# norlab-ulaval/mask_bev

Measured on AMD Instinct MI355X. Metric: LiDAR scans/sec fwd+bwd, 120k-pt 512x512 BEV 100q, higher is better.
Workload: dtype bf16; 1 GPU; semantic_kitti_512: 120000 pts/scan, 512x512 BEV, 100 queries; scans_per_gpu=4, global_batch=4, parallelism=dp1, step=fwd + Hungarian loss + bwd + AdamW; inputs device-resident, launch=hip-graph, tuned_gemm_table=True, k3_adam_fused=True

## Files before the change

### include/maskbev_hip.h

```cpp
#ifndef MASKBEV_HIP_H_
#define MASKBEV_HIP_H_

#include <stddef.h>
#include <stdint.h>

#ifdef __cplusplus
extern "C" {
#endif

typedef enum {
  MBV_OK = 0,
  MBV_ERR_BAD_ARG = -1,
  MBV_ERR_WORKSPACE = -2,
  MBV_ERR_UNSUPPORTED = -3
} mbv_status;

int mbv_abi_version(void);

#define MBV_DT_F32 0
#define MBV_DT_BF16 1
#define MBV_DT_F16 2

size_t mbv_voxelize_workspace_bytes(int64_t total_points, int32_t batch, int64_t cells_per_scan);

// ... 18 lines not shown
int mbv_skinny_gemm_f32_supported(int64_t m, int32_t contraction, int32_t out_cols);
int mbv_skinny_gemm_f32(const float* x, const float* w, float* y, int64_t m, int32_t c, int32_t n, int32_t ldw,
                        int32_t weight_is_nk, void* stream);
int mbv_skinny_gemm_f32_addrows(const float* x, const float* w, float* y, int64_t m, int32_t c, int32_t n, int32_t ldw,
                                const float* add, const int64_t* index, void* stream);

int64_t mbv_pfn_forward_layout(int64_t num_rows, int64_t num_pillars, const int32_t* units, int32_t num_layers,
                               int64_t* offsets);
int mbv_pfn_forward(const float* rows, int32_t in_features, const int32_t* row_start, const int32_t* num_points,
                    const int64_t* row_pillar, int64_t num_rows, int64_t num_pillars, int32_t max_points,
                    const float* const* weights,
                    const float* const* gammas, const float* const* betas, float* const* running_means,
                    float* const* running_vars, const int32_t* units, int32_t num_layers, float eps, float momentum,
                    int32_t training, float* workspace, int64_t workspace_floats, void* stream);

int mbv_pfn_stats(float* y, const float* t, float* y_pad, const int32_t* row_start, const int32_t* num_points,
                  int64_t num_pillars, int32_t units, int32_t max_points, double* sums, void* stream);

int mbv_pfn_bn_finalize(const double* sums, double count, const float* gamma, const float* beta, float eps,
                        float momentum, int32_t training, float* running_mean, float* running_var, int32_t units,
                        float* scale, float* shift, float* mean, float* rstd, void* stream);

int mbv_pfn_apply_max(const float* y, const float* y_pad, const float* scale, const float* shift,
                      const int32_t* row_start, const int32_t* num_points, int64_t num_pillars, int32_t units,
                      int32_t max_points, float* a, float* a_pad, float* m, void* stream);

int mbv_pfn_bwd_route(const float* y, const float* y_pad, const float* scale, const float* shift,
                      const float* mean, const float* rstd, float* dz, int32_t has_da, const float* sum_da_pad,
                      const float* dm, const int32_t* row_start, const int32_t* num_points, int64_t num_pillars,
                      int32_t units, int32_t max_points, float* dz_pad, double* sums, void* stream);

int mbv_pfn_bwd_bn(const float* y, const float* y_pad, float* dz, float* dz_pad, const float* mean,
                   const float* rstd, const float* gamma, const double* sums, double count, int32_t training,
                   const int32_t* row_start, const int32_t* num_points, int64_t num_pillars, int32_t units,
                   int32_t max_points, float* dt, void* stream);

size_t mbv_scatter_layernorm_workspace_bytes(int32_t batch);

int mbv_scatter_layernorm_patch_supported(int32_t channels, int32_t ny, int32_t nx, int32_t patch);

int mbv_scatter_layernorm_fwd(const float* feats, const int32_t* pillar_batch_start,
                              const int32_t* cell_to_pillar, const float* weight, const float* bias,
                              int32_t batch, int32_t channels, int32_t ny, int32_t nx, float eps,
                              int32_t patch, int32_t patch_dtype, void* out, float* stats, void* workspace,
                              size_t workspace_bytes, void* stream, void* ev_start, void* ev_stop);
int mbv_scatter_layernorm_fwd2(const float* feats, const int32_t* pillar_batch_start, const int32_t* cell_to_pillar,
                               const float* weight, const float* bias, int32_t batch, int32_t channels, int32_t ny, int32_t nx,
                               float eps, int32_t patch, int32_t patch_dtype, void* out, float* stats, void* workspace,
                               size_t workspace_bytes, uint32_t* amax_out, void* stream, void* ev_start, void* ev_stop);

int mbv_scatter_layernorm_bwd(const void* grad_out, int32_t patch, int32_t patch_dtype, const float* feats,
                              const int32_t* pillar_batch_start, const int32_t* cell_to_pillar,
                              const float* weight, const float* stats,
                              int32_t batch, int32_t channels, int32_t ny, int32_t nx, int64_t num_pillars,
                              float* grad_feats, float* grad_weight, float* grad_bias, int32_t accumulate,
                              void* workspace, size_t workspace_bytes, void* stream,
                              void* ev_start, void* ev_stop);

int mbv_scatter_layernorm_bwd_adamw(const void* grad_out, int32_t patch, int32_t patch_dtype, const float* feats,
                                    const int32_t* pillar_batch_start, const int32_t* cell_to_pillar, float* weight,
                                    float* bias, const float* stats, int32_t batch, int32_t channels, int32_t ny, int32_t nx,
                                    int64_t num_pillars, float* grad_feats, float* exp_avg_w, float* exp_avg_sq_w,
                                    float* exp_avg_b, float* exp_avg_sq_b, void* shadow_w, void* shadow_b,
                                    int32_t shadow_dtype, float lr, float beta1, float beta2, float eps, float weight_decay,
                                    int64_t step, int32_t decoupled, void* workspace, size_t workspace_bytes, void* stream,
                                    void* ev_start, void* ev_stop);

int mbv_ms_deform_attn_fwd(const float* value, const int64_t* spatial_shapes, const int64_t* level_start,
                           const float* sampling_loc, const float* attn_weight,
                           int32_t batch, int32_t num_value, int32_t num_heads, int32_t head_dim,
                           int32_t num_levels, int32_t num_query, int32_t num_points,
                           float* out, void* stream);

int mbv_ms_deform_attn_fwd_v(const void* value, int32_t value_dtype, const int64_t* spatial_shapes, const int64_t* level_start,
                             const float* sampling_loc, const float* attn_weight, int32_t batch, int32_t num_value,
                             int32_t num_heads, int32_t head_dim, int32_t num_levels, int32_t num_query, int32_t num_points,
                             float* out, void* stream);
int mbv_ms_deform_attn_bwd_locattn(const float* grad_out, const void* value, int32_t value_dtype, const int64_t* spatial_shapes,
                                   const int64_t* level_start, const float* sampling_loc, const float* attn_weight,
                                   int32_t batch, int32_t num_value, int32_t num_heads, int32_t head_dim, int32_t num_levels,
                                   int32_t num_query, int32_t num_points, float* grad_loc, float* grad_attn, void* stream);

int mbv_ms_deform_attn_bwd_split(int32_t head_dim, int32_t num_levels, const int64_t* spatial_shapes_host);

int mbv_ms_deform_attn_bwd_value_packed_supported(int32_t head_dim, int32_t num_levels, int32_t num_points,
                                                  int32_t num_query, const int64_t* spatial_shapes_host);
size_t mbv_ms_deform_attn_bwd_value_packed_workspace_bytes(int32_t batch, int32_t num_heads, int32_t num_levels,
                                                           int32_t num_query);
int mbv_ms_deform_attn_bwd_value_packed(const float* grad_out, const float* sampling_loc, const float* attn_weight,
                                        int32_t batch, int32_t num_value, int32_t num_heads, int32_t head_dim,
                                        int32_t num_levels, int32_t num_query, int32_t num_points,
                                        const int64_t* spatial_shapes_host, void* grad_value, int32_t out_dtype,
                                        int64_t out_ld, void* workspace, size_t workspace_bytes, void* stream);

int mbv_ms_deform_attn_bwd(const float* grad_out, const float* value, const int64_t* spatial_shapes,
                           const int64_t* level_start, const float* sampling_loc, const float* attn_weight,
                           int32_t batch, int32_t num_value, int32_t num_heads, int32_t head_dim,
                           int32_t num_levels, int32_t num_query, int32_t num_points,
                           const int64_t* spatial_shapes_host, float* grad_value, float* grad_loc, float* grad_attn,
                           int32_t part, void* stream);

int mbv_msda_prepare_supported(int32_t num_levels, int32_t num_points);

int mbv_msda_query_inputs(const float* x, const float* pos, int64_t rows, int64_t pos_rows, int32_t C, int32_t dtype,
                          void* x_lo, void* q_lo, void* stream);

int mbv_msda_prepare_fwd(const void* offsets, const void* logits, int32_t is_bf16, const float* ref_points,
                         const int64_t* spatial_shapes_host, int32_t batch, int32_t num_query, int32_t num_heads,
                         int32_t num_levels, int32_t num_points, float* loc, float* attn, void* stream);

int mbv_msda_prepare_fwd_ld(const void* offsets, int64_t ld_offsets, const void* logits, int64_t ld_logits,
                            const float* bias_offsets, const float* bias_logits, int32_t is_bf16, const float* ref_points,
                            const int64_t* spatial_shapes_host, int32_t batch, int32_t num_query, int32_t num_heads,
                            int32_t num_levels, int32_t num_points, float* loc, float* attn, void* stream);

int mbv_msda_prepare_bwd(const float* grad_loc, const float* grad_attn, const float* attn,
                         const int64_t* spatial_shapes_host, int32_t batch, int32_t num_query, int32_t num_heads,
                         int32_t num_levels, int32_t num_points, int32_t out_bf16, void* grad_offsets,
                         void* grad_logits, void* stream);

int mbv_msda_prepare_bwd_ld(const float* grad_loc, const float* grad_attn, const float* attn,
                            const int64_t* spatial_shapes_host, int32_t batch, int32_t num_query, int32_t num_heads,
                            int32_t num_levels, int32_t num_points, int32_t out_bf16, void* grad_offsets,
                            int64_t ld_offsets, void* grad_logits, int64_t ld_logits, void* stream);

int64_t mbv_window_attn_lse_elems(int32_t batch, int32_t H, int32_t W, int32_t heads, int32_t ws);

int mbv_window_attn_fwd(const void* qkv, const float* qkv_bias, const float* bias_table, int32_t is_bf16,
                        int32_t batch, int32_t H, int32_t W, int32_t C, int32_t heads, int32_t ws, int32_t shift,
                        void* out, float* lse, void* stream);

int mbv_window_attn_bwd(const void* qkv, const float* qkv_bias, const float* bias_table, const void* out,
                        const void* grad_out, const float* lse, int32_t is_bf16,
                        int32_t batch, int32_t H, int32_t W, int32_t C, int32_t heads, int32_t ws, int32_t shift,
                        void* grad_qkv, float* grad_table, float* grad_qkv_bias, int32_t full_bias_grad,
                        int32_t accumulate, void* stream);

int mbv_window_attn_split_supported(int32_t C, int32_t heads, int32_t ws);
int mbv_window_attn_split_fwd(const float* qkv, const float* qkv_bias, const float* bias_table, int32_t batch, int32_t H,
                              int32_t W, int32_t C, int32_t heads, int32_t ws, int32_t shift, const uint32_t* amax_qkv,
                              float* out, float* lse, void* stream);
int mbv_window_attn_split_bwd(const float* qkv, const float* qkv_bias, const float* bias_table, const float* out,
                              const float* grad_out, const float* lse, int32_t batch, int32_t H, int32_t W, int32_t C,
                              int32_t heads, int32_t ws, int32_t shift, const uint32_t* amax_qkv,
                              const uint32_t* amax_grad_out, float* grad_qkv, float* grad_table, float* grad_qkv_bias,
                              int32_t full_bias_grad, int32_t accumulate, uint32_t* amax_grad_qkv, void* stream);

int mbv_point_sample_fwd(const float* src, const int32_t* src_index, const float* coords,
                         const int32_t* coord_index, int32_t num_rows, int32_t num_points, int32_t H, int32_t W,
                         float* out, void* stream);

int mbv_point_sample_bwd(const float* grad_out, const int32_t* src_index, const float* coords,
                         const int32_t* coord_index, int32_t num_rows, int32_t num_points, int32_t H, int32_t W,
                         int64_t num_src_maps, float* grad_src, void* stream);

int mbv_point_sample_bwd_stack(const float* grad_out, const int32_t* src_index, const float* coords,
                               const int32_t* coord_index, int32_t num_rows, int32_t num_points, int32_t H, int32_t W,
                               int32_t outer, int32_t inner, int32_t rows, void* grad_src, int32_t out_dtype, void* stream);

int64_t mbv_packed_mask_words(int32_t H, int32_t W);

int mbv_pack_binary_masks(const float* src, int64_t num_maps, int32_t H, int32_t W, uint32_t* packed, void* stream);

int mbv_point_sample_packed_fwd(const uint32_t* packed, const int32_t* src_index, const float* coords,
                                const int32_t* coord_index, int32_t num_rows, int32_t num_points,
                                int32_t H, int32_t W, float* out, void* stream);
// ... 324 lines not shown
```

### mask_bev_amd/_lib.py

```python
from __future__ import annotations

import ctypes
import os
from ctypes import c_double, c_float, c_int32, c_int64, c_size_t, c_void_p
from typing import Dict, List, Tuple

_PKG_DIR = os.path.dirname(os.path.abspath(__file__))
LIB_PATH = os.path.join(_PKG_DIR, 'libmaskbev_hip.so')

ABI_VERSION = 59


class MaskBevHipError(RuntimeError):
    pass


_P = c_void_p
_F = c_float
_I = c_int32
_L = c_int64
_D = c_double

SIGNATURES: Dict[str, Tuple[object, List[object]]] = {
    'mbv_abi_version': (ctypes.c_int, []),
    'mbv_voxelize_workspace_bytes': (c_size_t, [_L, _I, _L]),
    'mbv_voxelize': (ctypes.c_int, [_P, _I, _L, _P, _I, _F, _F, _F, _F, _F, _F, _F, _F, _F, _I, _I, _I, _I, _I, _I, _L,
                                    _P, _P, _P, _P, _P, _P, _P, c_size_t, _P]),
    'mbv_gather_voxels': (ctypes.c_int, [_P, _I, _P, _L, _I, _P, _P]),
    'mbv_pfn_decorate': (ctypes.c_int, [_P, _I, _P, _P, _P, _P, _L, _I, _F, _F, _F, _F, _F, _F, _P, _P, _P]),
    'mbv_pfn_stats': (ctypes.c_int, [_P, _P, _P, _P, _P, _L, _I, _I, _P, _P]),
    'mbv_pfn_bn_finalize': (ctypes.c_int, [_P, c_double, _P, _P, _F, _F, _I, _P, _P, _I, _P, _P, _P, _P, _P]),
    'mbv_pfn_apply_max': (ctypes.c_int, [_P, _P, _P, _P, _P, _P, _L, _I, _I, _P, _P, _P, _P]),
    'mbv_pfn_bwd_route': (ctypes.c_int, [_P, _P, _P, _P, _P, _P, _P, _I, _P, _P, _P, _P, _L, _I, _I, _P, _P, _P]),
    'mbv_pfn_bwd_bn': (ctypes.c_int, [_P, _P, _P, _P, _P, _P, _P, _P, c_double, _I, _P, _P, _L, _I, _I, _P, _P]),
    'mbv_scatter_layernorm_workspace_bytes': (c_size_t, [_I]),
    'mbv_scatter_layernorm_patch_supported': (ctypes.c_int, [_I, _I, _I, _I]),
    'mbv_scatter_layernorm_fwd': (ctypes.c_int, [_P, _P, _P, _P, _P, _I, _I, _I, _I, _F, _I, _I, _P, _P, _P, c_size_t,
                                                 _P, _P, _P]),
    'mbv_scatter_layernorm_fwd2': (ctypes.c_int, [_P, _P, _P, _P, _P, _I, _I, _I, _I, _F, _I, _I, _P, _P, _P, c_size_t,
                                                  _P, _P, _P, _P]),
    'mbv_scatter_layernorm_bwd': (ctypes.c_int, [_P, _I, _I, _P, _P, _P, _P, _P, _I, _I, _I, _I, _L, _P, _P, _P, _I, _P,
                                                 c_size_t, _P, _P, _P]),
    'mbv_scatter_layernorm_bwd_adamw': (ctypes.c_int, [_P, _I, _I, _P, _P, _P, _P, _P, _P, _I, _I, _I, _I, _L, _P, _P, _P, _P, _P,
                                                       _P, _P, _I, _F, _F, _F, _F, _F, _L, _I, _P, c_size_t, _P, _P, _P]),
    'mbv_msda_prepare_supported': (ctypes.c_int, [_I, _I]),
    'mbv_pfn_forward_layout': (ctypes.c_int64, [_L, _L, _P, _I, _P]),
    'mbv_pfn_forward': (ctypes.c_int, [_P, _I, _P, _P, _P, _L, _L, _I, _P, _P, _P, _P, _P, _P, _I, _F, _F, _I, _P, _L, _P]),
    'mbv_skinny_gemm_f32_addrows': (ctypes.c_int, [_P, _P, _P, _L, _I, _I, _I, _P, _P, _P]),
    'mbv_skinny_gemm_f32_supported': (ctypes.c_int, [_L, _I, _I]),
    'mbv_skinny_gemm_f32': (ctypes.c_int, [_P, _P, _P, _L, _I, _I, _I, _I, _P]),
    'mbv_msda_prepare_fwd': (ctypes.c_int, [_P, _P, _I, _P, _P, _I, _I, _I, _I, _I, _P, _P, _P]),
    'mbv_msda_prepare_fwd_ld': (ctypes.c_int, [_P, _L, _P, _L, _P, _P, _I, _P, _P, _I, _I, _I, _I, _I, _P, _P, _P]),
    'mbv_msda_prepare_bwd': (ctypes.c_int, [_P, _P, _P, _P, _I, _I, _I, _I, _I, _I, _P, _P, _P]),
    'mbv_msda_prepare_bwd_ld': (ctypes.c_int, [_P, _P, _P, _P, _I, _I, _I, _I, _I, _I, _P, _L, _P, _L, _P]),
    'mbv_ms_deform_attn_fwd': (ctypes.c_int, [_P, _P, _P, _P, _P, _I, _I, _I, _I, _I, _I, _I, _P, _P]),
    'mbv_ms_deform_attn_fwd_v': (ctypes.c_int, [_P, _I, _P, _P, _P, _P, _I, _I, _I, _I, _I, _I, _I, _P, _P]),
    'mbv_ms_deform_attn_bwd_locattn': (ctypes.c_int, [_P, _P, _I, _P, _P, _P, _P, _I, _I, _I, _I, _I, _I, _I, _P, _P, _P]),
    'mbv_ms_deform_attn_bwd_split': (ctypes.c_int, [_I, _I, _P]),
    'mbv_ms_deform_attn_bwd_value_packed_supported': (ctypes.c_int, [_I, _I, _I, _I, _P]),
    'mbv_ms_deform_attn_bwd_value_packed_workspace_bytes': (c_size_t, [_I, _I, _I, _I]),
    'mbv_ms_deform_attn_bwd_value_packed': (ctypes.c_int, [_P, _P, _P, _I, _I, _I, _I, _I, _I, _I, _P, _P, _I, _L, _P, c_size_t, _P]),
    'mbv_ms_deform_attn_bwd': (ctypes.c_int, [_P, _P, _P, _P, _P, _P, _I, _I, _I, _I, _I, _I, _I, _P, _P, _P, _P, _I,
                                              _P]),
    'mbv_rowchain_max_stages': (ctypes.c_int, []),
    'mbv_rowchain_slots': (ctypes.c_int, []),
    'mbv_rowchain_run': (ctypes.c_int, [_P, _I, _I, _I, _F, _I, _P]),
    'mbv_rowchain_run_split': (ctypes.c_int, [_P, _I, _I, _I, _F, _I, _I, _P]),
    'mbv_transpose_group': (ctypes.c_int, [_P, _P, _P, _P, _I, _I, _P]),
    'mbv_copy_group': (ctypes.c_int, [_P, _P, _P, _I, _P]),
    'mbv_fragment_group': (ctypes.c_int, [_P, _P, _P, _P, _P, _P, _I, _P]),
    'mbv_window_attn_lse_elems': (_L, [_I, _I, _I, _I, _I]),
    'mbv_window_attn_fwd': (ctypes.c_int, [_P, _P, _P, _I, _I, _I, _I, _I, _I, _I, _I, _P, _P, _P]),
    'mbv_window_attn_bwd': (ctypes.c_int, [_P, _P, _P, _P, _P, _P, _I, _I, _I, _I, _I, _I, _I, _I, _P, _P, _P, _I, _I, _P]),
    'mbv_point_sample_fwd': (ctypes.c_int, [_P, _P, _P, _P, _I, _I, _I, _I, _P, _P]),
    'mbv_point_sample_bwd': (ctypes.c_int, [_P, _P, _P, _P, _I, _I, _I, _I, _L, _P, _P]),
    'mbv_point_sample_bwd_stack': (ctypes.c_int, [_P, _P, _P, _P, _I, _I, _I, _I, _I, _I, _I, _P, _I, _P]),
    'mbv_hungarian': (ctypes.c_int, [_P, _I, _I, _I, _P, _P]),
    'mbv_hungarian_padded': (ctypes.c_int, [_P, _I, _I, _I, _P, _P, _P]),
    'mbv_hungarian_wide_t': (ctypes.c_int, [_P, _I, _I, _I, _P, _P]),
    'mbv_select_uncertain_points': (ctypes.c_int, [_P, _P, _L, _I, _I, _P, _P]),
    'mbv_adamw_step': (ctypes.c_int, [_P, _P, _P, _P, _P, _I, _L, _F, _F, _F, _F, _F, _L, _F, _I, _I, _P, _P, _P, _P]),
    'mbv_grad_nonfinite': (ctypes.c_int, [_P, _L, _P, _P]),
    'mbv_loss_scale_update': (ctypes.c_int, [_P, _P, _P, _F, _F, _I, _P, _P]),
    'mbv_refresh_shadow': (ctypes.c_int, [_P, _P, _I, _L, _P]),
    'mbv_colsum_accum': (ctypes.c_int, [_P, _I, _L, _I, _P, _P]),
    'mbv_act_bwd_colsum': (ctypes.c_int, [_P, _P, _I, _I, _L, _I, _P, _P, _P]),
    'mbv_wgrad_small_f32': (ctypes.c_int, [_P, _P, _I, _I, _I, _P, _P, _P]),
    'mbv_wgrad_small_f32_group': (ctypes.c_int, [_P, _P, _P, _P, _P, _P, _P, _I, _P]),
    'mbv_mask_loss_rows_fwd': (ctypes.c_int, [_P, _P, _L, _I, _P, _P]),
    'mbv_mask_loss_rows_bwd': (ctypes.c_int, [_P, _P, _P, _L, _I, _P, _P]),
    'mbv_dice_bce_reduce': (ctypes.c_int, [_P, _L, _I, _F, _F, _P, _P, _P, _P]),
    'mbv_mask_loss_rows_bwd_coef': (ctypes.c_int, [_P, _P, _P, _P, _I, _P, _I, _L, _I, _I, _P, _P]),
    'mbv_sample_select_uncertain': (ctypes.c_int, [_P, _P, _P, _P, _L, _I, _I, _I, _I, _P, _I, _P, _P]),
    'mbv_uniform_points': (ctypes.c_int, [_P, _L, _I, _P, _P]),
    'mbv_add_layernorm_supported': (ctypes.c_int, [_I]),
    'mbv_add_layernorm_bwd_blocks': (_L, [_L, _I]),
    'mbv_add_layernorm_fwd': (ctypes.c_int, [_P, _I, _P, _I, _P, _P, _L, _I, _F, _P, _P, _I, _P, _P, _P]),
    'mbv_add_layernorm_fwd2': (ctypes.c_int, [_P, _I, _P, _I, _L, _P, _P, _L, _I, _F, _P, _P, _I, _P, _I, _P, _P, _P]),
    'mbv_transposed_batch_sum_accum': (ctypes.c_int, [_P, _I, _L, _I, _P, _P]),
    'mbv_add_layernorm_bwd': (ctypes.c_int, [_P, _I, _P, _I, _P, _P, _P, _P, _L, _I, _P, _P, _I, _P, _P, _I, _P, _P,
                                             _I, _P]),
    'mbv_add_layernorm_bwd2': (ctypes.c_int, [_P, _I, _P, _I, _P, _I, _P, _P, _P, _P, _L, _I, _P, _P, _I, _P, _P, _I, _P,
                                              _P, _I, _P]),
    'mbv_add_layernorm_bwd3': (ctypes.c_int, [_P, _I, _P, _I, _P, _I, _P, _P, _P, _P, _L, _I, _P, _P, _I, _P, _P, _I, _P,
                                              _P, _I, _P, _P]),
    'mbv_add_layernorm_bwd_direct': (ctypes.c_int, [_L, _I]),
    'mbv_merge_layernorm_supported': (ctypes.c_int, [_I, _I, _I]),
    'mbv_merge_layernorm_fwd': (ctypes.c_int, [_P, _L, _I, _I, _I, _P, _P, _F, _P, _I, _P, _P, _P]),
    'mbv_merge_layernorm_bwd': (ctypes.c_int, [_P, _I, _P, _P, _P, _P, _L, _I, _I, _I, _P, _P, _P, _I, _P, _I, _P]),
    'mbv_colsum_accum_group': (ctypes.c_int, [_P, _P, _P, _P, _P, _P, _I, _P]),
    'mbv_instance_ids': (ctypes.c_int, [_P, _I, _I, _I, _I, _I, _P, _P, _P, _P]),
    'mbv_expand_instance_masks': (ctypes.c_int, [_P, _P, _I, _I, _I, _I, _P, _P, _P]),
    'mbv_matched_mask_iou': (ctypes.c_int, [_P, _P, _P, _P, _I, _I, _I, _I, _I, _P, _P, _P]),
    'mbv_match_cost_terms': (ctypes.c_int, [_P, _L, _I, _I, _I, _P, _P, _P]),
    'mbv_match_cost': (ctypes.c_int, [_P, _P, _P, _P, _L, _I, _I, _I, _I, _I, _P, _P]),
    'mbv_match_products_supported': (ctypes.c_int, [_I, _I, _I]),
    'mbv_match_products': (ctypes.c_int, [_P, _P, _L, _I, _I, _I, _I, _P, _P, _P]),
    'mbv_match_cost_split': (ctypes.c_int, [_P, _P, _P, _P, _L, _I, _I, _I, _I, _I, _I, _P, _P]),
    'mbv_cls_loss_fwd': (ctypes.c_int, [_P, _P, _P, _P, _I, _I, _I, _I, _I, _F, _F, _P, _P, _P]),
    'mbv_cls_loss_bwd': (ctypes.c_int, [_P, _P, _P, _P, _P, _P, _I, _I, _I, _I, _I, _F, _F, _P, _P]),
    'mbv_packed_mask_words': (_L, [_I, _I]),
    'mbv_pack_binary_masks': (ctypes.c_int, [_P, _L, _I, _I, _P, _P]),
    'mbv_point_sample_packed_fwd': (ctypes.c_int, [_P, _P, _P, _P, _I, _I, _I, _I, _P, _P]),
    'mbv_mask_logits_fwd': (ctypes.c_int, [_P, _P, _I, _I, _I, _I, _L, _P, _I, _P]),
    'mbv_attn_mask_from_logits': (ctypes.c_int, [_P, _I, _L, _I, _I, _I, _I, _P, _P]),
    'mbv_attn_workspace_bytes': (c_size_t, [_I, _I, _I, _I, _I]),
    'mbv_attn_fwd': (ctypes.c_int, [_P, _P, _P, _P, _I, _I, _I, _I, _I, _I, _P, _P, _P, c_size_t, _P]),
    'mbv_attn_bwd': (ctypes.c_int, [_P, _P, _P, _P, _P, _P, _P, _I, _I, _I, _I, _I, _I, _P, _P, _P, _P]),
    'mbv_attn_fwd_ld': (ctypes.c_int, [_P, _P, _P, _I, _P, _I, _I, _I, _I, _I, _I, _P, _P, _P, c_size_t, _P]),
    'mbv_gemm16_supported': (ctypes.c_int, [_I, _L, _L, _L]),
    'mbv_gemm16_nt': (ctypes.c_int, [_P, _P, _P, _P, _P, _L, _L, _L, _L, _L, _L, _I, _I, _I, _I, _L, _L, _L, _P]),
    'mbv_gemm16_nt_acc': (ctypes.c_int, [_P, _P, _P, _L, _L, _L, _L, _L, _L, _I, _I, _I, _L, _L, _L, _P]),
    'mbv_gemm16_nn_workspace_bytes': (c_size_t, [_L, _L, _I]),
    'mbv_gemm16_nn': (ctypes.c_int, [_P, _P, _P, _P, _P, _L, _L, _L, _L, _L, _L, _L, _I, _I, _I, _I, _L, _L, _L, _P,
                                     c_size_t, _P]),
    'mbv_gemm16_nn_part_rows': (ctypes.c_int64, [_L, _L, _I]),
    'mbv_gemm16_nn_parts': (ctypes.c_int, [_P, _P, _P, _P, _P, c_size_t, _L, _L, _L, _L, _L, _L, _L, _I, _I, _I, _I, _L,
                                           _L, _L, _P]),
    'mbv_gemm16_tn_workspace_bytes': (c_size_t, [_L, _L, _L]),
    'mbv_gemm16_tn': (ctypes.c_int, [_P, _P, _P, _L, _L, _L, _L, _L, _L, _I, _I, _I, _I, _I, _L, _L, _L, _P, c_size_t,
                                     _P]),
# ... 99 lines not shown
```

### mask_bev_amd/csrc/msda.hip

```cpp

#include "common.hpp"

namespace {

__device__ __forceinline__ int64_t xcd_block(unsigned bid, unsigned nwg) {
  const unsigned q = nwg >> 3, r = nwg & 7, x = bid & 7, s = bid >> 3;
  return (int64_t)((x < r ? x * (q + 1) : r * (q + 1) + (x - r) * q) + s);
}

struct Corner {
  int off[4];
  float wgt[4];
  float lh, lw;
};

__device__ __forceinline__ bool bilinear_setup(float loc_x, float loc_y, int h, int w, int stride_pix, Corner& c) {
  const float him = loc_y * (float)h - 0.5f;
  const float wim = loc_x * (float)w - 0.5f;
  if (!(him > -1.f && wim > -1.f && him < (float)h && wim < (float)w)) return false;
  const int hl = (int)floorf(him), wl = (int)floorf(wim);
  const int hh = hl + 1, wh = wl + 1;
  const float lh = him - (float)hl, lw = wim - (float)wl;
  const float uh = 1.f - lh, uw = 1.f - lw;
  c.lh = lh;
  c.lw = lw;
  c.wgt[0] = uh * uw;
  c.wgt[1] = uh * lw;
  c.wgt[2] = lh * uw;
  c.wgt[3] = lh * lw;
  c.off[0] = (hl >= 0 && wl >= 0) ? (hl * w + wl) * stride_pix : -1;
  c.off[1] = (hl >= 0 && wh <= w - 1) ? (hl * w + wh) * stride_pix : -1;
  c.off[2] = (hh <= h - 1 && wl >= 0) ? (hh * w + wl) * stride_pix : -1;
  c.off[3] = (hh <= h - 1 && wh <= w - 1) ? (hh * w + wh) * stride_pix : -1;
  return true;
}

__global__ void __launch_bounds__(256) k_msda_fwd(const float* __restrict__ value,
                                                  const int64_t* __restrict__ shapes,
                                                  const int64_t* __restrict__ level_start,
                                                  const float* __restrict__ loc, const float* __restrict__ attn,
                                                  int64_t total, int num_value, int heads, int dim, int levels,
                                                  int num_query, int points, float* __restrict__ out) {
  const int64_t idx = (int64_t)blockIdx.x * blockDim.x + threadIdx.x;
  if (idx >= total) return;
  const int d = (int)(idx % dim);
  int64_t t = idx / dim;
  const int hd = (int)(t % heads);
  t /= heads;
  const int b = (int)(t / num_query);
  const int stride_pix = heads * dim;
  const float* vb = value + (int64_t)b * num_value * stride_pix + hd * dim + d;
  const int64_t lw_base = (t * heads + hd) * levels * points;
  float acc = 0.f;
  for (int l = 0; l < levels; ++l) {
    const int h = (int)shapes[l * 2], w = (int)shapes[l * 2 + 1];
    const float* vl = vb + level_start[l] * stride_pix;
    for (int p = 0; p < points; ++p) {
      const int64_t k = lw_base + l * points + p;
      const float lx = loc[k * 2], ly = loc[k * 2 + 1], aw = attn[k];
      Corner c;
      if (bilinear_setup(lx, ly, h, w, stride_pix, c)) {
        float v = 0.f;
#pragma unroll
        for (int j = 0; j < 4; ++j)
          if (c.off[j] >= 0) v += c.wgt[j] * vl[c.off[j]];
        acc += aw * v;
      }
    }
  }
  out[idx] = acc;
}

template <int VK>
__device__ __forceinline__ float4 value4(const void* __restrict__ base, int64_t elem) {
  if constexpr (VK == MBV_DT_F32) {
    return *reinterpret_cast<const float4*>(reinterpret_cast<const float*>(base) + elem);
  } else {
    const uint2 u = *reinterpret_cast<const uint2*>(reinterpret_cast<const unsigned short*>(base) + elem);
    if constexpr (VK == MBV_DT_BF16)
      return make_float4(__uint_as_float(u.x << 16), __uint_as_float(u.x & 0xffff0000u), __uint_as_float(u.y << 16),
                         __uint_as_float(u.y & 0xffff0000u));
    return make_float4((float)__builtin_bit_cast(_Float16, (unsigned short)(u.x & 0xffffu)),
                       (float)__builtin_bit_cast(_Float16, (unsigned short)(u.x >> 16)),
                       (float)__builtin_bit_cast(_Float16, (unsigned short)(u.y & 0xffffu)),
// ... 411 lines not shown
  l1 = red[0];
#pragma unroll
  for (int i = 1; i < NT / 64; ++i) l1 += red[i];
  l1 *= 1.0001f;
  if (!(l1 == l1) || l1 > 3.0e38f) l1 = 3.0e38f;
  int e = 0;
  if (l1 > 0.f) (void)frexpf(l1, &e);
  const float scale = ldexpf(1.f, 29 - e), inv_scale = ldexpf(1.f, e - 29);
  float4 n_go = make_float4(0.f, 0.f, 0.f, 0.f), n_l01 = n_go, n_l23 = n_go, n_a4 = n_go;
  const float* go_b = A.go_t + ((((int64_t)b * heads + hd) * 8 + grp4) * num_query) * 4 + (PLANES == 2 ? 0 : (split & 1) * 2);
  const float* loc_b = A.loc_t + ((((int64_t)b * heads + hd) * levels + level) * num_query) * 8;
  const float* attn_b = A.attn_t + ((((int64_t)b * heads + hd) * levels + level) * num_query) * 4;
  auto load_q = [&](int q, float4& go, float4& l01, float4& l23, float4& a4) {
    if constexpr (PLANES == 2) {
      go = *reinterpret_cast<const float4*>(go_b + (int64_t)q * 4);
    } else {
      const float2 g = *reinterpret_cast<const float2*>(go_b + (int64_t)q * 4);
      go = make_float4(g.x, g.y, 0.f, 0.f);
    }
    l01 = *reinterpret_cast<const float4*>(loc_b + (int64_t)q * 8);
    l23 = *reinterpret_cast<const float4*>(loc_b + (int64_t)q * 8 + 4);
    a4 = *reinterpret_cast<const float4*>(attn_b + (int64_t)q * 4);
  };
  if ((int)threadIdx.x < num_query) load_q(threadIdx.x, n_go, n_l01, n_l23, n_a4);
  for (int q = threadIdx.x; q < num_query; q += NT) {
    float4 go = n_go;
    const float4 l01 = n_l01, l23 = n_l23, a4 = n_a4;
    if (q + NT < num_query) load_q(q + NT, n_go, n_l01, n_l23, n_a4);
    go.x *= scale; go.y *= scale; go.z *= scale; go.w *= scale;
    const float lx[4] = {l01.x, l01.z, l23.x, l23.z}, ly[4] = {l01.y, l01.w, l23.y, l23.w};
    const float aw[4] = {a4.x, a4.y, a4.z, a4.w};
#pragma unroll
    for (int u = 0; u < 4; ++u) {
      Corner c;
      if (!bilinear_setup(lx[u], ly[u], h, w, 1, c)) continue;
#pragma unroll
      for (int j = 0; j < 4; ++j) {
        const int off = c.off[j];
        if (off < 0) continue;
        const float wj = c.wgt[j] * aw[u];
        atomicAdd(&map[off], fx_pack(wj * go.x, wj * go.y));
        if constexpr (PLANES == 2) atomicAdd(&map[npix + off], fx_pack(wj * go.z, wj * go.w));
      }
    }
  }
  __syncthreads();
  const int64_t gv = ((int64_t)b * A.num_value + A.lstart[level]) * A.out_ld + hd * dim + split * CH;
  for (int i = threadIdx.x; i < npix; i += NT) {
#pragma unroll
    for (int pl = 0; pl < PLANES; ++pl) {
      const long long v = (long long)map[pl * npix + i];
      const int lo = (int)(unsigned)(v & 0xffffffffll);
      const int hi = (int)((v - (long long)lo) >> 32);
      fx_store2<DT>(A.out, gv + (int64_t)i * A.out_ld + 2 * pl, (float)lo * inv_scale, (float)hi * inv_scale);
    }
  }
}

struct Taps4 {
  int off[4];
  float wgt[4];
};
__device__ __forceinline__ void taps_clamped(float loc_x, float loc_y, float aw, int h, int w, int stride_pix, Taps4& t) {
  const float him = loc_y * (float)h - 0.5f;
  const float wim = loc_x * (float)w - 0.5f;
  const bool in = him > -1.f && wim > -1.f && him < (float)h && wim < (float)w;
  const int hl = (int)floorf(him), wl = (int)floorf(wim);
  const int hh = hl + 1, wh = wl + 1;
  const float lh = him - (float)hl, lw = wim - (float)wl;
  const float uh = 1.f - lh, uw = 1.f - lw;
  const bool t0 = in && hl >= 0 && wl >= 0, t1 = in && hl >= 0 && wh <= w - 1;
  const bool t2 = in && hh <= h - 1 && wl >= 0, t3 = in && hh <= h - 1 && wh <= w - 1;
  t.off[0] = t0 ? (hl * w + wl) * stride_pix : 0;
  t.off[1] = t1 ? (hl * w + wh) * stride_pix : 0;
  t.off[2] = t2 ? (hh * w + wl) * stride_pix : 0;
  t.off[3] = t3 ? (hh * w + wh) * stride_pix : 0;
  t.wgt[0] = t0 ? aw * uh * uw : 0.f;
  t.wgt[1] = t1 ? aw * uh * lw : 0.f;
  t.wgt[2] = t2 ? aw * lh * uw : 0.f;
  t.wgt[3] = t3 ? aw * lh * lw : 0.f;
}

template <int VK>
__global__ void __launch_bounds__(256) k_msda_fwd_p4(const void* __restrict__ value, const int64_t* __restrict__ shapes,
                                                     const int64_t* __restrict__ level_start,
                                                     const float* __restrict__ loc, const float* __restrict__ attn,
                                                     int64_t total4, int num_value, int heads, int dim, int levels,
                                                     int num_query, float* __restrict__ out) {
  const int64_t idx = xcd_block(blockIdx.x, gridDim.x) * blockDim.x + threadIdx.x;
  if (idx >= total4) return;
  const int d4n = dim >> 2;
  const int d4 = (int)(idx % d4n);
  int64_t t = idx / d4n;
  const int hd = (int)(t % heads);
  t /= heads;
  const int b = (int)(t / num_query);
  const int stride_pix = heads * dim;
  const int64_t vb = (int64_t)b * num_value * stride_pix + hd * dim + d4 * 4;
  const int64_t lw_base = (t * heads + hd) * levels * 4;
  float4 acc = make_float4(0.f, 0.f, 0.f, 0.f);
  for (int l = 0; l < levels; ++l) {
    const int h = (int)shapes[l * 2], w = (int)shapes[l * 2 + 1];
    const int64_t vl = vb + level_start[l] * stride_pix;
    const float4 xy0 = *reinterpret_cast<const float4*>(loc + (lw_base + l * 4) * 2);
    const float4 xy1 = *reinterpret_cast<const float4*>(loc + (lw_base + l * 4) * 2 + 4);
    const float4 aw = *reinterpret_cast<const float4*>(attn + lw_base + l * 4);
    Taps4 tp[4];
    taps_clamped(xy0.x, xy0.y, aw.x, h, w, stride_pix, tp[0]);
    taps_clamped(xy0.z, xy0.w, aw.y, h, w, stride_pix, tp[1]);
    taps_clamped(xy1.x, xy1.y, aw.z, h, w, stride_pix, tp[2]);
    taps_clamped(xy1.z, xy1.w, aw.w, h, w, stride_pix, tp[3]);
    float4 x[16];
#pragma unroll
    for (int p = 0; p < 4; ++p)
#pragma unroll
      for (int j = 0; j < 4; ++j) x[p * 4 + j] = value4<VK>(value, vl + tp[p].off[j]);
#pragma unroll
    for (int p = 0; p < 4; ++p)
#pragma unroll
      for (int j = 0; j < 4; ++j) {
        const float wj = tp[p].wgt[j];
        acc.x += wj * x[p * 4 + j].x; acc.y += wj * x[p * 4 + j].y;
        acc.z += wj * x[p * 4 + j].z; acc.w += wj * x[p * 4 + j].w;
      }
  }
  *reinterpret_cast<float4*>(out + ((t * heads + hd) * dim + d4 * 4)) = acc;
}

__global__ void __launch_bounds__(256) k_msda_bwd_relayout(const float* __restrict__ grad_out,
                                                           const float* __restrict__ loc, const float* __restrict__ attn,
                                                           int num_query, int heads, int levels, int q_tiles,
                                                           float* __restrict__ go_t, float* __restrict__ loc_t,
                                                           float* __restrict__ attn_t, float* __restrict__ l1_part) {
  __shared__ __attribute__((aligned(16))) float s_go[64 * 32];
  __shared__ __attribute__((aligned(16))) float s_loc[64 * 8 * 8];
  __shared__ __attribute__((aligned(16))) float s_at[64 * 8 * 4];
  __shared__ float s_sum[8 * 8];
  const int tile = blockIdx.x % q_tiles;
  const int bh = blockIdx.x / q_tiles;
  const int hd = bh % heads, b = bh / heads;
  const int q0 = tile * 64;
  const int tid = threadIdx.x;
  if (tid < 64) s_sum[tid] = 0.f;
  for (int p = tid; p < 64 * 8; p += 256) {
    const int q = p >> 3, c = p & 7;
    const int qq = q0 + q < num_query ? q0 + q : num_query - 1;
    *reinterpret_cast<float4*>(s_go + q * 32 + c * 4) =
        *reinterpret_cast<const float4*>(grad_out + (((int64_t)b * num_query + qq) * heads + hd) * 32 + c * 4);
  }
  const int lp = levels * 2;
  for (int p = tid; p < 64 * lp; p += 256) {
    const int q = p / lp, c = p - q * lp;
    const int qq = q0 + q < num_query ? q0 + q : num_query - 1;
    *reinterpret_cast<float4*>(s_loc + q * 64 + c * 4) =
        *reinterpret_cast<const float4*>(loc + ((((int64_t)b * num_query + qq) * heads + hd) * levels) * 8 + c * 4);
  }
  for (int p = tid; p < 64 * levels; p += 256) {
    const int q = p / levels, l = p - q * levels;
    const int qq = q0 + q < num_query ? q0 + q : num_query - 1;
    *reinterpret_cast<float4*>(s_at + q * 32 + l * 4) =
        *reinterpret_cast<const float4*>(attn + ((((int64_t)b * num_query + qq) * heads + hd) * levels + l) * 4);
  }
  __syncthreads();
  for (int p = tid; p < 8 * 64; p += 256) {
    const int g = p >> 6, q = p & 63;
    if (q0 + q < num_query)
      *reinterpret_cast<float4*>(go_t + ((((int64_t)b * heads + hd) * 8 + g) * num_query + q0 + q) * 4) =
          *reinterpret_cast<const float4*>(s_go + q * 32 + g * 4);
  }
  for (int p = tid; p < levels * 64 * 2; p += 256) {
    const int l = p / 128, r = p - l * 128, q = r >> 1, hf = r & 1;
    if (q0 + q < num_query)
      *reinterpret_cast<float4*>(loc_t + ((((int64_t)b * heads + hd) * levels + l) * num_query + q0 + q) * 8 + hf * 4) =
          *reinterpret_cast<const float4*>(s_loc + q * 64 + l * 8 + hf * 4);
  }
  for (int p = tid; p < levels * 64; p += 256) {
    const int l = p >> 6, q = p & 63;
    if (q0 + q < num_query)
      *reinterpret_cast<float4*>(attn_t + ((((int64_t)b * heads + hd) * levels + l) * num_query + q0 + q) * 4) =
          *reinterpret_cast<const float4*>(s_at + q * 32 + l * 4);
  }
  for (int p = tid; p < 64 * 8; p += 256) {
    const int q = p & 63, g = p >> 6;
    const bool live = q0 + q < num_query;
    const float4 gv = *reinterpret_cast<const float4*>(s_go + q * 32 + g * 4);
    const float m = fmaxf(fmaxf(fabsf(gv.x), fabsf(gv.y)), fmaxf(fabsf(gv.z), fabsf(gv.w)));
    for (int l = 0; l < levels; ++l) {
      const float4 a = *reinterpret_cast<const float4*>(s_at + q * 32 + l * 4);
      float t = live ? m * (fabsf(a.x) + fabsf(a.y) + fabsf(a.z) + fabsf(a.w)) : 0.f;
#pragma unroll
      for (int o = 32; o > 0; o >>= 1) t += __shfl_xor(t, o);
      if ((tid & 63) == 0) s_sum[l * 8 + g] = t;
    }
  }
  __syncthreads();
  if (tid < levels * 8) {
    const int l = tid >> 3, g = tid & 7;
    l1_part[((((int64_t)b * heads + hd) * q_tiles + tile) * levels + l) * 8 + g] = s_sum[l * 8 + g];
  }
}

template <int DT>
__global__ void __launch_bounds__(512) k_msda_bwd_value_fx(const MsdaFxArgs A) {
  extern __shared__ __attribute__((aligned(16))) unsigned long long fxmap[];
  int level = 0;
  for (int l = 1; l < A.levels; ++l)
    if ((int)blockIdx.x >= A.block_begin[l]) level = l;
  const int local = (int)blockIdx.x - A.block_begin[level];
  if (A.planes[level] == 2)
// ... 11 lines not shown
                                                          int64_t total8, int num_value, int heads, int levels,
                                                          int num_query, int points, float* __restrict__ grad_loc,
                                                          float* __restrict__ grad_attn) {
  constexpr int dim = 32;
  const int stride_pix = heads * dim;
  const int64_t idx = xcd_block(blockIdx.x, gridDim.x) * blockDim.x + threadIdx.x;
  const bool live = idx < total8;
  const int64_t sidx = live ? idx : total8 - 1;
  const int d4 = (int)(sidx & 7);
  int64_t t = sidx >> 3;
  const int hd = (int)(t % heads);
  t /= heads;
  const int b = (int)(t / num_query);
  const int64_t vb = (int64_t)b * num_value * stride_pix + hd * dim + d4 * 4;
  const int64_t lw_base = (t * heads + hd) * levels * points;
  const float4 go = *reinterpret_cast<const float4*>(grad_out + (t * heads + hd) * dim + d4 * 4);
  float keep_w = 0.f, keep_x = 0.f, keep_y = 0.f;
  for (int l = 0; l < levels; ++l) {
    const int h = (int)shapes[l * 2], w = (int)shapes[l * 2 + 1];
    const int64_t vl = vb + level_start[l] * stride_pix;
    for (int p = 0; p < points; ++p) {
      const int64_t k = lw_base + l * points + p;
      const float lx = loc[k * 2], ly = loc[k * 2 + 1], aw = attn[k];
      float g_w = 0.f, g_x = 0.f, g_y = 0.f;
      Corner c;
      if (bilinear_setup(lx, ly, h, w, stride_pix, c)) {
        float s4[4];
#pragma unroll
        for (int j = 0; j < 4; ++j) {
          s4[j] = 0.f;
          if (c.off[j] >= 0) {
            const float4 x = value4<VK>(value, vl + c.off[j]);
            s4[j] = go.x * x.x + go.y * x.y + go.z * x.z + go.w * x.w;
          }
        }
        const float uh = 1.f - c.lh, uw = 1.f - c.lw;
        g_w = c.wgt[0] * s4[0] + c.wgt[1] * s4[1] + c.wgt[2] * s4[2] + c.wgt[3] * s4[3];
        const float gh = -uw * s4[0] - c.lw * s4[1] + uw * s4[2] + c.lw * s4[3];
        const float gw = -uh * s4[0] + uh * s4[1] - c.lh * s4[2] + c.lh * s4[3];
        g_x = (float)w * gw * aw;
        g_y = (float)h * gh * aw;
      }
      g_w = group8_allsum(g_w);
      g_x = group8_allsum(g_x);
      g_y = group8_allsum(g_y);
      const int sidx8 = l * points + p;
      if ((sidx8 & 7) == d4) { keep_w = g_w; keep_x = g_x; keep_y = g_y; }
      if ((sidx8 & 7) == 7 || (l == levels - 1 && p == points - 1)) {
        const int first = sidx8 & ~7;
        if (live && first + d4 <= sidx8) {
          grad_attn[lw_base + first + d4] = keep_w;
          *reinterpret_cast<float2*>(grad_loc + (lw_base + first + d4) * 2) = make_float2(keep_x, keep_y);
        }
      }
    }
  }
}

struct TapsG {
  int off[4];
  float ok[4];
  float lh, lw;
  float in;
};
__device__ __forceinline__ void taps_grad(float loc_x, float loc_y, int h, int w, int stride_pix, TapsG& t) {
  const float him = loc_y * (float)h - 0.5f;
  const float wim = loc_x * (float)w - 0.5f;
  const bool in = him > -1.f && wim > -1.f && him < (float)h && wim < (float)w;
  const int hl = (int)floorf(him), wl = (int)floorf(wim);
  const int hh = hl + 1, wh = wl + 1;
  t.lh = him - (float)hl;
  t.lw = wim - (float)wl;
  t.in = in ? 1.f : 0.f;
  const bool t0 = in && hl >= 0 && wl >= 0, t1 = in && hl >= 0 && wh <= w - 1;
  const bool t2 = in && hh <= h - 1 && wl >= 0, t3 = in && hh <= h - 1 && wh <= w - 1;
  t.off[0] = t0 ? (hl * w + wl) * stride_pix : 0;
  t.off[1] = t1 ? (hl * w + wh) * stride_pix : 0;
  t.off[2] = t2 ? (hh * w + wl) * stride_pix : 0;
  t.off[3] = t3 ? (hh * w + wh) * stride_pix : 0;
  t.ok[0] = t0 ? 1.f : 0.f; t.ok[1] = t1 ? 1.f : 0.f; t.ok[2] = t2 ? 1.f : 0.f; t.ok[3] = t3 ? 1.f : 0.f;
}

template <int VK>
__global__ void __launch_bounds__(256) k_msda_bwd_locattn_p4(const float* __restrict__ grad_out,
                                                             const void* __restrict__ value,
                                                             const int64_t* __restrict__ shapes,
                                                             const int64_t* __restrict__ level_start,
                                                             const float* __restrict__ loc, const float* __restrict__ attn,
                                                             int64_t total8, int num_value, int heads, int levels,
                                                             int num_query, float* __restrict__ grad_loc,
                                                             float* __restrict__ grad_attn) {
  constexpr int dim = 32, points = 4;
  const int stride_pix = heads * dim;
  const int64_t idx = xcd_block(blockIdx.x, gridDim.x) * blockDim.x + threadIdx.x;
  const bool live = idx < total8;
  const int64_t sidx = live ? idx : total8 - 1;
  const int d4 = (int)(sidx & 7);
  int64_t t = sidx >> 3;
  const int hd = (int)(t % heads);
  t /= heads;
  const int b = (int)(t / num_query);
  const int64_t vb = (int64_t)b * num_value * stride_pix + hd * dim + d4 * 4;
  const int64_t lw_base = (t * heads + hd) * levels * points;
  const float4 go = *reinterpret_cast<const float4*>(grad_out + (t * heads + hd) * dim + d4 * 4);
  float keep_w = 0.f, keep_x = 0.f, keep_y = 0.f;
  for (int l = 0; l < levels; ++l) {
    const int h = (int)shapes[l * 2], w = (int)shapes[l * 2 + 1];
    const int64_t vl = vb + level_start[l] * stride_pix;
    const float4 xy0 = *reinterpret_cast<const float4*>(loc + (lw_base + l * 4) * 2);
    const float4 xy1 = *reinterpret_cast<const float4*>(loc + (lw_base + l * 4) * 2 + 4);
    const float4 aw4 = *reinterpret_cast<const float4*>(attn + lw_base + l * 4);
    const float awp[4] = {aw4.x, aw4.y, aw4.z, aw4.w};
    TapsG tp[4];
    taps_grad(xy0.x, xy0.y, h, w, stride_pix, tp[0]);
    taps_grad(xy0.z, xy0.w, h, w, stride_pix, tp[1]);
    taps_grad(xy1.x, xy1.y, h, w, stride_pix, tp[2]);
    taps_grad(xy1.z, xy1.w, h, w, stride_pix, tp[3]);
    float4 x[16];
#pragma unroll
    for (int p = 0; p < 4; ++p)
#pragma unroll
      for (int j = 0; j < 4; ++j) x[p * 4 + j] = value4<VK>(value, vl + tp[p].off[j]);
#pragma unroll
    for (int p = 0; p < 4; ++p) {
      float s4[4];
#pragma unroll
      for (int j = 0; j < 4; ++j) {
        const float4 v = x[p * 4 + j];
        s4[j] = tp[p].ok[j] * (go.x * v.x + go.y * v.y + go.z * v.z + go.w * v.w);
      }
      const float lh = tp[p].lh, lw = tp[p].lw, uh = 1.f - lh, uw = 1.f - lw;
      float g_w = uh * uw * s4[0] + uh * lw * s4[1] + lh * uw * s4[2] + lh * lw * s4[3];
      const float gh = -uw * s4[0] - lw * s4[1] + uw * s4[2] + lw * s4[3];
      const float gw = -uh * s4[0] + uh * s4[1] - lh * s4[2] + lh * s4[3];
      float g_x = (float)w * gw * awp[p] * tp[p].in;
      float g_y = (float)h * gh * awp[p] * tp[p].in;
      g_w = group8_allsum(g_w * tp[p].in);
      g_x = group8_allsum(g_x);
      g_y = group8_allsum(g_y);
      const int sidx8 = l * points + p;
      if ((sidx8 & 7) == d4) { keep_w = g_w; keep_x = g_x; keep_y = g_y; }
      if ((sidx8 & 7) == 7 || (l == levels - 1 && p == points - 1)) {
        const int first = sidx8 & ~7;
        if (live && first + d4 <= sidx8) {
          grad_attn[lw_base + first + d4] = keep_w;
          *reinterpret_cast<float2*>(grad_loc + (lw_base + first + d4) * 2) = make_float2(keep_x, keep_y);
        }
      }
    }
  }
}

struct MsdaLevels {
  int levels;
  int h[8], w[8], lstart[8];
};

bool pow2_le64(int d) { return d > 0 && d <= 64 && (d & (d - 1)) == 0; }

}

extern "C" int mbv_ms_deform_attn_fwd(const float* value, const int64_t* spatial_shapes, const int64_t* level_start,
                                      const float* sampling_loc, const float* attn_weight, int32_t batch,
                                      int32_t num_value, int32_t num_heads, int32_t head_dim, int32_t num_levels,
                                      int32_t num_query, int32_t num_points, float* out, void* stream_) {
  hipStream_t stream = reinterpret_cast<hipStream_t>(stream_);
  if (batch <= 0 || num_value <= 0 || num_heads <= 0 || num_levels <= 0 || num_query <= 0 || num_points <= 0)
    return MBV_ERR_BAD_ARG;
  if (!pow2_le64(head_dim)) return MBV_ERR_UNSUPPORTED;
  if (!value || !spatial_shapes || !level_start || !sampling_loc || !attn_weight || !out) return MBV_ERR_BAD_ARG;
  const int64_t total = (int64_t)batch * num_query * num_heads * head_dim;
  if ((head_dim & 3) == 0 && ((reinterpret_cast<size_t>(value) | reinterpret_cast<size_t>(out)) & 15) == 0) {
    const int64_t total4 = total / 4;
    if (num_points == 4 && ((reinterpret_cast<size_t>(sampling_loc) | reinterpret_cast<size_t>(attn_weight)) & 15) == 0) {
      hipLaunchKernelGGL(k_msda_fwd_p4<MBV_DT_F32>, dim3((unsigned)((total4 + 255) / 256)), dim3(256), 0, stream,
                         (const void*)value, spatial_shapes, level_start, sampling_loc, attn_weight, total4, num_value,
                         num_heads, head_dim, num_levels, num_query, out);
      MBV_CHECK_LAUNCH();
      return MBV_OK;
    }
    hipLaunchKernelGGL(k_msda_fwd_v4<MBV_DT_F32>, dim3((unsigned)((total4 + 255) / 256)), dim3(256), 0, stream,
                       (const void*)value, spatial_shapes, level_start, sampling_loc, attn_weight, total4, num_value,
                       num_heads, head_dim, num_levels, num_query, num_points, out);
    MBV_CHECK_LAUNCH();
    return MBV_OK;
  }
  hipLaunchKernelGGL(k_msda_fwd, dim3((unsigned)((total + 255) / 256)), dim3(256), 0, stream, value, spatial_shapes,
                     level_start, sampling_loc, attn_weight, total, num_value, num_heads, head_dim, num_levels,
                     num_query, num_points, out);
  MBV_CHECK_LAUNCH();
  return MBV_OK;
}

extern "C" int mbv_ms_deform_attn_fwd_v(const void* value, int32_t value_dtype, const int64_t* spatial_shapes,
                                        const int64_t* level_start, const float* sampling_loc, const float* attn_weight,
                                        int32_t batch, int32_t num_value, int32_t num_heads, int32_t head_dim,
                                        int32_t num_levels, int32_t num_query, int32_t num_points, float* out, void* stream_) {
  if (value_dtype == MBV_DT_F32)
    return mbv_ms_deform_attn_fwd(reinterpret_cast<const float*>(value), spatial_shapes, level_start, sampling_loc,
                                  attn_weight, batch, num_value, num_heads, head_dim, num_levels, num_query, num_points, out,
                                  stream_);
  hipStream_t stream = reinterpret_cast<hipStream_t>(stream_);
  if (batch <= 0 || num_value <= 0 || num_heads <= 0 || num_levels <= 0 || num_query <= 0 || num_points <= 0)
    return MBV_ERR_BAD_ARG;
  if (value_dtype != MBV_DT_BF16 && value_dtype != MBV_DT_F16) return MBV_ERR_BAD_ARG;
  if (!pow2_le64(head_dim) || (head_dim & 3)) return MBV_ERR_UNSUPPORTED;
  if (!value || !spatial_shapes || !level_start || !sampling_loc || !attn_weight || !out) return MBV_ERR_BAD_ARG;
  if ((reinterpret_cast<size_t>(value) & 7) || (reinterpret_cast<size_t>(out) & 15)) return MBV_ERR_UNSUPPORTED;
  const int64_t total4 = (int64_t)batch * num_query * num_heads * head_dim / 4;
  const dim3 grid((unsigned)((total4 + 255) / 256)), block(256);
  if (num_points == 4 && ((reinterpret_cast<size_t>(sampling_loc) | reinterpret_cast<size_t>(attn_weight)) & 15) == 0) {
    if (value_dtype == MBV_DT_BF16)
      hipLaunchKernelGGL(k_msda_fwd_p4<MBV_DT_BF16>, grid, block, 0, stream, value, spatial_shapes, level_start, sampling_loc,
                         attn_weight, total4, num_value, num_heads, head_dim, num_levels, num_query, out);
    else
      hipLaunchKernelGGL(k_msda_fwd_p4<MBV_DT_F16>, grid, block, 0, stream, value, spatial_shapes, level_start, sampling_loc,
                         attn_weight, total4, num_value, num_heads, head_dim, num_levels, num_query, out);
    MBV_CHECK_LAUNCH();
    return MBV_OK;
  }
  if (value_dtype == MBV_DT_BF16)
    hipLaunchKernelGGL(k_msda_fwd_v4<MBV_DT_BF16>, grid, block, 0, stream, value, spatial_shapes, level_start, sampling_loc,
                       attn_weight, total4, num_value, num_heads, head_dim, num_levels, num_query, num_points, out);
  else
    hipLaunchKernelGGL(k_msda_fwd_v4<MBV_DT_F16>, grid, block, 0, stream, value, spatial_shapes, level_start, sampling_loc,
                       attn_weight, total4, num_value, num_heads, head_dim, num_levels, num_query, num_points, out);
  MBV_CHECK_LAUNCH();
  return MBV_OK;
}

extern "C" int mbv_ms_deform_attn_bwd_locattn(const float* grad_out, const void* value, int32_t value_dtype,
                                              const int64_t* spatial_shapes, const int64_t* level_start,
                                              const float* sampling_loc, const float* attn_weight, int32_t batch,
                                              int32_t num_value, int32_t num_heads, int32_t head_dim, int32_t num_levels,
                                              int32_t num_query, int32_t num_points, float* grad_loc, float* grad_attn,
                                              void* stream_) {
  hipStream_t stream = reinterpret_cast<hipStream_t>(stream_);
  if (batch <= 0 || num_value <= 0 || num_heads <= 0 || num_levels <= 0 || num_query <= 0 || num_points <= 0)
    return MBV_ERR_BAD_ARG;
  if (head_dim != 32) return MBV_ERR_UNSUPPORTED;
  if (!grad_out || !value || !spatial_shapes || !level_start || !sampling_loc || !attn_weight || !grad_loc || !grad_attn)
    return MBV_ERR_BAD_ARG;
  if ((reinterpret_cast<size_t>(grad_out) & 15) || (reinterpret_cast<size_t>(value) & (value_dtype == MBV_DT_F32 ? 15 : 7)))
    return MBV_ERR_UNSUPPORTED;
  const int64_t total8 = (int64_t)batch * num_query * num_heads * 8;
  const dim3 grid((unsigned)((total8 + 255) / 256)), block(256);
  const bool p4 = num_points == 4 && ((reinterpret_cast<size_t>(sampling_loc) | reinterpret_cast<size_t>(attn_weight)) & 15) == 0;
#define MBV_LOCATTN(VK)                                                                                                  \
  if (p4)                                                                                                                \
    hipLaunchKernelGGL(k_msda_bwd_locattn_p4<VK>, grid, block, 0, stream, grad_out, value, spatial_shapes, level_start,  \
                       sampling_loc, attn_weight, total8, num_value, num_heads, num_levels, num_query, grad_loc,         \
                       grad_attn);                                                                                       \
  else                                                                                                                   \
    hipLaunchKernelGGL(k_msda_bwd_locattn<VK>, grid, block, 0, stream, grad_out, value, spatial_shapes, level_start,     \
                       sampling_loc, attn_weight, total8, num_value, num_heads, num_levels, num_query, num_points,       \
                       grad_loc, grad_attn)
  if (value_dtype == MBV_DT_F32) { MBV_LOCATTN(MBV_DT_F32); }
  else if (value_dtype == MBV_DT_BF16) { MBV_LOCATTN(MBV_DT_BF16); }
  else if (value_dtype == MBV_DT_F16) { MBV_LOCATTN(MBV_DT_F16); }
  else return MBV_ERR_BAD_ARG;
#undef MBV_LOCATTN
  MBV_CHECK_LAUNCH();
  return MBV_OK;
}

extern "C" int mbv_ms_deform_attn_bwd_split(int32_t head_dim, int32_t num_levels, const int64_t* spatial_shapes_host) {
  if (!spatial_shapes_host || head_dim != 32 || num_levels <= 0 || num_levels > 8) return 0;
  for (int l = 0; l < num_levels; ++l) {
    const int64_t h = spatial_shapes_host[2 * l], w = spatial_shapes_host[2 * l + 1];
    if (h <= 0 || w <= 0 || h * w > 4096) return 0;
  }
  return 1;
}

extern "C" int mbv_ms_deform_attn_bwd(const float* grad_out, const float* value, const int64_t* spatial_shapes,
                                      const int64_t* level_start, const float* sampling_loc,
                                      const float* attn_weight, int32_t batch, int32_t num_value, int32_t num_heads,
                                      int32_t head_dim, int32_t num_levels, int32_t num_query, int32_t num_points,
                                      const int64_t* spatial_shapes_host, float* grad_value, float* grad_loc,
                                      float* grad_attn, int32_t part, void* stream_) {
  hipStream_t stream = reinterpret_cast<hipStream_t>(stream_);
  if (batch <= 0 || num_value <= 0 || num_heads <= 0 || num_levels <= 0 || num_query <= 0 || num_points <= 0)
    return MBV_ERR_BAD_ARG;
  if (!pow2_le64(head_dim)) return MBV_ERR_UNSUPPORTED;
  if (!grad_out || !value || !spatial_shapes || !level_start || !sampling_loc || !attn_weight) return MBV_ERR_BAD_ARG;
  if ((!grad_value && ((part & 3) != 2)) || ((!grad_loc || !grad_attn) && ((part & 3) != 1))) return MBV_ERR_BAD_ARG;
  const int level_mask = part >> 2;
  part &= 3;
  if (part < 1 || level_mask < 0 || level_mask > 255 || (level_mask && part != 1)) return MBV_ERR_BAD_ARG;
  {
    bool fits = mbv_ms_deform_attn_bwd_split(head_dim, num_levels, spatial_shapes_host) != 0 &&
                ((reinterpret_cast<size_t>(grad_out) | reinterpret_cast<size_t>(value) |
                  reinterpret_cast<size_t>(grad_value) | reinterpret_cast<size_t>(sampling_loc) |
                  reinterpret_cast<size_t>(attn_weight)) & 15) == 0;
    MsdaLevels lv;
    lv.levels = num_levels;
    int lstart = 0, max_pix = 0;
    for (int l = 0; fits && l < num_levels; ++l) {
      const int h = (int)spatial_shapes_host[2 * l], w = (int)spatial_shapes_host[2 * l + 1];
      if (h <= 0 || w <= 0 || h * w > 4096) { fits = false; break; }
      lv.h[l] = h; lv.w[l] = w; lv.lstart[l] = lstart;
      lstart += h * w;
      if (h * w > max_pix) max_pix = h * w;
    }
    if (fits && lstart == num_value) {
      static bool attr_done = false;
      if (!attr_done && max_pix * 32 > 65536) {
        MBV_CHECK_HIP(hipFuncSetAttribute(reinterpret_cast<const void*>(&k_msda_bwd_value<4>),
                                          hipFuncAttributeMaxDynamicSharedMemorySize, 131072));
        MBV_CHECK_HIP(hipFuncSetAttribute(reinterpret_cast<const void*>(&k_msda_bwd_value<0>),
                                          hipFuncAttributeMaxDynamicSharedMemorySize, 131072));
        attr_done = true;
      }
      const int which = part;
      for (int l = num_levels - 1; l >= 0 && (which & 1); --l) {
        if (level_mask && !((level_mask >> l) & 1)) continue;
        const dim3 grid((unsigned)(batch * num_heads * 8)), block(1024);
        const size_t lds = (size_t)lv.h[l] * lv.w[l] * 4 * sizeof(double);
        if (num_points == 4)
          hipLaunchKernelGGL(k_msda_bwd_value<4>, grid, block, lds, stream, grad_out, sampling_loc, attn_weight, l,
                             num_levels, lv.h[l], lv.w[l], lv.lstart[l], num_value, num_query, num_heads, num_points,
                             grad_value);
        else
          hipLaunchKernelGGL(k_msda_bwd_value<0>, grid, block, lds, stream, grad_out, sampling_loc, attn_weight, l,
                             num_levels, lv.h[l], lv.w[l], lv.lstart[l], num_value, num_query, num_heads, num_points,
                             grad_value);
        MBV_CHECK_LAUNCH();
      }
      if (which & 2) {
        const int64_t total8 = (int64_t)batch * num_query * num_heads * 8;
        if (num_points == 4 && ((reinterpret_cast<size_t>(sampling_loc) | reinterpret_cast<size_t>(attn_weight)) & 15) == 0)
          hipLaunchKernelGGL(k_msda_bwd_locattn_p4<MBV_DT_F32>, dim3((unsigned)((total8 + 255) / 256)), dim3(256), 0, stream,
                             grad_out, (const void*)value, spatial_shapes, level_start, sampling_loc, attn_weight, total8,
                             num_value, num_heads, num_levels, num_query, grad_loc, grad_attn);
        else
          hipLaunchKernelGGL(k_msda_bwd_locattn<MBV_DT_F32>, dim3((unsigned)((total8 + 255) / 256)), dim3(256), 0, stream,
                             grad_out, (const void*)value, spatial_shapes, level_start, sampling_loc, attn_weight, total8,
                             num_value, num_heads, num_levels, num_query, num_points, grad_loc, grad_attn);
        MBV_CHECK_LAUNCH();
      }
      return MBV_OK;
    }
  }
  if (part != 3) return MBV_ERR_UNSUPPORTED;
  MBV_CHECK_HIP(mbv_fill_async(grad_value, 0, sizeof(float) * (size_t)batch * num_value * num_heads * head_dim, stream));
  if (spatial_shapes_host && num_query == num_value && num_levels <= 8) {
    MsdaBands cfg;
    cfg.levels = num_levels;
// ... 133 lines not shown
```

### mask_bev_amd/csrc/msda_prepare.hip

```cpp
#include "common.hpp"

namespace {

constexpr int kMaxLP = 16;

template <typename T>
__device__ __forceinline__ float ldf(const T* p);
template <>
__device__ __forceinline__ float ldf<float>(const float* p) { return *p; }
template <>
__device__ __forceinline__ float ldf<unsigned short>(const unsigned short* p) { return __uint_as_float((unsigned)*p << 16); }
template <typename T>
__device__ __forceinline__ void stf(T* p, float v);
template <>
__device__ __forceinline__ void stf<float>(float* p, float v) { *p = v; }
template <>
__device__ __forceinline__ void stf<unsigned short>(unsigned short* p, float v) { *p = f32_to_bf16_rne(v); }
template <typename T>
__device__ __forceinline__ float round_like(float v);
template <>
__device__ __forceinline__ float round_like<float>(float v) { return v; }
template <>
__device__ __forceinline__ float round_like<unsigned short>(float v) { return __uint_as_float((unsigned)f32_to_bf16_rne(v) << 16); }

template <typename T>
__device__ __forceinline__ void ld4(const T* p, float* v);
template <>
__device__ __forceinline__ void ld4<float>(const float* p, float* v) {
  const float4 q = *reinterpret_cast<const float4*>(p);
  v[0] = q.x; v[1] = q.y; v[2] = q.z; v[3] = q.w;
}
template <>
__device__ __forceinline__ void ld4<unsigned short>(const unsigned short* p, float* v) {
  const uint2 u = *reinterpret_cast<const uint2*>(p);
  v[0] = __uint_as_float(u.x << 16); v[1] = __uint_as_float(u.x & 0xffff0000u);
  v[2] = __uint_as_float(u.y << 16); v[3] = __uint_as_float(u.y & 0xffff0000u);
}
template <typename T>
__device__ __forceinline__ void st4(T* p, const float* v);
template <>
__device__ __forceinline__ void st4<float>(float* p, const float* v) {
  *reinterpret_cast<float4*>(p) = make_float4(v[0], v[1], v[2], v[3]);
}
template <>
__device__ __forceinline__ void st4<unsigned short>(unsigned short* p, const float* v) {
  uint2 u;
  u.x = pack_bf16x2(v[0], v[1]);
  u.y = pack_bf16x2(v[2], v[3]);
  *reinterpret_cast<uint2*>(p) = u;
}

template <>
__device__ __forceinline__ float ldf<_Float16>(const _Float16* p) { return (float)*p; }
template <>
__device__ __forceinline__ void stf<_Float16>(_Float16* p, float v) { *p = (_Float16)v; }
template <>
__device__ __forceinline__ float round_like<_Float16>(float v) { return (float)(_Float16)v; }
template <>
__device__ __forceinline__ void ld4<_Float16>(const _Float16* p, float* v) {
  typedef _Float16 h4 __attribute__((ext_vector_type(4)));
  const h4 q = *reinterpret_cast<const h4*>(p);
  v[0] = (float)q[0]; v[1] = (float)q[1]; v[2] = (float)q[2]; v[3] = (float)q[3];
}
template <>
__device__ __forceinline__ void st4<_Float16>(_Float16* p, const float* v) {
  typedef _Float16 h4 __attribute__((ext_vector_type(4)));
  h4 q;
  q[0] = (_Float16)v[0]; q[1] = (_Float16)v[1]; q[2] = (_Float16)v[2]; q[3] = (_Float16)v[3];
  *reinterpret_cast<h4*>(p) = q;
}

struct Norm { float w[8], h[8]; };

template <typename T>
__global__ void __launch_bounds__(256) k_msda_prepare_fwd(const T* __restrict__ off, const T* __restrict__ logit,
                                                          const float* __restrict__ ref, Norm nrm, long rows,
                                                          int num_query, int heads, int levels, int points,
                                                          float* __restrict__ loc, float* __restrict__ attn,
                                                          long ld_off, long ld_logit, const float* __restrict__ b_off,
                                                          const float* __restrict__ b_logit) {
  const long i = (long)blockIdx.x * blockDim.x + threadIdx.x;
  if (i >= rows) return;
  const int lp = levels * points;
  const long tok = i / heads;
  const int head = (int)(i - tok * heads);
  const int n = (int)(tok % num_query);
  const float rx = ref[2 * n], ry = ref[2 * n + 1];
  const T* o = off + tok * ld_off + (long)head * lp * 2;
  const T* a = logit + tok * ld_logit + (long)head * lp;
  const float* bo = b_off ? b_off + (long)head * lp * 2 : nullptr;
  const float* ba = b_logit ? b_logit + (long)head * lp : nullptr;
  float v[kMaxLP];
  float m = -INFINITY;
  const bool vec = (lp & 3) == 0;
  if (vec) {
#pragma unroll
    for (int k = 0; k < kMaxLP; k += 4) {
      if (k < lp) ld4<T>(a + k, v + k);
      else v[k] = v[k + 1] = v[k + 2] = v[k + 3] = -INFINITY;
    }
  } else {
#pragma unroll
    for (int k = 0; k < kMaxLP; ++k) v[k] = k < lp ? ldf<T>(a + k) : -INFINITY;
  }
  if (ba) {
#pragma unroll
    for (int k = 0; k < kMaxLP; ++k)
      if (k < lp) v[k] += ba[k];
  }
#pragma unroll
  for (int k = 0; k < kMaxLP; ++k) m = fmaxf(m, v[k]);
  float s = 0.f;
#pragma unroll
  for (int k = 0; k < kMaxLP; ++k) {
    v[k] = k < lp ? expf(v[k] - m) : 0.f;
    s += v[k];
  }
  const float inv = 1.f / s;
  float* lo = loc + i * lp * 2;
  float* ao = attn + i * lp;
  if (vec) {
#pragma unroll
    for (int k = 0; k < kMaxLP; k += 4) {
      if (k < lp) {
        const float w4[4] = {v[k] * inv, v[k + 1] * inv, v[k + 2] * inv, v[k + 3] * inv};
        st4<float>(ao + k, w4);
        float o8[8], r8[8];
        ld4<T>(o + 2 * k, o8);
        ld4<T>(o + 2 * k + 4, o8 + 4);
        if (bo) {
#pragma unroll
          for (int e = 0; e < 8; ++e) o8[e] += bo[2 * k + e];
        }
#pragma unroll
        for (int e = 0; e < 4; ++e) {
          const int l = (k + e) / points;
          r8[2 * e] = rx + round_like<T>(o8[2 * e] / nrm.w[l]);
          r8[2 * e + 1] = ry + round_like<T>(o8[2 * e + 1] / nrm.h[l]);
        }
        st4<float>(lo + 2 * k, r8);
        st4<float>(lo + 2 * k + 4, r8 + 4);
      }
    }
    return;
  }
#pragma unroll
  for (int k = 0; k < kMaxLP; ++k) {
    if (k < lp) {
      const int l = k / points;
      ao[k] = v[k] * inv;
      lo[2 * k] = rx + round_like<T>((ldf<T>(o + 2 * k) + (bo ? bo[2 * k] : 0.f)) / nrm.w[l]);
      lo[2 * k + 1] = ry + round_like<T>((ldf<T>(o + 2 * k + 1) + (bo ? bo[2 * k + 1] : 0.f)) / nrm.h[l]);
    }
  }
}

template <typename T>
__global__ void __launch_bounds__(256) k_msda_prepare_bwd(const float* __restrict__ g_loc,
                                                          const float* __restrict__ g_attn,
                                                          const float* __restrict__ attn, Norm nrm, long rows,
                                                          int levels, int points, T* __restrict__ g_off,
                                                          T* __restrict__ g_logit, int heads, long ld_off,
                                                          long ld_logit) {
  const long i = (long)blockIdx.x * blockDim.x + threadIdx.x;
  if (i >= rows) return;
  const int lp = levels * points;
  const float* gl = g_loc + i * lp * 2;
  const float* ga = g_attn + i * lp;
  const float* aw = attn + i * lp;
  float a[kMaxLP], g[kMaxLP];
  float dot = 0.f;
  const bool vec = (lp & 3) == 0;
  if (vec) {
#pragma unroll
    for (int k = 0; k < kMaxLP; k += 4) {
      if (k < lp) {
        ld4<float>(aw + k, a + k);
        ld4<float>(ga + k, g + k);
      } else {
        a[k] = a[k + 1] = a[k + 2] = a[k + 3] = 0.f;
        g[k] = g[k + 1] = g[k + 2] = g[k + 3] = 0.f;
      }
    }
  } else {
#pragma unroll
    for (int k = 0; k < kMaxLP; ++k) {
      a[k] = k < lp ? aw[k] : 0.f;
      g[k] = k < lp ? ga[k] : 0.f;
    }
  }
#pragma unroll
  for (int k = 0; k < kMaxLP; ++k) dot += a[k] * g[k];
  const long bn = i / heads;
  const int hh = (int)(i - bn * heads);
  T* go = g_off + bn * ld_off + (long)hh * lp * 2;
  T* gq = g_logit + bn * ld_logit + (long)hh * lp;
  if (vec) {
#pragma unroll
    for (int k = 0; k < kMaxLP; k += 4) {
      if (k < lp) {
        const float q4[4] = {a[k] * (g[k] - dot), a[k + 1] * (g[k + 1] - dot), a[k + 2] * (g[k + 2] - dot),
                             a[k + 3] * (g[k + 3] - dot)};
        st4<T>(gq + k, q4);
        float l8[8], o8[8];
        ld4<float>(gl + 2 * k, l8);
        ld4<float>(gl + 2 * k + 4, l8 + 4);
#pragma unroll
        for (int e = 0; e < 4; ++e) {
          const int l = (k + e) / points;
          o8[2 * e] = round_like<T>(l8[2 * e]) / nrm.w[l];
          o8[2 * e + 1] = round_like<T>(l8[2 * e + 1]) / nrm.h[l];
        }
        st4<T>(go + 2 * k, o8);
        st4<T>(go + 2 * k + 4, o8 + 4);
      }
    }
    return;
  }
#pragma unroll
  for (int k = 0; k < kMaxLP; ++k) {
    if (k < lp) {
      const int l = k / points;
      stf<T>(gq + k, a[k] * (g[k] - dot));
      stf<T>(go + 2 * k, round_like<T>(gl[2 * k]) / nrm.w[l]);
      stf<T>(go + 2 * k + 1, round_like<T>(gl[2 * k + 1]) / nrm.h[l]);
    }
  }
}

bool fill_norm(const int64_t* shapes_host, int levels, Norm& n) {
  if (!shapes_host || levels < 1 || levels > 8) return false;
  for (int l = 0; l < 8; ++l) { n.w[l] = 1.f; n.h[l] = 1.f; }
  for (int l = 0; l < levels; ++l) {
    const int64_t h = shapes_host[2 * l], w = shapes_host[2 * l + 1];
    if (h <= 0 || w <= 0) return false;
    n.h[l] = (float)h; n.w[l] = (float)w;
  }
  return true;
}

__global__ void __launch_bounds__(256) k_msda_query_inputs(const float* __restrict__ x, const float* __restrict__ pos,
                                                           long n4, long pos_n4, int f16, unsigned short* __restrict__ x_lo,
                                                           unsigned short* __restrict__ q_lo) {
  const long i = (long)blockIdx.x * 256 + threadIdx.x;
  if (i >= n4) return;
  const float4 a = reinterpret_cast<const float4*>(x)[i];
  const float4 p = reinterpret_cast<const float4*>(pos)[i % pos_n4];
  const float q[4] = {a.x + p.x, a.y + p.y, a.z + p.z, a.w + p.w};
  const float v[4] = {a.x, a.y, a.z, a.w};
  unsigned short xo[4], qo[4];
#pragma unroll
  for (int e = 0; e < 4; ++e) {
    if (f16) {
      xo[e] = __builtin_bit_cast(unsigned short, (_Float16)v[e]);
      qo[e] = __builtin_bit_cast(unsigned short, (_Float16)q[e]);
    } else {
      xo[e] = f32_to_bf16_rne(v[e]);
      qo[e] = f32_to_bf16_rne(q[e]);
    }
  }
  reinterpret_cast<uint2*>(x_lo)[i] = make_uint2(xo[0] | ((unsigned)xo[1] << 16), xo[2] | ((unsigned)xo[3] << 16));
  reinterpret_cast<uint2*>(q_lo)[i] = make_uint2(qo[0] | ((unsigned)qo[1] << 16), qo[2] | ((unsigned)qo[3] << 16));
}

}

extern "C" int mbv_msda_prepare_supported(int32_t num_levels, int32_t num_points) {
  return num_levels >= 1 && num_levels <= 8 && num_points >= 1 && num_levels * num_points <= kMaxLP;
}

extern "C" int mbv_msda_prepare_fwd_ld(const void* offsets, int64_t ld_offsets, const void* logits, int64_t ld_logits,
                                       const float* bias_offsets, const float* bias_logits, int32_t is_bf16,
                                       const float* ref_points, const int64_t* spatial_shapes_host, int32_t batch,
                                       int32_t num_query, int32_t num_heads, int32_t num_levels, int32_t num_points,
                                       float* loc, float* attn, void* stream) {
  if (batch <= 0 || num_query <= 0 || num_heads <= 0) return MBV_ERR_BAD_ARG;
  if (ld_offsets < (int64_t)num_heads * num_levels * num_points * 2 || ld_logits < (int64_t)num_heads * num_levels * num_points)
    return MBV_ERR_BAD_ARG;
  if (!mbv_msda_prepare_supported(num_levels, num_points)) return MBV_ERR_UNSUPPORTED;
  {
    const size_t es = is_bf16 ? 2 : 4;
    if ((num_levels * num_points) % 4 == 0 &&
        (((reinterpret_cast<size_t>(offsets) | reinterpret_cast<size_t>(logits)) & (4 * es - 1)) != 0 ||
         (ld_offsets % 4) != 0 || (ld_logits % 4) != 0))
      return MBV_ERR_BAD_ARG;
  }
  if (!offsets || !logits || !ref_points || !loc || !attn) return MBV_ERR_BAD_ARG;
  Norm n;
  if (!fill_norm(spatial_shapes_host, num_levels, n)) return MBV_ERR_BAD_ARG;
  const long rows = (long)batch * num_query * num_heads;
  const dim3 grid((unsigned)((rows + 255) / 256)), block(256);
  if (is_bf16 == MBV_DT_F16)
    hipLaunchKernelGGL(k_msda_prepare_fwd<_Float16>, grid, block, 0, (hipStream_t)stream,
                       reinterpret_cast<const _Float16*>(offsets), reinterpret_cast<const _Float16*>(logits),
                       ref_points, n, rows, num_query, num_heads, num_levels, num_points, loc, attn, (long)ld_offsets,
                       (long)ld_logits, bias_offsets, bias_logits);
  else if (is_bf16)
    hipLaunchKernelGGL(k_msda_prepare_fwd<unsigned short>, grid, block, 0, (hipStream_t)stream,
                       reinterpret_cast<const unsigned short*>(offsets), reinterpret_cast<const unsigned short*>(logits),
                       ref_points, n, rows, num_query, num_heads, num_levels, num_points, loc, attn, (long)ld_offsets,
                       (long)ld_logits, bias_offsets, bias_logits);
  else
    hipLaunchKernelGGL(k_msda_prepare_fwd<float>, grid, block, 0, (hipStream_t)stream,
                       reinterpret_cast<const float*>(offsets), reinterpret_cast<const float*>(logits), ref_points, n,
                       rows, num_query, num_heads, num_levels, num_points, loc, attn, (long)ld_offsets, (long)ld_logits,
                       bias_offsets, bias_logits);
  MBV_CHECK_LAUNCH();
  return MBV_OK;
}

extern "C" int mbv_msda_prepare_fwd(const void* offsets, const void* logits, int32_t is_bf16, const float* ref_points,
                                    const int64_t* spatial_shapes_host, int32_t batch, int32_t num_query,
                                    int32_t num_heads, int32_t num_levels, int32_t num_points, float* loc, float* attn,
                                    void* stream) {
  const int64_t lp = (int64_t)num_levels * num_points;
  if (!offsets || !logits) return MBV_ERR_BAD_ARG;
  return mbv_msda_prepare_fwd_ld(offsets, num_heads * lp * 2, logits, num_heads * lp, nullptr, nullptr, is_bf16,
                                 ref_points, spatial_shapes_host, batch, num_query, num_heads, num_levels, num_points, loc,
                                 attn, stream);
}

// ... 56 lines not shown
```

### mask_bev_amd/layers.py

```python
from __future__ import annotations

import math
from typing import Dict, Optional, Sequence, Tuple

import torch
import torch.nn as nn
import torch.nn.functional as F

from . import ops


def trunc_normal_(t: torch.Tensor, std: float = 0.02) -> torch.Tensor:
    return nn.init.trunc_normal_(t, mean=0.0, std=std, a=-2 * std, b=2 * std)


class Linear(nn.Linear):

    def forward(self, x: torch.Tensor, skip_bias_grad: bool = False) -> torch.Tensor:
        return ops.linear(x, self.weight, self.bias, skip_bias_grad=skip_bias_grad)


class LayerNorm(nn.LayerNorm):

    def forward(self, x: torch.Tensor, residual: Optional[torch.Tensor] = None, gemm_input: bool = False,
# ... 178 lines not shown
        px = torch.stack((px[:, :, 0::2].sin(), px[:, :, 1::2].cos()), dim=3).view(h, w, -1)
        py = torch.stack((py[:, :, 0::2].sin(), py[:, :, 1::2].cos()), dim=3).view(h, w, -1)
        pe = torch.cat((py, px), dim=2).permute(2, 0, 1).unsqueeze(0).contiguous()
        _SINE_CACHE[key] = pe
    return pe


class _AttnParams(nn.Module):

    def __init__(self, embed_dims: int):
        super().__init__()
        self.in_proj_weight = nn.Parameter(torch.empty(3 * embed_dims, embed_dims))
        self.in_proj_bias = nn.Parameter(torch.zeros(3 * embed_dims))
        self.out_proj = Linear(embed_dims, embed_dims)
        nn.init.xavier_uniform_(self.in_proj_weight)
        nn.init.zeros_(self.out_proj.bias)


class MultiheadAttention(nn.Module):

    def __init__(self, embed_dims: int, num_heads: int):
        super().__init__()
        self.embed_dims, self.num_heads = embed_dims, num_heads
        self.attn = _AttnParams(embed_dims)

    def forward(self, query, key, value, query_pos=None, key_pos=None, blocked: Optional[torch.Tensor] = None,
                add_identity: bool = True, defer_out_bias: bool = False, shared_kv=None):
        e, h = self.embed_dims, self.num_heads
        w, bias = self.attn.in_proj_weight, self.attn.in_proj_bias
        q_in = query + query_pos if query_pos is not None else query
        q = ops.linear(q_in, w, bias, rows=(0, e))
        if shared_kv is not None:
            holder, token, slot = shared_kv
            o = ops.attention_shared_kv(q, token, blocked, h, holder, slot)
        else:
            if key is query and key_pos is query_pos:
                k = q_in
            else:
                k = key + key_pos if key_pos is not None else key
            k = ops.linear(k, w, bias, rows=(e, 2 * e))
            v = ops.linear(value, w, bias, rows=(2 * e, 3 * e))
            o = ops.attention(q, k, v, blocked, h)
        o = self.attn.out_proj(o, skip_bias_grad=defer_out_bias and not add_identity)
        return query + o if add_identity else o


class MultiScaleDeformableAttention(nn.Module):

    def __init__(self, embed_dims: int = 256, num_heads: int = 8, num_levels: int = 3, num_points: int = 4):
        super().__init__()
        self.embed_dims, self.num_heads, self.num_levels, self.num_points = embed_dims, num_heads, num_levels, num_points
        self.sampling_offsets = Linear(embed_dims, num_heads * num_levels * num_points * 2)
        self.attention_weights = Linear(embed_dims, num_heads * num_levels * num_points)
        self.value_proj = Linear(embed_dims, embed_dims)
        self.output_proj = Linear(embed_dims, embed_dims)
        self.init_weights()

    def init_weights(self):
        nn.init.zeros_(self.sampling_offsets.weight)
        thetas = torch.arange(self.num_heads, dtype=torch.float32) * (2.0 * math.pi / self.num_heads)
        grid = torch.stack([thetas.cos(), thetas.sin()], -1)
        grid = (grid / grid.abs().max(-1, keepdim=True)[0]).view(self.num_heads, 1, 1, 2).repeat(
            1, self.num_levels, self.num_points, 1)
        for i in range(self.num_points):
            grid[:, :, i, :] *= i + 1
        with torch.no_grad():
            self.sampling_offsets.bias.copy_(grid.view(-1))
        nn.init.zeros_(self.attention_weights.weight)
        nn.init.zeros_(self.attention_weights.bias)
        nn.init.xavier_uniform_(self.value_proj.weight)
        nn.init.zeros_(self.value_proj.bias)
        nn.init.xavier_uniform_(self.output_proj.weight)
        nn.init.zeros_(self.output_proj.bias)

    def forward(self, query: torch.Tensor, query_pos: torch.Tensor, reference_points: torch.Tensor,
                spatial_shapes: Sequence[Tuple[int, int]], shapes_t: torch.Tensor, level_start: torch.Tensor,
                add_identity: bool = True, defer_out_bias: bool = False, pos_share=None, pos_share_index: int = 0,
                wcat=None):
        b, n, e = query.shape
        h, l, p = self.num_heads, self.num_levels, self.num_points
        if (spatial_shapes is not None and query.is_cuda and query.dtype == torch.float32
                and query_pos.shape[0] == 1 and sum(hh * ww for hh, ww in spatial_shapes) == n
                and ops.msda_prepare_supported(l, p)):
            out = ops.msda_query_side(query, query_pos, reference_points, self.value_proj, self.sampling_offsets,
                                      self.attention_weights, h, l, p, spatial_shapes, shapes_t, level_start,
                                      pos_share=pos_share, pos_share_index=pos_share_index, wcat=wcat)
            out = self.output_proj(out, skip_bias_grad=defer_out_bias and not add_identity)
            return out + query if add_identity else out
        q = query + query_pos
        if torch.is_autocast_enabled('cuda') and q.is_cuda:
            q = q.to(torch.get_autocast_dtype('cuda'))
        value = self.value_proj(query).view(b, n, h, e // h)
        off = self.sampling_offsets(q).view(b, n, h, l, p, 2)
        aw = self.attention_weights(q).view(b, n, h, l * p)
        if spatial_shapes is not None and off.is_cuda and ops.msda_prepare_supported(l, p):
            loc, aw = ops.msda_prepare(off, aw, reference_points, spatial_shapes)
        else:
            aw = aw.softmax(-1).view(b, n, h, l, p)
            normalizer = torch.stack([shapes_t[:, 1], shapes_t[:, 0]], -1).to(off.dtype)
            loc = reference_points.view(1, n, 1, 1, 1, 2) + off / normalizer.view(1, 1, 1, l, 1, 2)
        out = ops.ms_deform_attn(value, spatial_shapes, shapes_t, level_start, loc, aw)
        out = self.output_proj(out, skip_bias_grad=defer_out_bias and not add_identity)
        return out + query if add_identity else out
```

### mask_bev_amd/ops_msda.py

```python
from __future__ import annotations

import ctypes
from dataclasses import dataclass
from typing import List, Optional, Sequence

import torch

from . import _lib, switches
from ._lib import MaskBevHipError, check
from .ops_core import *
from .ops_records import *
from .ops_gemm import *


class _MSDeformAttn(torch.autograd.Function):
    @staticmethod
    @torch.amp.custom_fwd(device_type='cuda', cast_inputs=torch.float32)
    def forward(ctx, value, shapes_t, level_start, loc, attn, shapes_host):
        lib = _lib.load()
        _need_gpu(value, shapes_t, level_start, loc, attn)
        ctx.shapes_host = shapes_host
        value, loc, attn = value.contiguous(), loc.contiguous(), attn.contiguous()
        b, nv, nh, d = value.shape
        _, nq, _, nl, npnt, _ = loc.shape
        out = torch.empty((b, nq, nh * d), dtype=torch.float32, device=value.device)
        rc = lib.mbv_ms_deform_attn_fwd(_ptr(value), _ptr(shapes_t), _ptr(level_start), _ptr(loc), _ptr(attn), b, nv,
                                        nh, d, nl, nq, npnt, _ptr(out), _stream())
        check(rc, 'mbv_ms_deform_attn_fwd')
        ctx.save_for_backward(value, shapes_t, level_start, loc, attn)
        return out

    @staticmethod
    @torch.amp.custom_bwd(device_type='cuda')
    def backward(ctx, grad_out):
        lib = _lib.load()
        value, shapes_t, level_start, loc, attn = ctx.saved_tensors
        b, nv, nh, d = value.shape
        _, nq, _, nl, npnt, _ = loc.shape
        grad_out = grad_out.to(torch.float32).contiguous()
        g_value = torch.empty_like(value)
        g_loc = torch.empty_like(loc)
        g_attn = torch.empty_like(attn)
        host = None
        if ctx.shapes_host is not None and len(ctx.shapes_host) == nl:
            host = (ctypes.c_int64 * (2 * nl))(*[int(v) for hw in ctx.shapes_host for v in hw])
        _msda_backward(lib, grad_out, value, shapes_t, level_start, loc, attn, (b, nv, nh, d, nl, nq, npnt), host,
                       g_value, g_loc, g_attn)
        return g_value, None, None, g_loc, g_attn, None


def msda_value_packed_ok(dims, host) -> bool:
    b, nv, nh, d, nl, nq, npnt = dims
    return bool(host is not None
                and _lib.load().mbv_ms_deform_attn_bwd_value_packed_supported(d, nl, npnt, nq, host))


def _msda_backward(lib, g_out, value, shapes_t, level_start, loc, attn, dims, host, g_value, g_loc, g_attn,
                   packed_out=None):
    if packed_out is not None:
        b, nv, nh, d, nl, nq, npnt = dims
        dst, ld = packed_out
        ws = _workspace(lib.mbv_ms_deform_attn_bwd_value_packed_workspace_bytes(b, nh, nl, nq), g_out.device)
        check(lib.mbv_ms_deform_attn_bwd_value_packed(_ptr(g_out), _ptr(loc), _ptr(attn), b, nv, nh, d, nl, nq, npnt, host,
                                                      _ptr(dst), _dt_flag(dst.dtype), int(ld), _ptr(ws), ws.numel(), _stream()),
              'mbv_ms_deform_attn_bwd_value_packed')
        check(lib.mbv_ms_deform_attn_bwd_locattn(_ptr(g_out), _ptr(value), _dt_flag(value.dtype), _ptr(shapes_t),
                                                 _ptr(level_start), _ptr(loc), _ptr(attn), b, nv, nh, d, nl, nq, npnt,
                                                 _ptr(g_loc), _ptr(g_attn), _stream()), 'mbv_ms_deform_attn_bwd_locattn')
        return
    _msda_backward_f64(lib, g_out, value, shapes_t, level_start, loc, attn, dims, host, g_value, g_loc, g_attn)


def _msda_backward_f64(lib, g_out, value, shapes_t, level_start, loc, attn, dims, host, g_value, g_loc, g_attn):
    b, nv, nh, d, nl, nq, npnt = dims
    check(lib.mbv_ms_deform_attn_bwd(_ptr(g_out), _ptr(value), _ptr(shapes_t), _ptr(level_start), _ptr(loc), _ptr(attn),
                                     b, nv, nh, d, nl, nq, npnt, host, _ptr(g_value), _ptr(g_loc), _ptr(g_attn), 3,
                                     _stream()), 'mbv_ms_deform_attn_bwd')


class _MSDAPrepare(torch.autograd.Function):

    @staticmethod
    def forward(ctx, off, logits, ref, shapes_host):
        lib = _lib.load()
        _need_gpu(off, logits, ref)
        if off.dtype != logits.dtype or off.dtype not in _ACT_DTYPES:
            raise MaskBevHipError('msda_prepare: offsets and logits must share one of f32, bf16, fp16')
        off, logits = off.contiguous(), logits.contiguous()
        ref = ref.to(torch.float32).contiguous()
        b, n, h, l, p, _ = off.shape
        host = (ctypes.c_int64 * (2 * l))(*[int(v) for hw in shapes_host for v in hw])
        loc = torch.empty((b, n, h, l, p, 2), dtype=torch.float32, device=off.device)
        attn = torch.empty((b, n, h, l, p), dtype=torch.float32, device=off.device)
        check(lib.mbv_msda_prepare_fwd(_ptr(off), _ptr(logits), _dt_flag(off.dtype), _ptr(ref), host,
                                       b, n, h, l, p, _ptr(loc), _ptr(attn), _stream()), 'mbv_msda_prepare_fwd')
        ctx.save_for_backward(attn)
        ctx.meta = (host, off.dtype, (b, n, h, l, p), logits.shape)
        return loc, attn

    @staticmethod
    def backward(ctx, g_loc, g_attn):
        lib = _lib.load()
        attn, = ctx.saved_tensors
        host, dt, (b, n, h, l, p), lshape = ctx.meta
        g_loc = g_loc.to(torch.float32).contiguous()
        g_attn = g_attn.to(torch.float32).contiguous()
        g_off = torch.empty((b, n, h, l, p, 2), dtype=dt, device=attn.device)
        g_logit = torch.empty(lshape, dtype=dt, device=attn.device)
        check(lib.mbv_msda_prepare_bwd(_ptr(g_loc), _ptr(g_attn), _ptr(attn), host, b, n, h, l, p,
                                       _dt_flag(dt), _ptr(g_off), _ptr(g_logit), _stream()),
              'mbv_msda_prepare_bwd')
        return g_off, g_logit, None, None


def msda_prepare_supported(num_levels: int, num_points: int) -> bool:
    return bool(_lib.load().mbv_msda_prepare_supported(num_levels, num_points))


def msda_prepare(offsets: torch.Tensor, logits: torch.Tensor, reference_points: torch.Tensor, spatial_shapes):
    host = tuple((int(h), int(w)) for h, w in spatial_shapes)
    return _MSDAPrepare.apply(offsets, logits, reference_points, host)


def ms_deform_attn(value: torch.Tensor, spatial_shapes, shapes_t: torch.Tensor, level_start: torch.Tensor,
                   sampling_locations: torch.Tensor, attention_weights: torch.Tensor) -> torch.Tensor:
    host = None if spatial_shapes is None else tuple((int(h), int(w)) for h, w in spatial_shapes)
    return _MSDeformAttn.apply(value.float(), shapes_t, level_start, sampling_locations.float(),
                               attention_weights.float(), host)


class PosGradShare:

    def __init__(self, layers: int):
        self.layers = int(layers)
        self.weights = [None] * self.layers
        self.sums = None
        self.written = set()

    def store(self, index: int, block: torch.Tensor, weight: torch.Tensor):
        b, n, w = block.shape
        if self.sums is None:
            self.sums = torch.empty((n, self.layers * w), dtype=block.dtype if block.dtype in _LO_DTYPES else torch.float32,
                                    device=block.device)
        torch.sum(block, 0, out=self.sums[:, index * w:(index + 1) * w])
        self.weights[index] = weight
        self.written.add(index)

    def finish(self) -> torch.Tensor:
        if len(self.written) != self.layers:
            raise MaskBevHipError(f'PosGradShare: {len(self.written)} of {self.layers} layers ran their backward')
        od = {} if self.sums.dtype == torch.float32 else dict(out_dtype=torch.float32)
        out = torch.mm(self.sums, torch.cat(self.weights, 0), **od)
        self.sums, self.weights, self.written = None, [None] * self.layers, set()
        return out


class _MSDAQuerySide(torch.autograd.Function):

    @staticmethod
    def forward(ctx, x, pos, ref, wv, bv, wo, bo, wa, ba, heads, levels, points, shapes_host, shapes_t, level_start,
                share=None, share_index=0, wcat=None):
        lib = _lib.load()
        ctx.share = (share, int(share_index))
        _need_gpu(x, pos, ref, wv, wo, wa)
        b, n, e = x.shape
        d = e // heads
        dt = torch.get_autocast_dtype('cuda') if torch.is_autocast_enabled('cuda') else x.dtype
        if dt not in _ACT_DTYPES:
            raise MaskBevHipError('msda_query_side supports f32, bf16 and fp16 compute')
        lo, la = heads * levels * points * 2, heads * levels * points
        with torch.autocast('cuda', enabled=False):
            qb = torch.empty(x.shape, dtype=dt, device=x.device)
            if wcat is None or wcat.dtype != dt or tuple(wcat.shape) != (e + lo + la, e):
                wcat = torch.cat([_compute_copy(wv, dt), _compute_copy(wo, dt), _compute_copy(wa, dt)], 0)
            wvc = wcat[:e]
            pos_rows = pos.numel() // e
            if (dt in _LO_DTYPES and x.dtype == torch.float32 and pos.dtype == torch.float32 and x.is_contiguous()
                    and pos.is_contiguous() and e % 4 == 0 and (b * n) % pos_rows == 0):
                xb = torch.empty(x.shape, dtype=dt, device=x.device)
                check(lib.mbv_msda_query_inputs(_ptr(x), _ptr(pos), b * n, pos_rows, e, _dt_flag(dt), _ptr(xb), _ptr(qb),
                                                _stream()), 'mbv_msda_query_inputs')
                bvf = bv.float().contiguous()
                lo_value = False
                if gemm16_policy() != 'none' and _gemm16_ok(xb.view(b * n, e), wvc) and bvf.data_ptr() % 16 == 0:
                    host_b = (ctypes.c_int64 * (2 * levels))(*[int(v) for hw in shapes_host for v in hw])
                    lo_value = bool(d == 32 and (e + lo + la) % 2 == 0
                                    and msda_value_packed_ok((b, n, heads, d, levels, n, points), host_b))
                    value = gemm16_nt(xb.view(b * n, e), wvc, bvf,
                                      out_dtype=None if lo_value else torch.float32).view(b, n, e)
                else:
                    value = torch.addmm(bvf, xb.view(b * n, e), wvc.t(), out_dtype=torch.float32).view(b, n, e)
            else:
                xb = x.to(dt)
                torch.add(x, pos, out=qb)
                if dt == torch.float32:
                    value = mm32_nt(xb.reshape(b * n, e), wvc, bv.contiguous()).view(b, n, e)
                else:
                    value = torch.nn.functional.linear(xb, wvc, _compute_copy(bv, dt)).float().contiguous()
            ol = mm32_nt(qb.view(b * n, e), wcat[e:]) if dt == torch.float32 else torch.mm(qb.view(b * n, e), wcat[e:].t())
        host = (ctypes.c_int64 * (2 * levels))(*[int(v) for hw in shapes_host for v in hw])
        ref32 = ref.to(torch.float32).contiguous()
        loc = torch.empty((b, n, heads, levels, points, 2), dtype=torch.float32, device=x.device)
        attn = torch.empty((b, n, heads, levels, points), dtype=torch.float32, device=x.device)
        esz = ol.element_size()
        bo32, ba32 = bo.float().contiguous(), ba.float().contiguous()
        check(lib.mbv_msda_prepare_fwd_ld(_ptr(ol), lo + la, ctypes.c_void_p(ol.data_ptr() + lo * esz), lo + la,
                                          _ptr(bo32), _ptr(ba32), _dt_flag(dt),
                                          _ptr(ref32), host, b, n, heads, levels, points, _ptr(loc), _ptr(attn), _stream()),
              'mbv_msda_prepare_fwd_ld')
        del ol
        out = torch.empty((b, n, e), dtype=torch.float32, device=x.device)
        check(lib.mbv_ms_deform_attn_fwd_v(_ptr(value), _dt_flag(value.dtype), _ptr(shapes_t), _ptr(level_start), _ptr(loc),
                                           _ptr(attn), b, n, heads, d, levels, n, points, _ptr(out), _stream()),
              'mbv_ms_deform_attn_fwd_v')
        ctx.save_for_backward(xb, qb, value, loc, attn, shapes_t, level_start, wcat)
        ctx.params = (wv, bv, wo, bo, wa, ba)
        ctx.meta = (heads, levels, points, host, tuple(shapes_host), dt, x.dtype, pos.dtype, tuple(pos.shape))
        return out

    @staticmethod
    def backward(ctx, g_out):
        lib = _lib.load()
        xb, qb, value, loc, attn, shapes_t, level_start, wcat = ctx.saved_tensors
        wv, bv, wo, bo, wa, ba = ctx.params
        heads, levels, points, host, shapes_host, dt, x_dtype, pos_dtype, pos_shape = ctx.meta
        b, n, e = xb.shape
        d = e // heads
        lo, la = heads * levels * points * 2, heads * levels * points
        width = e + lo + la
        t = b * n
        dev = xb.device
        g_out = g_out.to(torch.float32).contiguous()
        g_loc = torch.empty_like(loc)
        g_attn = torch.empty_like(attn)
        host_b = (ctypes.c_int64 * (2 * levels))(*[int(v) for hw in shapes_host for v in hw])
        g = torch.empty((t, width), dtype=dt, device=dev)
        dims = (b, n, heads, d, levels, n, points)
        packed = ((dt in _LO_DTYPES or (dt == torch.float32 and switches.get('msda_packed_f32'))) and width % 2 == 0
                  and msda_value_packed_ok(dims, host_b))
        if value.dtype in _LO_DTYPES and not packed:
            raise MaskBevHipError('MSDA backward: the forward kept a 16-bit value map, which only the packed value gradient '
                                  'reads, and that path is unavailable now (switch changed between forward and backward?)')
        if packed:
            _msda_backward(lib, g_out, value, shapes_t, level_start, loc, attn, dims, host_b, None, g_loc, g_attn,
                           packed_out=(g, width))
        else:
            g_value = torch.empty_like(value)
            _msda_backward(lib, g_out, value, shapes_t, level_start, loc, attn, dims, host_b, g_value, g_loc, g_attn)
            g[:, :e].copy_(g_value.view(t, e))
        esz = g.element_size()
        check(lib.mbv_msda_prepare_bwd_ld(_ptr(g_loc), _ptr(g_attn), _ptr(attn), host, b, n, heads, levels, points,
                                          _dt_flag(dt), ctypes.c_void_p(g.data_ptr() + e * esz), width,
                                          ctypes.c_void_p(g.data_ptr() + (e + lo) * esz), width, _stream()),
              'mbv_msda_prepare_bwd_ld')
        od = {} if dt == torch.float32 else dict(out_dtype=torch.float32)
        gx = gpos = None
        if ctx.needs_input_grad[0]:
            gx = (mm32_nn(g, wcat) if dt == torch.float32 else torch.mm(g, wcat, **od)).view(b, n, e).to(x_dtype)
        if ctx.needs_input_grad[1]:
            share, share_index = ctx.share
            if share is not None:
                share.store(share_index, g.view(b, n, width)[:, :, e:], wcat[e:])
                gpos = share.finish().view(1, n, e) if share_index == 0 else None
            else:
                gq_sum = g.view(b, n, width)[:, :, e:].sum(0) if dt in _LO_DTYPES else g.view(b, n, width)[:, :, e:].sum(0, dtype=torch.float32)
                gpos = torch.mm(gq_sum, wcat[e:], **od).view(1, n, e)
            if gpos is not None:
                if tuple(pos_shape) != (1, n, e):
                    gpos = gpos.sum_to_size(pos_shape) if len(pos_shape) == 3 else gpos.reshape(pos_shape)
                gpos = gpos.to(pos_dtype)
        x2, q2 = xb.view(t, e), qb.view(t, e)
        cols = ((0, e, x2), (e, e + lo, q2), (e + lo, width, q2))
        grads = [None] * 6
        bias_tmp = None
        arena_bias = [bool(ctx.needs_input_grad[4 + 2 * j] and getattr(bia, '_mbv_arena', False) and bia.grad is not None
                           and bia.grad.dtype == torch.float32 and bia.grad.is_contiguous())
                      for j, bia in enumerate((bv, bo, ba))]
        deferred = [False, False, False]
        for j, (c0, c1) in enumerate(((0, e), (e, e + lo), (e + lo, width))):
            if arena_bias[j]:
                deferred[j] = _defer_colsum(g, (bv, bo, ba)[j].grad, t, c1 - c0, width, offset=c0)
        if any(ctx.needs_input_grad[4 + 2 * j] and not deferred[j] for j in range(3)):
            bias_tmp = torch.zeros(width, dtype=torch.float32, device=dev)
            colsum_accum(g, bias_tmp)
        dst, src = [], []
        for j, ((c0, c1, inp), w, bia) in enumerate(zip(cols, (wv, wo, wa), (bv, bo, ba))):
            gj = g[:, c0:c1]
            if ctx.needs_input_grad[3 + 2 * j]:
                if getattr(w, '_mbv_arena', False) and w.grad is not None and w.grad.dtype == torch.float32:
                    _wgrad_into(w.grad, gj, inp, persistent=True)
                    _fire_grad_hooks(w)
                else:
                    acc = torch.zeros(w.shape, dtype=torch.float32, device=dev)
                    _wgrad_into(acc, gj, inp)
                    grads[2 * j] = acc.to(w.dtype)
            if ctx.needs_input_grad[4 + 2 * j]:
                if deferred[j]:
                    _fire_grad_hooks(bia)
                elif getattr(bia, '_mbv_arena', False) and bia.grad is not None and bia.grad.dtype == torch.float32:
                    dst.append(bia.grad)
                    src.append(bias_tmp[c0:c1])
                else:
                    grads[2 * j + 1] = bias_tmp[c0:c1].to(bia.dtype)
        if dst:
            torch._foreach_add_(dst, src)
            for j, bia in enumerate((bv, bo, ba)):
                if not deferred[j]:
                    _fire_grad_hooks(bia)
        return (gx, gpos, None) + tuple(grads) + (None,) * 9


@torch.no_grad()
def msda_weight_stacks(attns, dtype) -> Optional[List[torch.Tensor]]:
    if not attns or not attns[0].value_proj.weight.is_cuda:
        return None
    dev = attns[0].value_proj.weight.device
    src, dst, nb, outs, keep = [], [], [], [], []
    for a in attns:
        parts = [_compute_copy(m.weight, dtype) for m in (a.value_proj, a.sampling_offsets, a.attention_weights)]
        keep.append(parts)
        if any(not p.is_contiguous() or p.dtype != dtype for p in parts):
            return None
        rows, e = sum(int(p.shape[0]) for p in parts), int(parts[0].shape[1])
        out = torch.empty((rows, e), dtype=dtype, device=dev)
        r0 = 0
        for p in parts:
            src.append(p.data_ptr())
            dst.append(out[r0:r0 + p.shape[0]].data_ptr())
            nb.append(p.numel() * p.element_size())
            r0 += int(p.shape[0])
        outs.append(out)
    k = len(src)
    check(_lib.load().mbv_copy_group((ctypes.c_void_p * k)(*src), (ctypes.c_void_p * k)(*dst), (ctypes.c_int64 * k)(*nb), k,
                                     _stream()), 'mbv_copy_group')
    del keep
    return outs


def msda_query_side(x, pos, ref, value_proj, sampling_offsets, attention_weights, heads, levels, points, spatial_shapes,
                    shapes_t, level_start, pos_share=None, pos_share_index=0, wcat=None):
    host = tuple((int(h), int(w)) for h, w in spatial_shapes)
    return _MSDAQuerySide.apply(x, pos, ref, value_proj.weight, value_proj.bias, sampling_offsets.weight,
                                sampling_offsets.bias, attention_weights.weight, attention_weights.bias, heads, levels,
                                points, host, shapes_t, level_start, pos_share, pos_share_index, wcat)


__all__ = [_n for _n in list(globals()) if not _n.startswith('__')]
```

### mask_bev_amd/switches.py

```python
from __future__ import annotations

import contextlib
import os
from typing import Any, Dict

_DEFAULTS: Dict[str, Any] = {
    'decoder_fused': 'auto',
    'deferred_heads': True,
    'shared_kv': True,
    'early_targets': True,
    'wgrad_group': True,
    'tn_group': '1',
    'nn_colsum_defer': True,
    'gemm16': 'auto',
    'tn_max_in': 1536,
    'k17_fused_min': 4096,
    'gemm32s': True,
    'amax_hints': True,
    'amax_verify': False,
    'ffn32': True,
    'k4_split': True,
    'k6_split': True,
    'msda_packed_f32': True,
    'ln_bound_hints': True,
    'conv3x3_k20': True,
    'tn32_group': True,
    'gemm32s_min': 1024,
    'pfn_stream_stats': True,
    'pfn_one_call': True,
    'groupnorm': True,
    'merge_ln': True,
    'tuned_gemms': True,
}

_values: Dict[str, Any] = dict(_DEFAULTS)


def get(name: str) -> Any:
    return _values[name]


def defaults() -> Dict[str, Any]:
    return dict(_DEFAULTS)


def _coerce(name: str, value: Any) -> Any:
    d = _DEFAULTS[name]
    if isinstance(d, bool):
        if isinstance(value, str):
            return value not in ('0', '', 'false', 'False')
        return bool(value)
    if isinstance(d, int):
        return int(value)
    return str(value)


def set_value(name: str, value: Any) -> None:
    if name not in _DEFAULTS:
        raise KeyError(f'unknown switch {name!r}')
    _values[name] = _coerce(name, value)


@contextlib.contextmanager
def override(**kw: Any):
    old = {k: _values[k] for k in kw}
    try:
        for k, v in kw.items():
            set_value(k, v)
        yield
    finally:
        _values.update(old)


def load_from_env(prefix: str = 'MBV_') -> Dict[str, Any]:
    taken = {}
    for k in _DEFAULTS:
        e = os.environ.get(prefix + k.upper())
        if e is not None:
            set_value(k, e)
            taken[k] = _values[k]
    return taken


def patch(monkeypatch, **kw: Any) -> None:
    for k, v in kw.items():
        if k not in _DEFAULTS:
            raise KeyError(f'unknown switch {k!r}')
        monkeypatch.setitem(_values, k, _coerce(k, v))
```

### mask_bev_amd/workmodel.py

```python
from __future__ import annotations

from typing import Callable, Dict, Tuple

HBM_PEAK_GBS = 8000.0
MFMA_BF16_TFLOPS = 2500.0
MFMA_F32_TFLOPS = 157.3

Work = Tuple[str, str, float, float]


def _i(x) -> int:
    return int(getattr(x, 'value', x) or 0)


def _window_attn(a, bwd: bool) -> Work:
    if bwd:
        bf16, b, h, w, c, heads, ws = (_i(a[i]) for i in (6, 7, 8, 9, 10, 11, 12))
    else:
        bf16, b, h, w, c, heads, ws = (_i(a[i]) for i in (3, 4, 5, 6, 7, 8, 9))
    es = 2 if bf16 else 4
    t = b * h * w
    nwin = b * ((h + ws - 1) // ws) * ((w + ws - 1) // ws)
    n, d = ws * ws, c // max(1, heads)
    if bwd:
        return ('k_window_attn_bwd', 'hbm', t * c * es * (3 + 1 + 1 + 3), 10.0 * nwin * heads * n * n * d)
    return ('k_window_attn_fwd', 'hbm', t * c * es * (3 + 1), 4.0 * nwin * heads * n * n * d)


def _window_attn_split(a, bwd: bool) -> Work:
    if bwd:
        b, h, w, c, heads, ws = (_i(a[i]) for i in (6, 7, 8, 9, 10, 11))
    else:
        b, h, w, c, heads, ws = (_i(a[i]) for i in (3, 4, 5, 6, 7, 8))
    t = b * h * w
    nwin = b * ((h + ws - 1) // ws) * ((w + ws - 1) // ws)
    n, d = ws * ws, c // max(1, heads)
    if bwd:
        return ('k_window_attn_bwd', 'hbm', t * c * 4 * (3 + 1 + 1 + 3), 10.0 * nwin * heads * n * n * d)
    return ('k_window_attn_fwd', 'hbm', t * c * 4 * (3 + 1), 4.0 * nwin * heads * n * n * d)


def _msda(a, bwd: bool) -> Work:
    o = 1 if bwd else 0
    b, nv, heads, d, levels, nq, pts = (_i(a[i + o]) for i in (5, 6, 7, 8, 9, 10, 11))
    samples = b * nq * heads * levels * pts
    vmap, qmap = b * nv * heads * d * 4.0, b * nq * heads * d * 4.0
    if bwd:
        part = _i(a[17])
        if part == 1:
            return ('k_msda_bwd_value', 'hbm', vmap + qmap + samples * 12.0, 0.0)
        if part == 2:
            return ('k_msda_bwd_locattn', 'hbm', vmap + qmap + 2 * samples * 12.0, 0.0)
        return ('k_msda_bwd', 'hbm', 2 * vmap + qmap + 2 * samples * 12.0, 0.0)
    return ('k_msda_fwd_v4', 'hbm', vmap + qmap + samples * 12.0, 0.0)


def _pfn_forward(a) -> Work:
    k, v, n = _i(a[5]), _i(a[6]), _i(a[14])
    c, by, fl = _i(a[1]), 0.0, 0.0
    for l in range(n):
        u = int(a[13][l])
        last = l == n - 1
        by += (k * (c + u) + k * u + k * u + (0 if last else k * u) + 6.0 * v * u) * 4.0
        fl += 2.0 * k * c * u + (4.0 * v * c * u if l else 0.0)
        c = u
    return ('k_pfn_forward', 'hbm', by, fl)


def _msda_typed(a, bwd: bool) -> Work:
    o = 1 if bwd else 0
    ves = 4.0 if _i(a[1 + o]) == 0 else 2.0
    b, nv, heads, d, levels, nq, pts = (_i(a[i + o]) for i in (6, 7, 8, 9, 10, 11, 12))
    samples = b * nq * heads * levels * pts
    vmap, qmap = b * nv * heads * d * ves, b * nq * heads * d * 4.0
    if bwd:
        return ('k_msda_bwd_locattn', 'hbm', vmap + qmap + 2 * samples * 12.0, 0.0)
    return ('k_msda_fwd_v4', 'hbm', vmap + qmap + samples * 12.0, 0.0)


def _msda_value_packed(a) -> Work:
    b, nv, heads, d, levels, nq, pts = (_i(a[i]) for i in (3, 4, 5, 6, 7, 8, 9))
    samples = b * nq * heads * levels * pts
    out_es = 4.0 if _i(a[12]) == 0 else 2.0
    return ('k_msda_bwd_value_fx', 'hbm', b * nv * heads * d * out_es + b * nq * heads * d * 4.0 + samples * 12.0, 0.0)


def _rowchain(a) -> Work:
    stages, n, rows, wdt = a[0], _i(a[1]), _i(a[2]), _i(a[5])
    wes = 4.0 if wdt == 0 else 2.0
    by = fl = 0.0
    for i in range(n):
        st = stages[i]
        es = 4.0 if (st.flags & 3) == 0 else 2.0
        if st.op == 0:
            by += rows * st.n * (es if st.p0 else 0.0)
        elif st.op == 1:
            by += rows * st.n * es * (2.0 if st.flags & 4 else 1.0)
        elif st.op == 2:
            by += st.n * st.k * wes
            fl += 2.0 * rows * st.n * st.k
        elif st.op in (3, 4):
            by += rows * 8.0
        elif st.op == 7:
            by += 2.0 * st.n * st.k * wes + rows * st.k * 4.0 * (2.0 if st.flags & 16 else 1.0)
            fl += 4.0 * rows * st.n * st.k
        elif st.op == 9:
            by += rows * st.n * 4.0 * st.k
    return ('k_rowchain', 'hbm', by, fl)


def _rowchain_split(a) -> Work:
    name, bound, by, fl = _rowchain(a)
    stages, n, rows, split = a[0], _i(a[1]), _i(a[2]), _i(a[6])
    for i in range(n):
        st = stages[i]
        if st.op == 1 and (st.flags & 64):
            by += rows * st.n * 4.0 * (split - 1)
    return (name, bound, by, fl)


def _point_rows(rows: int, pts: int) -> float:
    from . import _lib
    _, n_sets = _lib.WORK_HINT.get('point_sample', (rows, rows))
    return min(rows, n_sets) * pts * 8.0 + rows * pts * 4.0


def _point_sample(a, kernel: str, bytes_per_pixel: float) -> Work:
    from . import _lib
    rows, pts, h, w = _i(a[4]), _i(a[5]), _i(a[6]), _i(a[7])
    n_src, _ = _lib.WORK_HINT.get('point_sample', (rows, rows))
    return (kernel, 'hbm', min(rows, n_src) * h * w * bytes_per_pixel + _point_rows(rows, pts), 0.0)


def _attn(a, bwd: bool, ld: bool) -> Work:
    if bwd:
        i0 = 8 if ld else 7
    else:
        i0 = 5 if ld else 4
    bf16, b, q, k, heads, d = (_i(a[i0 + j]) for j in range(6))
    es = 2 if bf16 else 4
    e = heads * d
    if bwd:
        return ('k_attn_bwd', 'hbm', b * (2 * q * e * es + 2 * k * e * es + q * k) + b * (q * e * 4 + 2 * k * e * 4),
                10.0 * b * heads * q * k * d)
    return ('k_attn_fwd_split', 'hbm', b * (q * e * es * 2 + 2 * k * e * es + q * k), 4.0 * b * heads * q * k * d)


def _attn_split(a, bwd: bool) -> Work:
    i0 = 8 if bwd else 5
    b, q, k, heads, d = (_i(a[i0 + j]) for j in range(5))
    e = heads * d
    if bwd:
        return ('k_attn_bwd', 'hbm', b * (2 * q * e * 4 + 2 * k * e * 4 + q * k) + b * (q * e * 4 + 2 * k * e * 4),
                10.0 * b * heads * q * k * d)
    return ('k_attn_fwd_split', 'hbm', b * (q * e * 4 * 2 + 2 * k * e * 4 + q * k), 4.0 * b * heads * q * k * d)


def _gemm16(a, layout: str) -> Work:
    if layout == 'nt':
        m, n, k, f32 = _i(a[5]), _i(a[6]), _i(a[7]), _i(a[12])
# ... 74 lines not shown
    return ('k_add_ln_fwd', 'hbm', n * (4.0 + _sz(a[9])), 0.0)


def _colsum_group(a) -> Work:
    n = _i(a[6])
    dt, rows, cols = a[1], a[2], a[3]
    by = sum(rows[j] * cols[j] * (4.0 if dt[j] == 0 else 2.0) + cols[j] * 8.0 for j in range(n))
    return ('k_colsum_group', 'hbm', by, 0.0)


def _pfn(a, kernel: str, rows_per_unit: float, pillars_per_unit: float, iv: int, iu: int) -> Work:
    from . import _lib
    k = _lib.WORK_HINT.get('pfn_rows', 0)
    v, u = _i(a[iv]), _i(a[iu])
    return (kernel, 'hbm', (rows_per_unit * k + pillars_per_unit * v) * u * 4.0, 0.0)


def _decorate(a) -> Work:
    from . import _lib
    k, dim = _lib.WORK_HINT.get('pfn_rows', 0), _i(a[1])
    return ('k_pfn_decorate', 'hbm', k * (dim * 4.0 + (dim + 7) * 4.0 + 8.0 + 4.0), 0.0)


def _voxelize(a) -> Work:
    n, dim, batch, gx, gy = _i(a[2]), _i(a[1]), _i(a[4]), _i(a[14]), _i(a[15])
    pillars = _i(a[20])
    return ('k_voxelize (22 launches)', 'hbm', n * (dim * 4.0 + 16.0 + 8.0) + pillars * (16.0 + 4.0 + 128.0 + 4.0)
            + batch * gx * gy * 4.0, 0.0)


def _msda_prepare(a, bwd: bool) -> Work:
    if bwd:
        b, nq, heads, levels, pts, lo = (_i(a[i]) for i in (4, 5, 6, 7, 8, 9))
        per = b * nq * heads * levels * pts
        return ('k_msda_prepare_bwd', 'hbm', per * (12.0 + 4.0) + per * 3.0 * (2.0 if lo else 4.0), 0.0)
    lo, b, nq, heads, levels, pts = (_i(a[i]) for i in (2, 5, 6, 7, 8, 9))
    per = b * nq * heads * levels * pts
    return ('k_msda_prepare_fwd', 'hbm', per * 3.0 * (2.0 if lo else 4.0) + per * 12.0, 0.0)


def _copy_group(a, kernel: str, es_index: int) -> Work:
    rows, cols, n = a[2], a[3], _i(a[6] if kernel == 'k_fragment_group' else a[4])
    es = 2.0 if kernel == 'k_fragment_group' else float(_i(a[es_index]))
    return (kernel, 'hbm', sum(2.0 * rows[j] * cols[j] * es for j in range(n)), 0.0)


def gemm_work(m: int, n: int, k: int, batch: int, es_in: float, es_out: float, extra_bytes: float = 0.0) -> Tuple[float, float]:
    return batch * ((m * k + k * n) * es_in + m * n * es_out) + extra_bytes, 2.0 * batch * m * n * k


MODELS: Dict[str, Callable[[tuple], Work]] = {
    'mbv_voxelize': _voxelize,
    'mbv_pfn_decorate': lambda a: _decorate(a),
    'mbv_pfn_stats': lambda a: _pfn(a, 'k_pfn_stats', 2.0 if a[1] else 1.0, 3.0 if a[1] else 1.0, 5, 6),
    'mbv_pfn_apply_max': lambda a: _pfn(a, 'k_pfn_apply_max', 2.0 if a[9] else 1.0, 3.0 if a[10] else 2.0, 6, 7),
    'mbv_pfn_bwd_route': lambda a: _pfn(a, 'k_pfn_bwd_route', 3.0 if _i(a[7]) else 2.0, 4.0, 12, 13),
    'mbv_pfn_bwd_bn': lambda a: _pfn(a, 'k_pfn_bwd_bn', 3.0, 4.0, 12, 13),
    'mbv_msda_prepare_fwd': lambda a: _msda_prepare(a, False),
    'mbv_msda_prepare_fwd_ld': lambda a: _msda_prepare((None, None) + tuple(a[6:7]) + (None, None) + tuple(a[9:14]), False),
    'mbv_msda_prepare_bwd': lambda a: _msda_prepare(a, True),
    'mbv_msda_prepare_bwd_ld': lambda a: _msda_prepare(a, True),
    'mbv_msda_query_inputs': lambda a: ('k_msda_query_inputs', 'hbm',
                                        _i(a[2]) * _i(a[4]) * (4.0 + 2.0 + 2.0) + _i(a[3]) * _i(a[4]) * 4.0, 0.0),
    'mbv_fragment_group': lambda a: _copy_group(a, 'k_fragment_group', 0),
    'mbv_transpose_group': lambda a: _copy_group(a, 'k_transpose_group', 5),
    'mbv_hungarian_padded': lambda a: ('k_hungarian', 'hbm', _i(a[1]) * _i(a[2]) * _i(a[3]) * 4.0 + _i(a[1]) * _i(a[2]) * 4.0, 0.0),
    'mbv_uniform_points': lambda a: ('k_uniform_points', 'hbm', _i(a[1]) * _i(a[2]) * 8.0, 0.0),
    'mbv_pack_binary_masks': lambda a: ('k_pack_binary', 'hbm', _i(a[1]) * _i(a[2]) * _i(a[3]) * (4.0 + 1.0 / 8.0), 0.0),
    'mbv_attn_mask_from_logits': lambda a: ('k_attn_mask', 'hbm',
                                            _i(a[2]) * (min(_i(a[3]) * _i(a[4]), 4 * _i(a[5]) * _i(a[6]))
                                                        * (2.0 if _i(a[1]) else 4.0) + _i(a[5]) * _i(a[6])), 0.0),
    'mbv_gemm16_nt_acc': lambda a: ('k_gemm16<NT,acc>', 'mfma',
                                    _i(a[11]) * ((_i(a[3]) + _i(a[4])) * _i(a[5]) * 2.0 + 2.0 * _i(a[3]) * _i(a[4]) * 4.0),
                                    2.0 * _i(a[11]) * _i(a[3]) * _i(a[4]) * _i(a[5])),
    'mbv_window_attn_fwd': lambda a: _window_attn(a, False),
    'mbv_window_attn_bwd': lambda a: _window_attn(a, True),
    'mbv_window_attn_split_fwd': lambda a: _window_attn_split(a, False),
    'mbv_window_attn_split_bwd': lambda a: _window_attn_split(a, True),
    'mbv_ms_deform_attn_fwd': lambda a: _msda(a, False),
    'mbv_ms_deform_attn_bwd': lambda a: _msda(a, True),
    'mbv_ms_deform_attn_fwd_v': lambda a: _msda_typed(a, False),
    'mbv_ms_deform_attn_bwd_locattn': lambda a: _msda_typed(a, True),
    'mbv_ms_deform_attn_bwd_value_packed': _msda_value_packed,
    'mbv_rowchain_run': _rowchain,
    'mbv_rowchain_run_split': _rowchain_split,
    'mbv_attn_fwd': lambda a: _attn(a, False, False),
    'mbv_attn_fwd_ld': lambda a: _attn(a, False, True),
    'mbv_attn_bwd': lambda a: _attn(a, True, False),
    'mbv_attn_bwd_ld': lambda a: _attn(a, True, True),
    'mbv_attn_split_fwd_ld': lambda a: _attn_split(a, False),
    'mbv_attn_split_bwd_ld': lambda a: _attn_split(a, True),
    'mbv_gemm16_nt': lambda a: _gemm16(a, 'nt'),
    'mbv_gemm16_nn': lambda a: _gemm16(a, 'nn'),
    'mbv_gemm16_nn_parts': lambda a: _gemm16(a, 'nn_parts'),
    'mbv_gemm16_tn': lambda a: _gemm16(a, 'tn'),
    'mbv_add_layernorm_fwd': lambda a: _add_ln(a, False),
    'mbv_add_layernorm_fwd2': lambda a: _add_ln_fwd2(a),
    'mbv_pfn_forward': lambda a: _pfn_forward(a),
    'mbv_skinny_gemm_f32_addrows': lambda a: ('k_skinny_f32', 'hbm',
                                              (_i(a[3]) * (_i(a[4]) + _i(a[5])) + _i(a[4]) * _i(a[5])) * 4.0,
                                              2.0 * _i(a[3]) * _i(a[4]) * _i(a[5])),
    'mbv_skinny_gemm_f32': lambda a: ('k_skinny_f32', 'hbm',
                                      (_i(a[3]) * (_i(a[4]) + _i(a[5])) + _i(a[4]) * _i(a[5])) * 4.0,
                                      2.0 * _i(a[3]) * _i(a[4]) * _i(a[5])),
    'mbv_copy_group': lambda a: ('k_copy_group', 'hbm', 2.0 * sum(int(a[2][j]) for j in range(_i(a[3]))), 0.0),
    'mbv_transposed_batch_sum_accum': lambda a: ('k_transposed_batch_sum', 'hbm',
                                                 (_i(a[1]) + 2.0) * _i(a[2]) * _i(a[3]) * 4.0, 0.0),
    'mbv_add_layernorm_bwd': lambda a: _add_ln(a, True),
    'mbv_add_layernorm_bwd2': lambda a: _add_ln_bwd2(a),
    'mbv_add_layernorm_bwd3': lambda a: _add_ln_bwd2(a),
    'mbv_sample_select_uncertain': lambda a: ('k_sample_select', 'hbm',
                                              _i(a[4]) * (_i(a[7]) * _i(a[8]) * 4.0 + _i(a[6]) * 8.0), 0.0),
    'mbv_hungarian': lambda a: ('k_hungarian', 'hbm', _i(a[1]) * _i(a[2]) * _i(a[3]) * 4.0 + _i(a[1]) * _i(a[2]) * 4.0, 0.0),
    'mbv_mask_logits_fwd': lambda a: ('k_mask_logits', 'hbm',
                                      _i(a[3]) * (_i(a[4]) * _i(a[5]) + _i(a[5]) * _i(a[6])) * (2 if _i(a[2]) else 4)
                                      + _i(a[3]) * _i(a[4]) * _i(a[6]) * (4 if (_i(a[8]) or not _i(a[2])) else 2),
                                      2.0 * _i(a[3]) * _i(a[4]) * _i(a[5]) * _i(a[6])),
    'mbv_point_sample_fwd': lambda a: _point_sample(a, 'k_point_sample_fwd_lds', 4.0),
    'mbv_point_sample_bwd': lambda a: ('k_point_sample_bwd_lds', 'hbm',
                                       _i(a[8]) * _i(a[6]) * _i(a[7]) * 4.0 + _point_rows(_i(a[4]), _i(a[5])), 0.0),
    'mbv_point_sample_bwd_stack': lambda a: ('k_point_sample_bwd_lds', 'hbm',
                                             _i(a[4]) * _i(a[6]) * _i(a[7]) * (4.0 if _i(a[12]) == 0 else 2.0)
                                             + _point_rows(_i(a[4]), _i(a[5])), 0.0),
    'mbv_point_sample_packed_fwd': lambda a: _point_sample(a, 'k_point_sample_packed', 1.0 / 8.0),
    'mbv_mask_loss_rows_fwd': lambda a: ('k_mask_loss_rows_fwd', 'hbm', _i(a[2]) * _i(a[3]) * 8.0, 0.0),
    'mbv_mask_loss_rows_bwd': lambda a: ('k_mask_loss_rows_bwd', 'hbm', _i(a[3]) * _i(a[4]) * 12.0, 0.0),
    'mbv_mask_loss_rows_bwd_coef': lambda a: ('k_mask_loss_rows_bwd', 'hbm', _i(a[7]) * _i(a[9]) * 12.0, 0.0),
    'mbv_act_bwd_colsum': lambda a: ('k_act_bwd_colsum', 'hbm', _i(a[4]) * _i(a[5]) * 3.0 * (2 if _i(a[2]) else 4), 0.0),
    'mbv_wgrad_small_f32': lambda a: ('k_wgrad_small', 'mfma_f32',
                                      (_i(a[2]) * (_i(a[3]) + _i(a[4])) + 2 * _i(a[3]) * _i(a[4])) * 4.0,
                                      2.0 * _i(a[2]) * _i(a[3]) * _i(a[4])),
    'mbv_wgrad_small_f32_group': lambda a: _wgrad_group(a),
    'mbv_colsum_accum_group': lambda a: _colsum_group(a),
    'mbv_gemm16_tn_group': lambda a: _tn_group(a),
    'mbv_gemm32s_nt': lambda a: ('k_gemm32s<NT>', 'mfma', ((_i(a[5]) * _i(a[7]) + _i(a[6]) * _i(a[7])) * 4.0
                                                          + _i(a[5]) * _i(a[6]) * 4.0 * (2 if a[4] is not None and _i(a[4]) else 1))
                                 * max(1, _i(a[15])), 2.0 * _i(a[5]) * _i(a[6]) * _i(a[7]) * max(1, _i(a[15]))),
    'mbv_gemm32s_nn': lambda a: ('k_gemm32s<NN>', 'mfma', (_i(a[3]) * _i(a[4]) + _i(a[4]) * _i(a[5]) + _i(a[3]) * _i(a[5])) * 4.0
                                 * max(1, _i(a[12])), 2.0 * _i(a[3]) * _i(a[4]) * _i(a[5]) * max(1, _i(a[12]))),
    'mbv_gemm32s_nn_act': lambda a: ('k_gemm32s<NN,dact>', 'mfma',
                                     (_i(a[6]) * _i(a[7]) + _i(a[7]) * _i(a[8]) + 2 * _i(a[6]) * _i(a[8])) * 4.0,
                                     2.0 * _i(a[6]) * _i(a[7]) * _i(a[8])),
    'mbv_gemm32s_tn_acc': lambda a: ('k_gemm32s<TN>', 'mfma', (_i(a[3]) * _i(a[4]) + _i(a[3]) * _i(a[5])) * 4.0
                                     + _i(a[4]) * _i(a[5]) * 4.0 * 2, 2.0 * _i(a[3]) * _i(a[4]) * _i(a[5])),
    'mbv_patch_embed32_fwd': lambda a: ('k_gemm32s<NT,patch>', 'mfma',
                                        (_i(a[4]) * _i(a[5]) * _i(a[6]) * _i(a[7]) + _i(a[4]) * _i(a[6]) * _i(a[7]) // 16 * _i(a[8])) * 4.0,
                                        2.0 * _i(a[4]) * (_i(a[6]) // 4) * (_i(a[7]) // 4) * _i(a[8]) * 16 * _i(a[5])),
    'mbv_patch_embed32_bwd_image': lambda a: ('k_gemm32s<NN,patch>', 'mfma',
                                              (_i(a[3]) * _i(a[4]) * _i(a[5]) * _i(a[6]) + _i(a[3]) * _i(a[5]) * _i(a[6]) // 16 * _i(a[7])) * 4.0,
                                              2.0 * _i(a[3]) * (_i(a[5]) // 4) * (_i(a[6]) // 4) * _i(a[7]) * 16 * _i(a[4])),
    'mbv_patch_embed32_bwd_weight': lambda a: ('k_gemm32s<TN,patch>', 'mfma',
                                               (_i(a[3]) * _i(a[4]) * _i(a[5]) * _i(a[6]) + _i(a[3]) * _i(a[5]) * _i(a[6]) // 16 * _i(a[7])) * 4.0,
                                               2.0 * _i(a[3]) * (_i(a[5]) // 4) * (_i(a[6]) // 4) * _i(a[7]) * 16 * _i(a[4])),
    'mbv_conv3x3_gemm32s': lambda a: ('k_gemm32s<NT,conv3x3>', 'mfma',
                                      (_i(a[3]) * (_i(a[4]) + 2) * (_i(a[5]) + 2) * (_i(a[6]) + _i(a[7])) + 9 * _i(a[6]) * _i(a[7])) * 4.0,
                                      2.0 * _i(a[3]) * (_i(a[4]) + 2) * (_i(a[5]) + 2) * _i(a[7]) * 9 * _i(a[6])),
    'mbv_conv3x3_gemm16': lambda a: ('k_gemm16<NT,conv3x3>', 'mfma',
                                     (_i(a[3]) * (_i(a[4]) + 2) * (_i(a[5]) + 2) * (_i(a[6]) + _i(a[7])) + 9 * _i(a[6]) * _i(a[7])) * 2.0,
                                     2.0 * _i(a[3]) * (_i(a[4]) + 2) * (_i(a[5]) + 2) * _i(a[7]) * 9 * _i(a[6])),
    'mbv_conv_pad_rows': lambda a: ('k_conv_pad_rows', 'hbm', 2.0 * _i(a[2]) * _i(a[3]) * _i(a[4]) * _i(a[5]) * _i(a[6]), 0.0),
    'mbv_conv_unpad_rows': lambda a: ('k_conv_pad_rows', 'hbm', 2.0 * _i(a[2]) * _i(a[3]) * _i(a[4]) * _i(a[5]) * _i(a[6]), 0.0),
    'mbv_gemm32s_tn_group': lambda a: ('k_gemm32s_tn_group', 'mfma',
                                       sum((int(a[3][i]) * (int(a[4][i]) + int(a[5][i])) + 2 * int(a[4][i]) * int(a[5][i])) * 4.0
                                           for i in range(_i(a[10]))),
                                       sum(2.0 * int(a[3][i]) * int(a[4][i]) * int(a[5][i]) for i in range(_i(a[10])))),
    'mbv_f32_absmax_group': lambda a: ('k_absmax_group', 'hbm',
# ... 121 lines not shown
```

Measured before the change: 180.3 scans/s.

## Fuse MSDA offset/logit prepare into sampling kernels for forward and backward

Adds fused kernels that compute softmax of attention logits and sampling locations from raw projection outputs inside the deformable-attention sampling kernel, and the matching backward that writes offset and logit gradients directly into the packed gradient buffer. This removes separate prepare launches and the round-trip of intermediate grad_loc/grad_attn tensors through memory. The forward can also emit output in the low-precision dtype to skip a cast. The cost is more register pressure per thread and a narrower supported configuration (head_dim 32, 4 points), with fallback to the old path otherwise.

```diff
diff --git a/include/maskbev_hip.h b/include/maskbev_hip.h
--- a/include/maskbev_hip.h
+++ b/include/maskbev_hip.h
@@ -124,6 +124,20 @@
                                    int32_t num_query, int32_t num_points, float* grad_loc, float* grad_attn, void* stream);
 
 int mbv_ms_deform_attn_bwd_split(int32_t head_dim, int32_t num_levels, const int64_t* spatial_shapes_host);
+
+int mbv_msda_fused_supported(int32_t head_dim, int32_t num_levels, int32_t num_points);
+int mbv_ms_deform_attn_fwd_prep(const void* value, int32_t value_dtype, const int64_t* spatial_shapes, const int64_t* level_start,
+                                const void* offsets, int64_t ld_offsets, const void* logits, int64_t ld_logits,
+                                const float* bias_offsets, const float* bias_logits, int32_t dtype, const float* ref_points,
+                                const int64_t* spatial_shapes_host, int32_t batch, int32_t num_value, int32_t num_heads,
+                                int32_t head_dim, int32_t num_levels, int32_t num_query, int32_t num_points, float* loc,
+                                float* attn, void* out, int32_t out_dtype, void* stream);
+int mbv_ms_deform_attn_bwd_locattn_prep(const float* grad_out, const void* value, int32_t value_dtype,
+                                        const int64_t* spatial_shapes, const int64_t* level_start, const float* sampling_loc,
+                                        const float* attn_weight, const int64_t* spatial_shapes_host, int32_t batch,
+                                        int32_t num_value, int32_t num_heads, int32_t head_dim, int32_t num_levels,
+                                        int32_t num_query, int32_t num_points, int32_t out_dtype, void* grad_offsets,
+                                        int64_t ld_offsets, void* grad_logits, int64_t ld_logits, void* stream);
 
 int mbv_ms_deform_attn_bwd_value_packed_supported(int32_t head_dim, int32_t num_levels, int32_t num_points,
                                                   int32_t num_query, const int64_t* spatial_shapes_host);
diff --git a/mask_bev_amd/_lib.py b/mask_bev_amd/_lib.py
--- a/mask_bev_amd/_lib.py
+++ b/mask_bev_amd/_lib.py
@@ -57,6 +57,11 @@
     'mbv_ms_deform_attn_fwd_v': (ctypes.c_int, [_P, _I, _P, _P, _P, _P, _I, _I, _I, _I, _I, _I, _I, _P, _P]),
     'mbv_ms_deform_attn_bwd_locattn': (ctypes.c_int, [_P, _P, _I, _P, _P, _P, _P, _I, _I, _I, _I, _I, _I, _I, _P, _P, _P]),
     'mbv_ms_deform_attn_bwd_split': (ctypes.c_int, [_I, _I, _P]),
+    'mbv_msda_fused_supported': (ctypes.c_int, [_I, _I, _I]),
+    'mbv_ms_deform_attn_fwd_prep': (ctypes.c_int, [_P, _I, _P, _P, _P, _L, _P, _L, _P, _P, _I, _P, _P, _I, _I, _I, _I, _I, _I, _I,
+                                                   _P, _P, _P, _I, _P]),
+    'mbv_ms_deform_attn_bwd_locattn_prep': (ctypes.c_int, [_P, _P, _I, _P, _P, _P, _P, _P, _I, _I, _I, _I, _I, _I, _I, _I, _P, _L,
+                                                           _P, _L, _P]),
     'mbv_ms_deform_attn_bwd_value_packed_supported': (ctypes.c_int, [_I, _I, _I, _I, _P]),
     'mbv_ms_deform_attn_bwd_value_packed_workspace_bytes': (c_size_t, [_I, _I, _I, _I]),
     'mbv_ms_deform_attn_bwd_value_packed': (ctypes.c_int, [_P, _P, _P, _I, _I, _I, _I, _I, _I, _I, _P, _P, _I, _L, _P, c_size_t, _P]),
diff --git a/mask_bev_amd/csrc/msda.hip b/mask_bev_amd/csrc/msda.hip
--- a/mask_bev_amd/csrc/msda.hip
+++ b/mask_bev_amd/csrc/msda.hip
@@ -1,5 +1,6 @@
 
 #include "common.hpp"
+#include "msda_prepare.hpp"
 
 namespace {
 
@@ -577,6 +578,29 @@
 }
 
 template <int VK>
+__device__ __forceinline__ void msda_level_gather_p4(const void* __restrict__ value, int64_t vl, int h, int w, int stride_pix,
+                                                     const float4& xy0, const float4& xy1, const float4& aw, float4& acc) {
+  Taps4 tp[4];
+  taps_clamped(xy0.x, xy0.y, aw.x, h, w, stride_pix, tp[0]);
+  taps_clamped(xy0.z, xy0.w, aw.y, h, w, stride_pix, tp[1]);
+  taps_clamped(xy1.x, xy1.y, aw.z, h, w, stride_pix, tp[2]);
+  taps_clamped(xy1.z, xy1.w, aw.w, h, w, stride_pix, tp[3]);
+  float4 x[16];
+#pragma unroll
+  for (int p = 0; p < 4; ++p)
+#pragma unroll
+    for (int j = 0; j < 4; ++j) x[p * 4 + j] = value4<VK>(value, vl + tp[p].off[j]);
+#pragma unroll
+  for (int p = 0; p < 4; ++p)
+#pragma unroll
+    for (int j = 0; j < 4; ++j) {
+      const float wj = tp[p].wgt[j];
+      acc.x += wj * x[p * 4 + j].x; acc.y += wj * x[p * 4 + j].y;
+      acc.z += wj * x[p * 4 + j].z; acc.w += wj * x[p * 4 + j].w;
+    }
+}
+
+template <int VK>
 __global__ void __launch_bounds__(256) k_msda_fwd_p4(const void* __restrict__ value, const int64_t* __restrict__ shapes,
                                                      const int64_t* __restrict__ level_start,
                                                      const float* __restrict__ loc, const float* __restrict__ attn,
@@ -600,26 +624,70 @@
     const float4 xy0 = *reinterpret_cast<const float4*>(loc + (lw_base + l * 4) * 2);
     const float4 xy1 = *reinterpret_cast<const float4*>(loc + (lw_base + l * 4) * 2 + 4);
     const float4 aw = *reinterpret_cast<const float4*>(attn + lw_base + l * 4);
-    Taps4 tp[4];
-    taps_clamped(xy0.x, xy0.y, aw.x, h, w, stride_pix, tp[0]);
-    taps_clamped(xy0.z, xy0.w, aw.y, h, w, stride_pix, tp[1]);
-    taps_clamped(xy1.x, xy1.y, aw.z, h, w, stride_pix, tp[2]);
-    taps_clamped(xy1.z, xy1.w, aw.w, h, w, stride_pix, tp[3]);
-    float4 x[16];
-#pragma unroll
-    for (int p = 0; p < 4; ++p)
-#pragma unroll
-      for (int j = 0; j < 4; ++j) x[p * 4 + j] = value4<VK>(value, vl + tp[p].off[j]);
-#pragma unroll
-    for (int p = 0; p < 4; ++p)
-#pragma unroll
-      for (int j = 0; j < 4; ++j) {
-        const float wj = tp[p].wgt[j];
-        acc.x += wj * x[p * 4 + j].x; acc.y += wj * x[p * 4 + j].y;
-        acc.z += wj * x[p * 4 + j].z; acc.w += wj * x[p * 4 + j].w;
-      }
+    msda_level_gather_p4<VK>(value, vl, h, w, stride_pix, xy0, xy1, aw, acc);
   }
   *reinterpret_cast<float4*>(out + ((t * heads + hd) * dim + d4 * 4)) = acc;
+}
+
+template <int VK, typename T, typename OT>
+__global__ void __launch_bounds__(256) k_msda_fwd_p4_prep(const void* __restrict__ value, const int64_t* __restrict__ shapes,
+                                                          const int64_t* __restrict__ level_start,
+                                                          const T* __restrict__ off, long ld_off, const T* __restrict__ logit,
+                                                          long ld_logit, const float* __restrict__ b_off,
+                                                          const float* __restrict__ b_logit, const float* __restrict__ ref,
+                                                          Norm nrm, int64_t total8, int num_value, int heads, int levels,
+                                                          int num_query, float* __restrict__ loc, float* __restrict__ attn,
+                                                          OT* __restrict__ out) {
+  constexpr int dim = 32;
+  const int64_t idx = xcd_block(blockIdx.x, gridDim.x) * blockDim.x + threadIdx.x;
+  if (idx >= total8) return;
+  const int d4 = (int)(idx & 7);
+  int64_t t = idx >> 3;
+  const int hd = (int)(t % heads);
+  t /= heads;
+  const int b = (int)(t / num_query);
+  const int n = (int)(t - (int64_t)b * num_query);
+  const int lp = levels * 4;
+  const int stride_pix = heads * dim;
+  const int64_t vb = (int64_t)b * num_value * stride_pix + hd * dim + d4 * 4;
+  const int64_t lw_base = (t * heads + hd) * lp;
+  const T* o = off + t * ld_off + (long)hd * lp * 2;
+  const T* a = logit + t * ld_logit + (long)hd * lp;
+  float v[kMaxLP], xy[2 * kMaxLP];
+#pragma unroll
+  for (int k = 0; k < kMaxLP; k += 4) {
+    const int kk = k < lp ? k : 0;
+    ld4<T>(a + kk, v + k);
+    ld4<T>(o + 2 * kk, xy + 2 * k);
+    ld4<T>(o + 2 * kk + 4, xy + 2 * k + 4);
+    if (k >= lp) v[k] = v[k + 1] = v[k + 2] = v[k + 3] = -INFINITY;
+  }
+  msda_prepare_row_fwd<T>(v, xy, b_logit ? b_logit + hd * lp : nullptr, b_off ? b_off + hd * lp * 2 : nullptr, ref[2 * n],
+                          ref[2 * n + 1], nrm, lp, 4);
+#pragma unroll
+  for (int r = 0; r < kMaxLP / 8; ++r) {
+    float keep_a = 0.f, keep_x = 0.f, keep_y = 0.f;
+#pragma unroll
+    for (int j = 0; j < 8; ++j)
+      if (j == d4) { keep_a = v[8 * r + j]; keep_x = xy[2 * (8 * r + j)]; keep_y = xy[2 * (8 * r + j) + 1]; }
+    if (8 * r + d4 < lp) {
+      attn[lw_base + 8 * r + d4] = keep_a;
+      *reinterpret_cast<float2*>(loc + (lw_base + 8 * r + d4) * 2) = make_float2(keep_x, keep_y);
+    }
+  }
+  float4 acc = make_float4(0.f, 0.f, 0.f, 0.f);
+#pragma unroll
+  for (int l = 0; l < kMaxLP / 4; ++l) {
+    if (l < levels) {
+      const int h = (int)shapes[l * 2], w = (int)shapes[l * 2 + 1];
+      const int64_t vl = vb + level_start[l] * stride_pix;
+      msda_level_gather_p4<VK>(value, vl, h, w, stride_pix, make_float4(xy[8 * l], xy[8 * l + 1], xy[8 * l + 2], xy[8 * l + 3]),
+                               make_float4(xy[8 * l + 4], xy[8 * l + 5], xy[8 * l + 6], xy[8 * l + 7]),
+                               make_float4(v[4 * l], v[4 * l + 1], v[4 * l + 2], v[4 * l + 3]), acc);
+    }
+  }
+  const float a4[4] = {acc.x, acc.y, acc.z, acc.w};
+  st4<OT>(out + ((t * heads + hd) * dim + d4 * 4), a4);
 }
 
 __global__ void __launch_bounds__(256) k_msda_bwd_relayout(const float* __restrict__ grad_out,
@@ -797,6 +865,41 @@
 }
 
 template <int VK>
+__device__ __forceinline__ void msda_level_grads_p4(const void* __restrict__ value, int64_t vl, int h, int w, int stride_pix,
+                                                    const float4& go, const float4& xy0, const float4& xy1,
+                                                    const float (&awp)[4], float (&gw4)[4], float (&gx4)[4],
+                                                    float (&gy4)[4]) {
+  TapsG tp[4];
+  taps_grad(xy0.x, xy0.y, h, w, stride_pix, tp[0]);
+  taps_grad(xy0.z, xy0.w, h, w, stride_pix, tp[1]);
+  taps_grad(xy1.x, xy1.y, h, w, stride_pix, tp[2]);
+  taps_grad(xy1.z, xy1.w, h, w, stride_pix, tp[3]);
+  float4 x[16];
+#pragma unroll
+  for (int p = 0; p < 4; ++p)
+#pragma unroll
+    for (int j = 0; j < 4; ++j) x[p * 4 + j] = value4<VK>(value, vl + tp[p].off[j]);
+#pragma unroll
+  for (int p = 0; p < 4; ++p) {
+    float s4[4];
+#pragma unroll
+    for (int j = 0; j < 4; ++j) {
+      const float4 v = x[p * 4 + j];
+      s4[j] = tp[p].ok[j] * (go.x * v.x + go.y * v.y + go.z * v.z + go.w * v.w);
+    }
+    const float lh = tp[p].lh, lw = tp[p].lw, uh = 1.f - lh, uw = 1.f - lw;
+    float g_w = uh * uw * s4[0] + uh * lw * s4[1] + lh * uw * s4[2] + lh * lw * s4[3];
+    const float gh = -uw * s4[0] - lw * s4[1] + uw * s4[2] + lw * s4[3];
+    const float gw = -uh * s4[0] + uh * s4[1] - lh * s4[2] + lh * s4[3];
+    float g_x = (float)w * gw * awp[p] * tp[p].in;
+    float g_y = (float)h * gh * awp[p] * tp[p].in;
+    gw4[p] = group8_allsum(g_w * tp[p].in);
+    gx4[p] = group8_allsum(g_x);
+    gy4[p] = group8_allsum(g_y);
+  }
+}
+
+template <int VK>
 __global__ void __launch_bounds__(256) k_msda_bwd_locattn_p4(const float* __restrict__ grad_out,
                                                              const void* __restrict__ value,
                                                              const int64_t* __restrict__ shapes,
@@ -826,33 +929,11 @@
     const float4 xy1 = *reinterpret_cast<const float4*>(loc + (lw_base + l * 4) * 2 + 4);
     const float4 aw4 = *reinterpret_cast<const float4*>(attn + lw_base + l * 4);
     const float awp[4] = {aw4.x, aw4.y, aw4.z, aw4.w};
-    TapsG tp[4];
-    taps_grad(xy0.x, xy0.y, h, w, stride_pix, tp[0]);
-    taps_grad(xy0.z, xy0.w, h, w, stride_pix, tp[1]);
-    taps_grad(xy1.x, xy1.y, h, w, stride_pix, tp[2]);
-    taps_grad(xy1.z, xy1.w, h, w, stride_pix, tp[3]);
-    float4 x[16];
-#pragma unroll
-    for (int p = 0; p < 4; ++p)
-#pragma unroll
-      for (int j = 0; j < 4; ++j) x[p * 4 + j] = value4<VK>(value, vl + tp[p].off[j]);
+    float gw4[4], gx4[4], gy4[4];
+    msda_level_grads_p4<VK>(value, vl, h, w, stride_pix, go, xy0, xy1, awp, gw4, gx4, gy4);
 #pragma unroll
     for (int p = 0; p < 4; ++p) {
-      float s4[4];
-#pragma unroll
-      for (int j = 0; j < 4; ++j) {
-        const float4 v = x[p * 4 + j];
-        s4[j] = tp[p].ok[j] * (go.x * v.x + go.y * v.y + go.z * v.z + go.w * v.w);
-      }
-      const float lh = tp[p].lh, lw = tp[p].lw, uh = 1.f - lh, uw = 1.f - lw;
-      float g_w = uh * uw * s4[0] + uh * lw * s4[1] + lh * uw * s4[2] + lh * lw * s4[3];
-      const float gh = -uw * s4[0] - lw * s4[1] + uw * s4[2] + lw * s4[3];
-      const float gw = -uh * s4[0] + uh * s4[1] - lh * s4[2] + lh * s4[3];
-      float g_x = (float)w * gw * awp[p] * tp[p].in;
-      float g_y = (float)h * gh * awp[p] * tp[p].in;
-      g_w = group8_allsum(g_w * tp[p].in);
-      g_x = group8_allsum(g_x);
-      g_y = group8_allsum(g_y);
+      const float g_w = gw4[p], g_x = gx4[p], g_y = gy4[p];
       const int sidx8 = l * points + p;
       if ((sidx8 & 7) == d4) { keep_w = g_w; keep_x = g_x; keep_y = g_y; }
       if ((sidx8 & 7) == 7 || (l == levels - 1 && p == points - 1)) {
@@ -862,6 +943,82 @@
           *reinterpret_cast<float2*>(grad_loc + (lw_base + first + d4) * 2) = make_float2(keep_x, keep_y);
         }
       }
+    }
+  }
+}
+
+template <typename T>
+__device__ __forceinline__ void st2(T* p, float a, float b);
+template <>
+__device__ __forceinline__ void st2<float>(float* p, float a, float b) { *reinterpret_cast<float2*>(p) = make_float2(a, b); }
+template <>
+__device__ __forceinline__ void st2<unsigned short>(unsigned short* p, float a, float b) {
+  *reinterpret_cast<unsigned*>(p) = pack_bf16x2(a, b);
+}
+template <>
+__device__ __forceinline__ void st2<_Float16>(_Float16* p, float a, float b) {
+  typedef _Float16 h2 __attribute__((ext_vector_type(2)));
+  h2 q;
+  q[0] = (_Float16)a; q[1] = (_Float16)b;
+  *reinterpret_cast<h2*>(p) = q;
+}
+
+template <int VK, typename T>
+__global__ void __launch_bounds__(256) k_msda_bwd_locattn_p4_prep(const float* __restrict__ grad_out,
+                                                                  const void* __restrict__ value,
+                                                                  const int64_t* __restrict__ shapes,
+                                                                  const int64_t* __restrict__ level_start,
+                                                                  const float* __restrict__ loc, const float* __restrict__ attn,
+                                                                  Norm nrm, int64_t total8, int num_value, int heads,
+                                                                  int levels, int num_query, T* __restrict__ g_off, long ld_off,
+                                                                  T* __restrict__ g_logit, long ld_logit) {
+  constexpr int dim = 32, points = 4;
+  const int stride_pix = heads * dim;
+  const int64_t idx = xcd_block(blockIdx.x, gridDim.x) * blockDim.x + threadIdx.x;
+  const bool live = idx < total8;
+  const int64_t sidx = live ? idx : total8 - 1;
+  const int d4 = (int)(sidx & 7);
+  int64_t t = sidx >> 3;
+  const int hd = (int)(t % heads);
+  t /= heads;
+  const int b = (int)(t / num_query);
+  const int lp = levels * points;
+  const int64_t vb = (int64_t)b * num_value * stride_pix + hd * dim + d4 * 4;
+  const int64_t lw_base = (t * heads + hd) * lp;
+  const float4 go = *reinterpret_cast<const float4*>(grad_out + (t * heads + hd) * dim + d4 * 4);
+  float keep_w[2] = {0.f, 0.f}, keep_x[2] = {0.f, 0.f}, keep_y[2] = {0.f, 0.f}, keep_a[2] = {0.f, 0.f};
+  float dot = 0.f;
+#pragma unroll
+  for (int l = 0; l < kMaxLP / 4; ++l) {
+    if (l < levels) {
+      const int h = (int)shapes[l * 2], w = (int)shapes[l * 2 + 1];
+      const int64_t vl = vb + level_start[l] * stride_pix;
+      const float4 xy0 = *reinterpret_cast<const float4*>(loc + (lw_base + l * 4) * 2);
+      const float4 xy1 = *reinterpret_cast<const float4*>(loc + (lw_base + l * 4) * 2 + 4);
+      const float4 aw4 = *reinterpret_cast<const float4*>(attn + lw_base + l * 4);
+      const float awp[4] = {aw4.x, aw4.y, aw4.z, aw4.w};
+      float gw4[4], gx4[4], gy4[4];
+      msda_level_grads_p4<VK>(value, vl, h, w, stride_pix, go, xy0, xy1, awp, gw4, gx4, gy4);
+#pragma unroll
+      for (int p = 0; p < 4; ++p) {
+        const int s = l * 4 + p;
+        dot = msda_prepare_dot_step(dot, awp[p], gw4[p]);
+        if ((s & 7) == d4) { keep_w[s >> 3] = gw4[p]; keep_x[s >> 3] = gx4[p]; keep_y[s >> 3] = gy4[p]; keep_a[s >> 3] = awp[p]; }
+      }
+    } else {
+#pragma unroll
+      for (int p = 0; p < 4; ++p) dot = msda_prepare_dot_step(dot, 0.f, 0.f);
+    }
+  }
+  T* gof = g_off + t * ld_off + (long)hd * lp * 2;
+  T* glg = g_logit + t * ld_logit + (long)hd * lp;
+#pragma unroll
+  for (int r = 0; r < kMaxLP / 8; ++r) {
+    const int s = 8 * r + d4;
+    if (live && s < lp) {
+      const float nw = d4 & 4 ? nrm.w[2 * r + 1] : nrm.w[2 * r], nh = d4 & 4 ? nrm.h[2 * r + 1] : nrm.h[2 * r];
+      stf<T>(glg + s, msda_prepare_logit_bwd(keep_a[r], keep_w[r], dot));
+      st2<T>(gof + 2 * s, msda_prepare_offset_bwd<T>(keep_x[r], nw), msda_prepare_offset_bwd<T>(keep_y[r], nh));
     }
   }
 }
@@ -979,6 +1136,114 @@
   return MBV_OK;
 }
 
+extern "C" int mbv_msda_fused_supported(int32_t head_dim, int32_t num_levels, int32_t num_points) {
+  return head_dim == 32 && num_points == 4 && num_levels >= 1 && num_levels * num_points <= kMaxLP;
+}
+
+namespace {
+bool msda_host_levels_ok(const int64_t* shapes_host, int levels, int num_value) {
+  int64_t n = 0;
+  for (int l = 0; l < levels; ++l) n += shapes_host[2 * l] * shapes_host[2 * l + 1];
+  return n == num_value;
+}
+}
+
+extern "C" int mbv_ms_deform_attn_fwd_prep(const void* value, int32_t value_dtype, const int64_t* spatial_shapes,
+                                           const int64_t* level_start, const void* offsets, int64_t ld_offsets,
+                                           const void* logits, int64_t ld_logits, const float* bias_offsets,
+                                           const float* bias_logits, int32_t dtype, const float* ref_points,
+                                           const int64_t* spatial_shapes_host, int32_t batch, int32_t num_value,
+                                           int32_t num_heads, int32_t head_dim, int32_t num_levels, int32_t num_query,
+                                           int32_t num_points, float* loc, float* attn, void* out, int32_t out_dtype,
+                                           void* stream_) {
+  hipStream_t stream = reinterpret_cast<hipStream_t>(stream_);
+  if (batch <= 0 || num_value <= 0 || num_heads <= 0 || num_levels <= 0 || num_query <= 0 || num_points <= 0)
+    return MBV_ERR_BAD_ARG;
+  if (dtype != MBV_DT_F32 && dtype != MBV_DT_BF16 && dtype != MBV_DT_F16) return MBV_ERR_BAD_ARG;
+  if ((value_dtype != MBV_DT_F32 && value_dtype != dtype) || (out_dtype != MBV_DT_F32 && out_dtype != dtype))
+    return MBV_ERR_BAD_ARG;
+  if (!mbv_msda_fused_supported(head_dim, num_levels, num_points)) return MBV_ERR_UNSUPPORTED;
+  if (!value || !spatial_shapes || !level_start || !offsets || !logits || !ref_points || !loc || !attn || !out)
+    return MBV_ERR_BAD_ARG;
+  const int64_t lp = (int64_t)num_levels * num_points;
+  if (ld_offsets < num_heads * lp * 2 || ld_logits < num_heads * lp) return MBV_ERR_BAD_ARG;
+  const size_t es = dtype == MBV_DT_F32 ? 4 : 2;
+  if (((reinterpret_cast<size_t>(offsets) | reinterpret_cast<size_t>(logits)) & (4 * es - 1)) != 0 || (ld_offsets % 4) != 0 ||
+      (ld_logits % 4) != 0)
+    return MBV_ERR_BAD_ARG;
+  if ((reinterpret_cast<size_t>(value) & (value_dtype == MBV_DT_F32 ? 15 : 7)) ||
+      (reinterpret_cast<size_t>(out) & (out_dtype == MBV_DT_F32 ? 15 : 7)) ||
+      ((reinterpret_cast<size_t>(loc) | reinterpret_cast<size_t>(attn)) & 15))
+    return MBV_ERR_UNSUPPORTED;
+  Norm n;
+  if (!fill_norm(spatial_shapes_host, num_levels, n) || !msda_host_levels_ok(spatial_shapes_host, num_levels, num_value))
+    return MBV_ERR_BAD_ARG;
+  const int64_t total8 = (int64_t)batch * num_query * num_heads * 8;
+  const dim3 grid((unsigned)((total8 + 255) / 256)), block(256);
+#define MBV_FWD_PREP(VK, T, OT)                                                                                          \
+  hipLaunchKernelGGL((k_msda_fwd_p4_prep<VK, T, OT>), grid, block, 0, stream, value, spatial_shapes, level_start,        \
+                     reinterpret_cast<const T*>(offsets), (long)ld_offsets, reinterpret_cast<const T*>(logits),          \
+                     (long)ld_logits, bias_offsets, bias_logits, ref_points, n, total8, num_value, num_heads, num_levels, \
+                     num_query, loc, attn, reinterpret_cast<OT*>(out))
+#define MBV_FWD_PREP_LO(DT, T)                                                                                           \
+  if (value_dtype == MBV_DT_F32) {                                                                                       \
+    if (out_dtype == MBV_DT_F32) MBV_FWD_PREP(MBV_DT_F32, T, float); else MBV_FWD_PREP(MBV_DT_F32, T, T);                \
+  } else {                                                                                                               \
+    if (out_dtype == MBV_DT_F32) MBV_FWD_PREP(DT, T, float); else MBV_FWD_PREP(DT, T, T);                                \
+  }
+  if (dtype == MBV_DT_F32) { MBV_FWD_PREP(MBV_DT_F32, float, float); }
+  else if (dtype == MBV_DT_BF16) { MBV_FWD_PREP_LO(MBV_DT_BF16, unsigned short) }
+  else { MBV_FWD_PREP_LO(MBV_DT_F16, _Float16) }
+#undef MBV_FWD_PREP_LO
+#undef MBV_FWD_PREP
+  MBV_CHECK_LAUNCH();
+  return MBV_OK;
+}
+
+extern "C" int mbv_ms_deform_attn_bwd_locattn_prep(const float* grad_out, const void* value, int32_t value_dtype,
+                                                   const int64_t* spatial_shapes, const int64_t* level_start,
+                                                   const float* sampling_loc, const float* attn_weight,
+                                                   const int64_t* spatial_shapes_host, int32_t batch, int32_t num_value,
+                                                   int32_t num_heads, int32_t head_dim, int32_t num_levels,
+                                                   int32_t num_query, int32_t num_points, int32_t out_dtype,
+                                                   void* grad_offsets, int64_t ld_offsets, void* grad_logits,
+                                                   int64_t ld_logits, void* stream_) {
+  hipStream_t stream = reinterpret_cast<hipStream_t>(stream_);
+  if (batch <= 0 || num_value <= 0 || num_heads <= 0 || num_levels <= 0 || num_query <= 0 || num_points <= 0)
+    return MBV_ERR_BAD_ARG;
+  if (out_dtype != MBV_DT_F32 && out_dtype != MBV_DT_BF16 && out_dtype != MBV_DT_F16) return MBV_ERR_BAD_ARG;
+  if (value_dtype != MBV_DT_F32 && value_dtype != out_dtype) return MBV_ERR_BAD_ARG;
+  if (!mbv_msda_fused_supported(head_dim, num_levels, num_points)) return MBV_ERR_UNSUPPORTED;
+  if (!grad_out || !value || !spatial_shapes || !level_start || !sampling_loc || !attn_weight || !grad_offsets || !grad_logits)
+    return MBV_ERR_BAD_ARG;
+  const int64_t lp = (int64_t)num_levels * num_points;
+  const size_t es = out_dtype == MBV_DT_F32 ? 4 : 2;
+  if (ld_offsets < num_heads * lp * 2 || ld_logits < num_heads * lp || (ld_offsets % 2) != 0 ||
+      (reinterpret_cast<size_t>(grad_offsets) & (2 * es - 1)) != 0 || (reinterpret_cast<size_t>(grad_logits) & (es - 1)) != 0)
+    return MBV_ERR_BAD_ARG;
+  if ((reinterpret_cast<size_t>(grad_out) & 15) || (reinterpret_cast<size_t>(value) & (value_dtype == MBV_DT_F32 ? 15 : 7)) ||
+      ((reinterpret_cast<size_t>(sampling_loc) | reinterpret_cast<size_t>(attn_weight)) & 15))
+    return MBV_ERR_UNSUPPORTED;
+  Norm n;
+  if (!fill_norm(spatial_shapes_host, num_levels, n) || !msda_host_levels_ok(spatial_shapes_host, num_levels, num_value))
+    return MBV_ERR_BAD_ARG;
+  const int64_t total8 = (int64_t)batch * num_query * num_heads * 8;
+  const dim3 grid((unsigned)((total8 + 255) / 256)), block(256);
+#define MBV_LOCATTN_PREP(VK, T)                                                                                          \
+  hipLaunchKernelGGL((k_msda_bwd_locattn_p4_prep<VK, T>), grid, block, 0, stream, grad_out, value, spatial_shapes,       \
+                     level_start, sampling_loc, attn_weight, n, total8, num_value, num_heads, num_levels, num_query,     \
+                     reinterpret_cast<T*>(grad_offsets), (long)ld_offsets, reinterpret_cast<T*>(grad_logits), (long)ld_logits)
+  if (out_dtype == MBV_DT_F32) { MBV_LOCATTN_PREP(MBV_DT_F32, float); }
+  else if (out_dtype == MBV_DT_BF16) {
+    if (value_dtype == MBV_DT_F32) MBV_LOCATTN_PREP(MBV_DT_F32, unsigned short); else MBV_LOCATTN_PREP(MBV_DT_BF16, unsigned short);
+  } else {
+    if (value_dtype == MBV_DT_F32) MBV_LOCATTN_PREP(MBV_DT_F32, _Float16); else MBV_LOCATTN_PREP(MBV_DT_F16, _Float16);
+  }
+#undef MBV_LOCATTN_PREP
+  MBV_CHECK_LAUNCH();
+  return MBV_OK;
+}
+
 extern "C" int mbv_ms_deform_attn_bwd_split(int32_t head_dim, int32_t num_levels, const int64_t* spatial_shapes_host) {
   if (!spatial_shapes_host || head_dim != 32 || num_levels <= 0 || num_levels > 8) return 0;
   for (int l = 0; l < num_levels; ++l) {
diff --git a/mask_bev_amd/csrc/msda_prepare.hip b/mask_bev_amd/csrc/msda_prepare.hip
--- a/mask_bev_amd/csrc/msda_prepare.hip
+++ b/mask_bev_amd/csrc/msda_prepare.hip
@@ -1,76 +1,6 @@
-#include "common.hpp"
+#include "msda_prepare.hpp"
 
 namespace {
-
-constexpr int kMaxLP = 16;
-
-template <typename T>
-__device__ __forceinline__ float ldf(const T* p);
-template <>
-__device__ __forceinline__ float ldf<float>(const float* p) { return *p; }
-template <>
-__device__ __forceinline__ float ldf<unsigned short>(const unsigned short* p) { return __uint_as_float((unsigned)*p << 16); }
-template <typename T>
-__device__ __forceinline__ void stf(T* p, float v);
-template <>
-__device__ __forceinline__ void stf<float>(float* p, float v) { *p = v; }
-template <>
-__device__ __forceinline__ void stf<unsigned short>(unsigned short* p, float v) { *p = f32_to_bf16_rne(v); }
-template <typename T>
-__device__ __forceinline__ float round_like(float v);
-template <>
-__device__ __forceinline__ float round_like<float>(float v) { return v; }
-template <>
-__device__ __forceinline__ float round_like<unsigned short>(float v) { return __uint_as_float((unsigned)f32_to_bf16_rne(v) << 16); }
-
-template <typename T>
-__device__ __forceinline__ void ld4(const T* p, float* v);
-template <>
-__device__ __forceinline__ void ld4<float>(const float* p, float* v) {
-  const float4 q = *reinterpret_cast<const float4*>(p);
-  v[0] = q.x; v[1] = q.y; v[2] = q.z; v[3] = q.w;
-}
-template <>
-__device__ __forceinline__ void ld4<unsigned short>(const unsigned short* p, float* v) {
-  const uint2 u = *reinterpret_cast<const uint2*>(p);
-  v[0] = __uint_as_float(u.x << 16); v[1] = __uint_as_float(u.x & 0xffff0000u);
-  v[2] = __uint_as_float(u.y << 16); v[3] = __uint_as_float(u.y & 0xffff0000u);
-}
-template <typename T>
-__device__ __forceinline__ void st4(T* p, const float* v);
-template <>
-__device__ __forceinline__ void st4<float>(float* p, const float* v) {
-  *reinterpret_cast<float4*>(p) = make_float4(v[0], v[1], v[2], v[3]);
-}
-template <>
-__device__ __forceinline__ void st4<unsigned short>(unsigned short* p, const float* v) {
-  uint2 u;
-  u.x = pack_bf16x2(v[0], v[1]);
-  u.y = pack_bf16x2(v[2], v[3]);
-  *reinterpret_cast<uint2*>(p) = u;
-}
-
-template <>
-__device__ __forceinline__ float ldf<_Float16>(const _Float16* p) { return (float)*p; }
-template <>
-__device__ __forceinline__ void stf<_Float16>(_Float16* p, float v) { *p = (_Float16)v; }
-template <>
-__device__ __forceinline__ float round_like<_Float16>(float v) { return (float)(_Float16)v; }
-template <>
-__device__ __forceinline__ void ld4<_Float16>(const _Float16* p, float* v) {
-  typedef _Float16 h4 __attribute__((ext_vector_type(4)));
-  const h4 q = *reinterpret_cast<const h4*>(p);
-  v[0] = (float)q[0]; v[1] = (float)q[1]; v[2] = (float)q[2]; v[3] = (float)q[3];
-}
-template <>
-__device__ __forceinline__ void st4<_Float16>(_Float16* p, const float* v) {
-  typedef _Float16 h4 __attribute__((ext_vector_type(4)));
-  h4 q;
-  q[0] = (_Float16)v[0]; q[1] = (_Float16)v[1]; q[2] = (_Float16)v[2]; q[3] = (_Float16)v[3];
-  *reinterpret_cast<h4*>(p) = q;
-}
-
-struct Norm { float w[8], h[8]; };
 
 template <typename T>
 __global__ void __launch_bounds__(256) k_msda_prepare_fwd(const T* __restrict__ off, const T* __restrict__ logit,
@@ -90,56 +20,39 @@
   const T* a = logit + tok * ld_logit + (long)head * lp;
   const float* bo = b_off ? b_off + (long)head * lp * 2 : nullptr;
   const float* ba = b_logit ? b_logit + (long)head * lp : nullptr;
-  float v[kMaxLP];
-  float m = -INFINITY;
+  float v[kMaxLP], xy[2 * kMaxLP];
   const bool vec = (lp & 3) == 0;
   if (vec) {
 #pragma unroll
     for (int k = 0; k < kMaxLP; k += 4) {
-      if (k < lp) ld4<T>(a + k, v + k);
-      else v[k] = v[k + 1] = v[k + 2] = v[k + 3] = -INFINITY;
+      if (k < lp) {
+        ld4<T>(a + k, v + k);
+        ld4<T>(o + 2 * k, xy + 2 * k);
+        ld4<T>(o + 2 * k + 4, xy + 2 * k + 4);
+      } else {
+        v[k] = v[k + 1] = v[k + 2] = v[k + 3] = -INFINITY;
+#pragma unroll
+        for (int e = 0; e < 8; ++e) xy[2 * k + e] = 0.f;
+      }
     }
   } else {
 #pragma unroll
-    for (int k = 0; k < kMaxLP; ++k) v[k] = k < lp ? ldf<T>(a + k) : -INFINITY;
-  }
-  if (ba) {
-#pragma unroll
-    for (int k = 0; k < kMaxLP; ++k)
-      if (k < lp) v[k] += ba[k];
-  }
-#pragma unroll
-  for (int k = 0; k < kMaxLP; ++k) m = fmaxf(m, v[k]);
-  float s = 0.f;
-#pragma unroll
-  for (int k = 0; k < kMaxLP; ++k) {
-    v[k] = k < lp ? expf(v[k] - m) : 0.f;
-    s += v[k];
-  }
-  const float inv = 1.f / s;
+    for (int k = 0; k < kMaxLP; ++k) {
+      v[k] = k < lp ? ldf<T>(a + k) : -INFINITY;
+      xy[2 * k] = k < lp ? ldf<T>(o + 2 * k) : 0.f;
+      xy[2 * k + 1] = k < lp ? ldf<T>(o + 2 * k + 1) : 0.f;
+    }
+  }
+  msda_prepare_row_fwd<T>(v, xy, ba, bo, rx, ry, nrm, lp, points);
   float* lo = loc + i * lp * 2;
   float* ao = attn + i * lp;
   if (vec) {
 #pragma unroll
     for (int k = 0; k < kMaxLP; k += 4) {
       if (k < lp) {
-        const float w4[4] = {v[k] * inv, v[k + 1] * inv, v[k + 2] * inv, v[k + 3] * inv};
-        st4<float>(ao + k, w4);
-        float o8[8], r8[8];
-        ld4<T>(o + 2 * k, o8);
-        ld4<T>(o + 2 * k + 4, o8 + 4);
-        if (bo) {
-#pragma unroll
-          for (int e = 0; e < 8; ++e) o8[e] += bo[2 * k + e];
-        }
-#pragma unroll
-        for (int e = 0; e < 4; ++e) {
-          const int l = (k + e) / points;
-          r8[2 * e] = rx + round_like<T>(o8[2 * e] / nrm.w[l]);
-          r8[2 * e + 1] = ry + round_like<T>(o8[2 * e + 1] / nrm.h[l]);
-        }
-        st4<float>(lo + 2 * k, r8);
-        st4<float>(lo + 2 * k + 4, r8 + 4);
+        st4<float>(ao + k, v + k);
+        st4<float>(lo + 2 * k, xy + 2 * k);
+        st4<float>(lo + 2 * k + 4, xy + 2 * k + 4);
       }
     }
     return;
@@ -147,10 +60,9 @@
 #pragma unroll
   for (int k = 0; k < kMaxLP; ++k) {
     if (k < lp) {
-      const int l = k / points;
-      ao[k] = v[k] * inv;
-      lo[2 * k] = rx + round_like<T>((ldf<T>(o + 2 * k) + (bo ? bo[2 * k] : 0.f)) / nrm.w[l]);
-      lo[2 * k + 1] = ry + round_like<T>((ldf<T>(o + 2 * k + 1) + (bo ? bo[2 * k + 1] : 0.f)) / nrm.h[l]);
+      ao[k] = v[k];
+      lo[2 * k] = xy[2 * k];
+      lo[2 * k + 1] = xy[2 * k + 1];
     }
   }
 }
@@ -190,7 +102,7 @@
     }
   }
 #pragma unroll
-  for (int k = 0; k < kMaxLP; ++k) dot += a[k] * g[k];
+  for (int k = 0; k < kMaxLP; ++k) dot = msda_prepare_dot_step(dot, a[k], g[k]);
   const long bn = i / heads;
   const int hh = (int)(i - bn * heads);
   T* go = g_off + bn * ld_off + (long)hh * lp * 2;
@@ -199,8 +111,8 @@
 #pragma unroll
     for (int k = 0; k < kMaxLP; k += 4) {
       if (k < lp) {
-        const float q4[4] = {a[k] * (g[k] - dot), a[k + 1] * (g[k + 1] - dot), a[k + 2] * (g[k + 2] - dot),
-                             a[k + 3] * (g[k + 3] - dot)};
+        const float q4[4] = {msda_prepare_logit_bwd(a[k], g[k], dot), msda_prepare_logit_bwd(a[k + 1], g[k + 1], dot),
+                             msda_prepare_logit_bwd(a[k + 2], g[k + 2], dot), msda_prepare_logit_bwd(a[k + 3], g[k + 3], dot)};
         st4<T>(gq + k, q4);
         float l8[8], o8[8];
         ld4<float>(gl + 2 * k, l8);
@@ -208,8 +120,8 @@
 #pragma unroll
         for (int e = 0; e < 4; ++e) {
           const int l = (k + e) / points;
-          o8[2 * e] = round_like<T>(l8[2 * e]) / nrm.w[l];
-          o8[2 * e + 1] = round_like<T>(l8[2 * e + 1]) / nrm.h[l];
+          o8[2 * e] = msda_prepare_offset_bwd<T>(l8[2 * e], nrm.w[l]);
+          o8[2 * e + 1] = msda_prepare_offset_bwd<T>(l8[2 * e + 1], nrm.h[l]);
         }
         st4<T>(go + 2 * k, o8);
         st4<T>(go + 2 * k + 4, o8 + 4);
@@ -221,22 +133,11 @@
   for (int k = 0; k < kMaxLP; ++k) {
     if (k < lp) {
       const int l = k / points;
-      stf<T>(gq + k, a[k] * (g[k] - dot));
-      stf<T>(go + 2 * k, round_like<T>(gl[2 * k]) / nrm.w[l]);
-      stf<T>(go + 2 * k + 1, round_like<T>(gl[2 * k + 1]) / nrm.h[l]);
-    }
-  }
-}
-
-bool fill_norm(const int64_t* shapes_host, int levels, Norm& n) {
-  if (!shapes_host || levels < 1 || levels > 8) return false;
-  for (int l = 0; l < 8; ++l) { n.w[l] = 1.f; n.h[l] = 1.f; }
-  for (int l = 0; l < levels; ++l) {
-    const int64_t h = shapes_host[2 * l], w = shapes_host[2 * l + 1];
-    if (h <= 0 || w <= 0) return false;
-    n.h[l] = (float)h; n.w[l] = (float)w;
-  }
-  return true;
+      stf<T>(gq + k, msda_prepare_logit_bwd(a[k], g[k], dot));
+      stf<T>(go + 2 * k, msda_prepare_offset_bwd<T>(gl[2 * k], nrm.w[l]));
+      stf<T>(go + 2 * k + 1, msda_prepare_offset_bwd<T>(gl[2 * k + 1], nrm.h[l]));
+    }
+  }
 }
 
 __global__ void __launch_bounds__(256) k_msda_query_inputs(const float* __restrict__ x, const float* __restrict__ pos,
diff --git a/mask_bev_amd/csrc/msda_prepare.hpp b/mask_bev_amd/csrc/msda_prepare.hpp
--- /dev/null
+++ b/mask_bev_amd/csrc/msda_prepare.hpp
@@ -0,0 +1,129 @@
+#pragma once
+#include "common.hpp"
+
+constexpr int kMaxLP = 16;
+
+struct Norm { float w[8], h[8]; };
+
+inline bool fill_norm(const int64_t* shapes_host, int levels, Norm& n) {
+  if (!shapes_host || levels < 1 || levels > 8) return false;
+  for (int l = 0; l < 8; ++l) { n.w[l] = 1.f; n.h[l] = 1.f; }
+  for (int l = 0; l < levels; ++l) {
+    const int64_t h = shapes_host[2 * l], w = shapes_host[2 * l + 1];
+    if (h <= 0 || w <= 0) return false;
+    n.h[l] = (float)h; n.w[l] = (float)w;
+  }
+  return true;
+}
+
+template <typename T>
+__device__ __forceinline__ float ldf(const T* p);
+template <>
+__device__ __forceinline__ float ldf<float>(const float* p) { return *p; }
+template <>
+__device__ __forceinline__ float ldf<unsigned short>(const unsigned short* p) { return __uint_as_float((unsigned)*p << 16); }
+template <typename T>
+__device__ __forceinline__ void stf(T* p, float v);
+template <>
+__device__ __forceinline__ void stf<float>(float* p, float v) { *p = v; }
+template <>
+__device__ __forceinline__ void stf<unsigned short>(unsigned short* p, float v) { *p = f32_to_bf16_rne(v); }
+template <typename T>
+__device__ __forceinline__ float round_like(float v);
+template <>
+__device__ __forceinline__ float round_like<float>(float v) { return v; }
+template <>
+__device__ __forceinline__ float round_like<unsigned short>(float v) { return __uint_as_float((unsigned)f32_to_bf16_rne(v) << 16); }
+
+template <typename T>
+__device__ __forceinline__ void ld4(const T* p, float* v);
+template <>
+__device__ __forceinline__ void ld4<float>(const float* p, float* v) {
+  const float4 q = *reinterpret_cast<const float4*>(p);
+  v[0] = q.x; v[1] = q.y; v[2] = q.z; v[3] = q.w;
+}
+template <>
+__device__ __forceinline__ void ld4<unsigned short>(const unsigned short* p, float* v) {
+  const uint2 u = *reinterpret_cast<const uint2*>(p);
+  v[0] = __uint_as_float(u.x << 16); v[1] = __uint_as_float(u.x & 0xffff0000u);
+  v[2] = __uint_as_float(u.y << 16); v[3] = __uint_as_float(u.y & 0xffff0000u);
+}
+template <typename T>
+__device__ __forceinline__ void st4(T* p, const float* v);
+template <>
+__device__ __forceinline__ void st4<float>(float* p, const float* v) {
+  *reinterpret_cast<float4*>(p) = make_float4(v[0], v[1], v[2], v[3]);
+}
+template <>
+__device__ __forceinline__ void st4<unsigned short>(unsigned short* p, const float* v) {
+  uint2 u;
+  u.x = pack_bf16x2(v[0], v[1]);
+  u.y = pack_bf16x2(v[2], v[3]);
+  *reinterpret_cast<uint2*>(p) = u;
+}
+
+template <>
+__device__ __forceinline__ float ldf<_Float16>(const _Float16* p) { return (float)*p; }
+template <>
+__device__ __forceinline__ void stf<_Float16>(_Float16* p, float v) { *p = (_Float16)v; }
+template <>
+__device__ __forceinline__ float round_like<_Float16>(float v) { return (float)(_Float16)v; }
+template <>
+__device__ __forceinline__ void ld4<_Float16>(const _Float16* p, float* v) {
+  typedef _Float16 h4 __attribute__((ext_vector_type(4)));
+  const h4 q = *reinterpret_cast<const h4*>(p);
+  v[0] = (float)q[0]; v[1] = (float)q[1]; v[2] = (float)q[2]; v[3] = (float)q[3];
+}
+template <>
+__device__ __forceinline__ void st4<_Float16>(_Float16* p, const float* v) {
+  typedef _Float16 h4 __attribute__((ext_vector_type(4)));
+  h4 q;
+  q[0] = (_Float16)v[0]; q[1] = (_Float16)v[1]; q[2] = (_Float16)v[2]; q[3] = (_Float16)v[3];
+  *reinterpret_cast<h4*>(p) = q;
+}
+
+template <typename T>
+__device__ __forceinline__ void msda_prepare_row_fwd(float (&v)[kMaxLP], float (&o)[2 * kMaxLP], const float* ba,
+                                                     const float* bo, float rx, float ry, const Norm& nrm, int lp,
+                                                     int points) {
+#pragma clang fp contract(off)
+  if (ba) {
+#pragma unroll
+    for (int k = 0; k < kMaxLP; ++k) {
+      const float bk = ba[k < lp ? k : 0];
+      v[k] = k < lp ? v[k] + bk : v[k];
+    }
+  }
+  float m = -INFINITY;
+#pragma unroll
+  for (int k = 0; k < kMaxLP; ++k) m = fmaxf(m, v[k]);
+  float s = 0.f;
+#pragma unroll
+  for (int k = 0; k < kMaxLP; ++k) {
+    v[k] = k < lp ? expf(v[k] - m) : 0.f;
+    s += v[k];
+  }
+  const float inv = 1.f / s;
+#pragma unroll
+  for (int k = 0; k < kMaxLP; ++k) {
+    const int kk = k < lp ? k : 0;
+    const int l = kk / points;
+    v[k] = v[k] * inv;
+    float ox = o[2 * k], oy = o[2 * k + 1];
+    if (bo) { ox += bo[2 * kk]; oy += bo[2 * kk + 1]; }
+    ox = rx + round_like<T>(ox / nrm.w[l]);
+    oy = ry + round_like<T>(oy / nrm.h[l]);
+    o[2 * k] = k < lp ? ox : 0.f;
+    o[2 * k + 1] = k < lp ? oy : 0.f;
+  }
+}
+
+__device__ __forceinline__ float msda_prepare_dot_step(float dot, float a, float g) { return fmaf(a, g, dot); }
+__device__ __forceinline__ float msda_prepare_logit_bwd(float a, float g, float dot) {
+#pragma clang fp contract(off)
+  return a * (g - dot);
+}
+template <typename T>
+__device__ __forceinline__ float msda_prepare_offset_bwd(float g_loc, float normaliser) {
+  return round_like<T>(g_loc) / normaliser;
+}
diff --git a/mask_bev_amd/layers.py b/mask_bev_amd/layers.py
--- a/mask_bev_amd/layers.py
+++ b/mask_bev_amd/layers.py
@@ -284,9 +284,11 @@
         if (spatial_shapes is not None and query.is_cuda and query.dtype == torch.float32
                 and query_pos.shape[0] == 1 and sum(hh * ww for hh, ww in spatial_shapes) == n
                 and ops.msda_prepare_supported(l, p)):
+            lo_dt = torch.get_autocast_dtype('cuda') if torch.is_autocast_enabled('cuda') else None
             out = ops.msda_query_side(query, query_pos, reference_points, self.value_proj, self.sampling_offsets,
                                       self.attention_weights, h, l, p, spatial_shapes, shapes_t, level_start,
-                                      pos_share=pos_share, pos_share_index=pos_share_index, wcat=wcat)
+                                      pos_share=pos_share, pos_share_index=pos_share_index, wcat=wcat,
+                                      out_dtype=lo_dt if lo_dt in ops._LO_DTYPES else None)
             out = self.output_proj(out, skip_bias_grad=defer_out_bias and not add_identity)
             return out + query if add_identity else out
         q = query + query_pos
diff --git a/mask_bev_amd/ops_msda.py b/mask_bev_amd/ops_msda.py
--- a/mask_bev_amd/ops_msda.py
+++ b/mask_bev_amd/ops_msda.py
@@ -55,8 +55,12 @@
                 and _lib.load().mbv_ms_deform_attn_bwd_value_packed_supported(d, nl, npnt, nq, host))
 
 
+def msda_fused_ok(head_dim: int, levels: int, points: int) -> bool:
+    return bool(switches.get('msda_fused') and _lib.load().mbv_msda_fused_supported(head_dim, levels, points))
+
+
 def _msda_backward(lib, g_out, value, shapes_t, level_start, loc, attn, dims, host, g_value, g_loc, g_attn,
-                   packed_out=None):
+                   packed_out=None, prep_out=None):
     if packed_out is not None:
         b, nv, nh, d, nl, nq, npnt = dims
         dst, ld = packed_out
@@ -64,6 +68,15 @@
         check(lib.mbv_ms_deform_attn_bwd_value_packed(_ptr(g_out), _ptr(loc), _ptr(attn), b, nv, nh, d, nl, nq, npnt, host,
                                                       _ptr(dst), _dt_flag(dst.dtype), int(ld), _ptr(ws), ws.numel(), _stream()),
               'mbv_ms_deform_attn_bwd_value_packed')
+        if prep_out is not None:
+            g, c0, lo = prep_out
+            esz = g.element_size()
+            check(lib.mbv_ms_deform_attn_bwd_locattn_prep(_ptr(g_out), _ptr(value), _dt_flag(value.dtype), _ptr(shapes_t),
+                                                          _ptr(level_start), _ptr(loc), _ptr(attn), host, b, nv, nh, d, nl, nq,
+                                                          npnt, _dt_flag(g.dtype), ctypes.c_void_p(g.data_ptr() + c0 * esz),
+                                                          g.stride(0), ctypes.c_void_p(g.data_ptr() + (c0 + lo) * esz),
+                                                          g.stride(0), _stream()), 'mbv_ms_deform_attn_bwd_locattn_prep')
+            return
         check(lib.mbv_ms_deform_attn_bwd_locattn(_ptr(g_out), _ptr(value), _dt_flag(value.dtype), _ptr(shapes_t),
                                                  _ptr(level_start), _ptr(loc), _ptr(attn), b, nv, nh, d, nl, nq, npnt,
                                                  _ptr(g_loc), _ptr(g_attn), _stream()), 'mbv_ms_deform_attn_bwd_locattn')
@@ -159,7 +172,7 @@
 
     @staticmethod
     def forward(ctx, x, pos, ref, wv, bv, wo, bo, wa, ba, heads, levels, points, shapes_host, shapes_t, level_start,
-                share=None, share_index=0, wcat=None):
+                share=None, share_index=0, wcat=None, out_dtype=None):
         lib = _lib.load()
         ctx.share = (share, int(share_index))
         _need_gpu(x, pos, ref, wv, wo, wa)
@@ -204,15 +217,27 @@
         attn = torch.empty((b, n, heads, levels, points), dtype=torch.float32, device=x.device)
         esz = ol.element_size()
         bo32, ba32 = bo.float().contiguous(), ba.float().contiguous()
-        check(lib.mbv_msda_prepare_fwd_ld(_ptr(ol), lo + la, ctypes.c_void_p(ol.data_ptr() + lo * esz), lo + la,
-                                          _ptr(bo32), _ptr(ba32), _dt_flag(dt),
-                                          _ptr(ref32), host, b, n, heads, levels, points, _ptr(loc), _ptr(attn), _stream()),
-              'mbv_msda_prepare_fwd_ld')
-        del ol
-        out = torch.empty((b, n, e), dtype=torch.float32, device=x.device)
-        check(lib.mbv_ms_deform_attn_fwd_v(_ptr(value), _dt_flag(value.dtype), _ptr(shapes_t), _ptr(level_start), _ptr(loc),
-                                           _ptr(attn), b, n, heads, d, levels, n, points, _ptr(out), _stream()),
-              'mbv_ms_deform_attn_fwd_v')
+        out = torch.empty((b, n, e), dtype=dt if out_dtype == dt else torch.float32, device=x.device)
+        fused = msda_fused_ok(d, levels, points)
+        if fused:
+            check(lib.mbv_ms_deform_attn_fwd_prep(_ptr(value), _dt_flag(value.dtype), _ptr(shapes_t), _ptr(level_start),
+                                                  _ptr(ol), lo + la, ctypes.c_void_p(ol.data_ptr() + lo * esz), lo + la,
+                                                  _ptr(bo32), _ptr(ba32), _dt_flag(dt), _ptr(ref32), host, b, n, heads, d,
+                                                  levels, n, points, _ptr(loc), _ptr(attn), _ptr(out), _dt_flag(out.dtype),
+                                                  _stream()), 'mbv_ms_deform_attn_fwd_prep')
+            del ol
+        else:
+            check(lib.mbv_msda_prepare_fwd_ld(_ptr(ol), lo + la, ctypes.c_void_p(ol.data_ptr() + lo * esz), lo + la,
+                                              _ptr(bo32), _ptr(ba32), _dt_flag(dt),
+                                              _ptr(ref32), host, b, n, heads, levels, points, _ptr(loc), _ptr(attn), _stream()),
+                  'mbv_msda_prepare_fwd_ld')
+            del ol
+            out32 = out if out.dtype == torch.float32 else torch.empty((b, n, e), dtype=torch.float32, device=x.device)
+            check(lib.mbv_ms_deform_attn_fwd_v(_ptr(value), _dt_flag(value.dtype), _ptr(shapes_t), _ptr(level_start), _ptr(loc),
+                                               _ptr(attn), b, n, heads, d, levels, n, points, _ptr(out32), _stream()),
+                  'mbv_ms_deform_attn_fwd_v')
+            if out32 is not out:
+                out.copy_(out32)
         ctx.save_for_backward(xb, qb, value, loc, attn, shapes_t, level_start, wcat)
         ctx.params = (wv, bv, wo, bo, wa, ba)
         ctx.meta = (heads, levels, points, host, tuple(shapes_host), dt, x.dtype, pos.dtype, tuple(pos.shape))
@@ -231,28 +256,32 @@
         t = b * n
         dev = xb.device
         g_out = g_out.to(torch.float32).contiguous()
-        g_loc = torch.empty_like(loc)
-        g_attn = torch.empty_like(attn)
         host_b = (ctypes.c_int64 * (2 * levels))(*[int(v) for hw in shapes_host for v in hw])
         g = torch.empty((t, width), dtype=dt, device=dev)
+        esz = g.element_size()
         dims = (b, n, heads, d, levels, n, points)
         packed = ((dt in _LO_DTYPES or (dt == torch.float32 and switches.get('msda_packed_f32'))) and width % 2 == 0
                   and msda_value_packed_ok(dims, host_b))
         if value.dtype in _LO_DTYPES and not packed:
             raise MaskBevHipError('MSDA backward: the forward kept a 16-bit value map, which only the packed value gradient '
                                   'reads, and that path is unavailable now (switch changed between forward and backward?)')
+        fused = packed and msda_fused_ok(d, levels, points) and width % 2 == 0 and e % 2 == 0
+        g_loc = g_attn = None
+        if not fused:
+            g_loc = torch.empty_like(loc)
+            g_attn = torch.empty_like(attn)
         if packed:
             _msda_backward(lib, g_out, value, shapes_t, level_start, loc, attn, dims, host_b, None, g_loc, g_attn,
-                           packed_out=(g, width))
+                           packed_out=(g, width), prep_out=(g, e, lo) if fused else None)
         else:
             g_value = torch.empty_like(value)
             _msda_backward(lib, g_out, value, shapes_t, level_start, loc, attn, dims, host_b, g_value, g_loc, g_attn)
             g[:, :e].copy_(g_value.view(t, e))
-        esz = g.element_size()
-        check(lib.mbv_msda_prepare_bwd_ld(_ptr(g_loc), _ptr(g_attn), _ptr(attn), host, b, n, heads, levels, points,
-                                          _dt_flag(dt), ctypes.c_void_p(g.data_ptr() + e * esz), width,
-                                          ctypes.c_void_p(g.data_ptr() + (e + lo) * esz), width, _stream()),
-              'mbv_msda_prepare_bwd_ld')
+        if not fused:
+            check(lib.mbv_msda_prepare_bwd_ld(_ptr(g_loc), _ptr(g_attn), _ptr(attn), host, b, n, heads, levels, points,
+                                              _dt_flag(dt), ctypes.c_void_p(g.data_ptr() + e * esz), width,
+                                              ctypes.c_void_p(g.data_ptr() + (e + lo) * esz), width, _stream()),
+                  'mbv_msda_prepare_bwd_ld')
         od = {} if dt == torch.float32 else dict(out_dtype=torch.float32)
         gx = gpos = None
         if ctx.needs_input_grad[0]:
@@ -307,7 +336,7 @@
             for j, bia in enumerate((bv, bo, ba)):
                 if not deferred[j]:
                     _fire_grad_hooks(bia)
-        return (gx, gpos, None) + tuple(grads) + (None,) * 9
+        return (gx, gpos, None) + tuple(grads) + (None,) * 10
 
 
 @torch.no_grad()
@@ -338,11 +367,11 @@
 
 
 def msda_query_side(x, pos, ref, value_proj, sampling_offsets, attention_weights, heads, levels, points, spatial_shapes,
-                    shapes_t, level_start, pos_share=None, pos_share_index=0, wcat=None):
+                    shapes_t, level_start, pos_share=None, pos_share_index=0, wcat=None, out_dtype=None):
     host = tuple((int(h), int(w)) for h, w in spatial_shapes)
     return _MSDAQuerySide.apply(x, pos, ref, value_proj.weight, value_proj.bias, sampling_offsets.weight,
                                 sampling_offsets.bias, attention_weights.weight, attention_weights.bias, heads, levels,
-                                points, host, shapes_t, level_start, pos_share, pos_share_index, wcat)
+                                points, host, shapes_t, level_start, pos_share, pos_share_index, wcat, out_dtype)
 
 
 __all__ = [_n for _n in list(globals()) if not _n.startswith('__')]
diff --git a/mask_bev_amd/switches.py b/mask_bev_amd/switches.py
--- a/mask_bev_amd/switches.py
+++ b/mask_bev_amd/switches.py
@@ -21,6 +21,7 @@
     'ffn32': True,
     'k4_split': True,
     'k6_split': True,
+    'msda_fused': True,
     'msda_packed_f32': True,
     'ln_bound_hints': True,
     'conv3x3_k20': True,
diff --git a/mask_bev_amd/workmodel.py b/mask_bev_amd/workmodel.py
--- a/mask_bev_amd/workmodel.py
+++ b/mask_bev_amd/workmodel.py
@@ -76,6 +76,22 @@
     if bwd:
         return ('k_msda_bwd_locattn', 'hbm', vmap + qmap + 2 * samples * 12.0, 0.0)
     return ('k_msda_fwd_v4', 'hbm', vmap + qmap + samples * 12.0, 0.0)
+
+
+def _msda_fused(a, bwd: bool) -> Work:
+    if bwd:
+        ves = 4.0 if _i(a[2]) == 0 else 2.0
+        b, nv, heads, d, levels, nq, pts = (_i(a[i]) for i in range(8, 15))
+        es = 4.0 if _i(a[15]) == 0 else 2.0
+        go = b * nq * heads * d * 4.0
+    else:
+        ves = 4.0 if _i(a[1]) == 0 else 2.0
+        b, nv, heads, d, levels, nq, pts = (_i(a[i]) for i in range(13, 20))
+        es = 4.0 if _i(a[10]) == 0 else 2.0
+        go = b * nq * heads * d * (4.0 if _i(a[23]) == 0 else 2.0)
+    samples = b * nq * heads * levels * pts
+    return ('k_msda_bwd_locattn_p4_prep' if bwd else 'k_msda_fwd_p4_prep', 'hbm',
+            b * nv * heads * d * ves + go + samples * 12.0 + samples * 3.0 * es, 0.0)
 
 
 def _msda_value_packed(a) -> Work:
@@ -316,6 +332,8 @@
     'mbv_ms_deform_attn_fwd_v': lambda a: _msda_typed(a, False),
     'mbv_ms_deform_attn_bwd_locattn': lambda a: _msda_typed(a, True),
     'mbv_ms_deform_attn_bwd_value_packed': _msda_value_packed,
+    'mbv_ms_deform_attn_fwd_prep': lambda a: _msda_fused(a, False),
+    'mbv_ms_deform_attn_bwd_locattn_prep': lambda a: _msda_fused(a, True),
     'mbv_rowchain_run': _rowchain,
     'mbv_rowchain_run_split': _rowchain_split,
     'mbv_attn_fwd': lambda a: _attn(a, False, False),
```

Result: no change. 180.1 scans/s (median of 2 runs) (-0.1%).
